# EdoardoLuciani/ARayTracingJourney

Measured on AMD Instinct MI355X. Metric: Mray/s (primary+shadow), Sponza-class 1080p, higher is better.
Workload: dtype f32; 1 GPU; sponza_like(seed=0x5A0A, 262816 triangles, 25 primitives) 1920x1080, 1 light(s), 794216 shadow rays/frame; width=1920, height=1080, lights=1, parallelism=single GPU, 8 frames in flight

## Files before the change

### araytracingjourney_amd/_abi.py

```python
import ctypes as C

ART_OK = 0
ART_E_INVALID = -1
ART_E_STATE = -2
ART_E_NO_DEVICE = -3
ART_E_HIP = -4
ART_E_NOMEM = -5
ART_FLAG_FAST_BUILD = 2
ART_FLAG_PACKED_TILES = 4
ART_FLAG_FIXED_WAVES = 16
ART_FLAG_TILE_OUTPUT = 32
ART_FLAG_DYNAMIC_SCENE = 64
ART_FLAG_KEEP_DEBUG = 1
ART_MASK_ALL = 255
ART_VIS_CAMERA = 1
ART_VIS_SHADOW = 2
ART_VIS_AO = 4
ART_VIS_QUERY = 8
ART_VERTS_FULL = 0
ART_VERTS_POSITIONS = 1
ART_CAST_CLOSEST = 0
ART_CAST_ANY = 1
ART_CAST_MAX_RAYS = 2147418112
ART_CAST_POOL = 32
# ... 93 lines not shown
                ("layout", C.c_uint32),
                ("stride_bytes", C.c_uint32),
                ("flags", C.c_uint32),
                ("reserved", C.c_uint32)]


class ArtRayCast(C.Structure):
    _fields_ = [("rays_dev", C.c_void_p),
                ("tuv_dev", C.c_void_p),
                ("ids_dev", C.c_void_p),
                ("hit_dev", C.c_void_p),
                ("hip_stream", C.c_void_p),
                ("n", C.c_uint32),
                ("kind", C.c_uint32),
                ("cull_mask", C.c_uint32),
                ("flags", C.c_uint32)]


class ArtRayCastMulti(C.Structure):
    _fields_ = [("rays_dev", C.c_void_p),
                ("tuv_dev", C.c_void_p),
                ("ids_dev", C.c_void_p),
                ("count_dev", C.c_void_p),
                ("hip_stream", C.c_void_p),
                ("n", C.c_uint32),
                ("max_hits", C.c_uint32),
                ("cull_mask", C.c_uint32),
                ("flags", C.c_uint32)]


class ArtRayCrossings(C.Structure):
    _fields_ = [("rays_dev", C.c_void_p),
                ("cross_dev", C.c_void_p),
                ("hip_stream", C.c_void_p),
                ("n", C.c_uint32),
                ("cull_mask", C.c_uint32),
                ("flags", C.c_uint32),
                ("reserved", C.c_uint32)]


class ArtHitResolve(C.Structure):
    _fields_ = [("tuv_dev", C.c_void_p),
                ("ids_dev", C.c_void_p),
                ("pos_dev", C.c_void_p),
                ("ng_dev", C.c_void_p),
                ("ns_dev", C.c_void_p),
                ("uv_dev", C.c_void_p),
                ("albedo_dev", C.c_void_p),
                ("orm_dev", C.c_void_p),
                ("hip_stream", C.c_void_p),
                ("n", C.c_uint32),
                ("flags", C.c_uint32)]


class ArtPointQuery(C.Structure):
    _fields_ = [("points_dev", C.c_void_p),
                ("duv_dev", C.c_void_p),
                ("ids_dev", C.c_void_p),
                ("point_dev", C.c_void_p),
                ("hip_stream", C.c_void_p),
                ("n", C.c_uint32),
                ("cull_mask", C.c_uint32),
                ("flags", C.c_uint32),
                ("reserved", C.c_uint32)]


class ArtSphereCast(C.Structure):
    _fields_ = [("rays_dev", C.c_void_p),
                ("tuv_dev", C.c_void_p),
                ("ids_dev", C.c_void_p),
                ("point_dev", C.c_void_p),
                ("hip_stream", C.c_void_p),
                ("n", C.c_uint32),
                ("cull_mask", C.c_uint32),
                ("flags", C.c_uint32),
                ("radius", C.c_float)]


class ArtPointQueryMulti(C.Structure):
    _fields_ = [("points_dev", C.c_void_p),
                ("duv_dev", C.c_void_p),
                ("ids_dev", C.c_void_p),
                ("point_dev", C.c_void_p),
                ("count_dev", C.c_void_p),
                ("hip_stream", C.c_void_p),
                ("n", C.c_uint32),
                ("max_hits", C.c_uint32),
                ("cull_mask", C.c_uint32),
                ("flags", C.c_uint32)]


class ArtBoxQuery(C.Structure):
    _fields_ = [("boxes_dev", C.c_void_p),
                ("hit_dev", C.c_void_p),
                ("ids_dev", C.c_void_p),
                ("count_dev", C.c_void_p),
                ("hip_stream", C.c_void_p),
                ("n", C.c_uint32),
                ("kind", C.c_uint32),
                ("max_hits", C.c_uint32),
                ("cull_mask", C.c_uint32),
                ("flags", C.c_uint32),
                ("reserved", C.c_uint32)]


class ArtTriQuery(C.Structure):
    _fields_ = [("tris_dev", C.c_void_p),
                ("hit_dev", C.c_void_p),
                ("ids_dev", C.c_void_p),
                ("count_dev", C.c_void_p),
                ("hip_stream", C.c_void_p),
                ("n", C.c_uint32),
                ("kind", C.c_uint32),
                ("max_hits", C.c_uint32),
                ("cull_mask", C.c_uint32),
                ("flags", C.c_uint32),
                ("reserved", C.c_uint32)]


class ArtTriDistance(C.Structure):
    _fields_ = [("tris_dev", C.c_void_p),
                ("duv_dev", C.c_void_p),
                ("ids_dev", C.c_void_p),
                ("point_dev", C.c_void_p),
                ("qpoint_dev", C.c_void_p),
                ("hip_stream", C.c_void_p),
                ("n", C.c_uint32),
                ("cull_mask", C.c_uint32),
                ("flags", C.c_uint32),
                ("reserved", C.c_uint32)]


class ArtLayout(C.Structure):
    _fields_ = [("width", C.c_uint32),
                ("height", C.c_uint32),
                ("frames_in_flight", C.c_uint32),
                ("frames_per_launch", C.c_uint32),
                ("shard_rank", C.c_uint32),
                ("shard_count", C.c_uint32),
                ("tiles_owned", C.c_uint32),
                ("tiles_padded", C.c_uint32),
                ("tile_bytes", C.c_uint32),
                ("reserved", C.c_uint32)]


class ArtMgpuConfig(C.Structure):
    _fields_ = [("rank", C.c_uint32),
                ("world", C.c_uint32),
                ("compositor", C.c_uint32),
                ("launches_per_gather", C.c_uint32),
                ("tile_buffers", C.c_uint32),
                ("transport", C.c_uint32),
                ("exchange", ArtMgpuExchangeFn),
                ("exchange_user", C.c_void_p),
                ("roots", C.c_uint32),
                ("reserved", C.c_uint32)]


class ArtGlbCopyInfo(C.Structure):
    _fields_ = [("mesh_buffer_offset", C.c_uint64),
                ("mesh_size", C.c_uint64),
                ("indices_buffer_offset", C.c_uint64),
                ("indices_size", C.c_uint64),
                ("image_buffer_offset", C.c_uint64),
                ("image_size", C.c_uint64),
                ("single_mesh_element_size", C.c_uint32),
                ("single_index_size", C.c_uint32),
                ("image_format", C.c_uint32),
                ("image_width", C.c_uint32),
                ("image_height", C.c_uint32),
                ("image_mip_levels", C.c_uint32),
                ("image_layers", C.c_uint32),
                ("reserved", C.c_uint32)]


SYMBOLS = {
    "art_last_error": (C.c_char_p, []),
    "art_device_count": (C.c_int32, []),
    "art_create": (C.c_int32, [C.c_void_p, C.c_void_p]),
    "art_destroy": (C.c_int32, [C.c_void_p]),
    "art_set_stream": (C.c_int32, [C.c_void_p, C.c_void_p]),
    "art_set_frames_per_launch": (C.c_int32, [C.c_void_p, C.c_uint32]),
    "art_set_camera_batch": (C.c_int32, [C.c_void_p, C.c_void_p, C.c_uint32]),
    "art_set_read_frame": (C.c_int32, [C.c_void_p, C.c_uint32]),
    "art_frames_in_flight": (C.c_int32, [C.c_void_p, C.c_void_p, C.c_void_p]),
    "art_frames_done": (C.c_int32, [C.c_void_p, C.c_uint64, C.c_uint32, C.c_void_p, C.c_void_p]),
    "art_scene_add_primitive": (C.c_int32, [C.c_void_p, C.c_void_p, C.c_uint32, C.c_void_p, C.c_uint32, C.c_uint32, C.c_void_p, C.c_uint32, C.c_uint32, C.c_void_p, C.c_void_p]),
    "art_scene_clear": (C.c_int32, [C.c_void_p]),
    "art_scene_set_primitive_enabled": (C.c_int32, [C.c_void_p, C.c_uint32, C.c_int32]),
    "art_scene_set_alpha_cutoff": (C.c_int32, [C.c_void_p, C.c_uint32, C.c_float]),
    "art_scene_set_primitive_mask": (C.c_int32, [C.c_void_p, C.c_uint32, C.c_uint32]),
    "art_set_ray_masks": (C.c_int32, [C.c_void_p, C.c_uint32, C.c_uint32, C.c_uint32]),
    "art_scene_needs_build": (C.c_int32, [C.c_void_p]),
    "art_scene_set_model_matrix": (C.c_int32, [C.c_void_p, C.c_uint32, C.c_uint32, C.c_void_p]),
    "art_scene_set_vertices": (C.c_int32, [C.c_void_p, C.c_uint32, C.c_void_p, C.c_uint32]),
    "art_scene_set_vertices_device": (C.c_int32, [C.c_void_p, C.c_void_p]),
    "art_scene_get_vertices": (C.c_int32, [C.c_void_p, C.c_uint32, C.c_void_p, C.c_uint32]),
    "art_scene_build": (C.c_int32, [C.c_void_p]),
    "art_set_camera": (C.c_int32, [C.c_void_p, C.c_void_p]),
    "art_camera_from_params": (C.c_int32, [C.c_void_p, C.c_void_p, C.c_float, C.c_float, C.c_float, C.c_float, C.c_void_p]),
    "art_set_lights": (C.c_int32, [C.c_void_p, C.c_void_p, C.c_uint32]),
    "art_light_point": (C.c_int32, [C.c_void_p, C.c_void_p, C.c_float, C.c_int32, C.c_void_p]),
    "art_light_spot": (C.c_int32, [C.c_void_p, C.c_void_p, C.c_void_p, C.c_float, C.c_float, C.c_float, C.c_int32, C.c_void_p]),
    "art_light_directional": (C.c_int32, [C.c_void_p, C.c_void_p, C.c_int32, C.c_void_p]),
    "art_light_area": (C.c_int32, [C.c_void_p, C.c_void_p, C.c_void_p, C.c_int32, C.c_void_p, C.c_float, C.c_float, C.c_float, C.c_int32, C.c_void_p]),
    "art_resize": (C.c_int32, [C.c_void_p, C.c_uint32, C.c_uint32]),
    "art_trace": (C.c_int32, [C.c_void_p]),
    "art_trace_ao": (C.c_int32, [C.c_void_p, C.c_uint32, C.c_float]),
    "art_read_ao": (C.c_int32, [C.c_void_p, C.c_void_p, C.c_size_t]),
    "art_present": (C.c_int32, [C.c_void_p]),
    "art_read_present": (C.c_int32, [C.c_void_p, C.c_void_p, C.c_size_t]),
    "art_read_packed": (C.c_int32, [C.c_void_p, C.c_void_p, C.c_void_p, C.c_void_p]),
    "art_lpm_control_block": (C.c_int32, [C.c_int32, C.c_float, C.c_float, C.c_float, C.c_float, C.c_float, C.c_void_p, C.c_void_p, C.c_void_p]),
    "art_sync": (C.c_int32, [C.c_void_p]),
    "art_cast_rays": (C.c_int32, [C.c_void_p, C.c_void_p]),
    "art_cast_rays_multi": (C.c_int32, [C.c_void_p, C.c_void_p]),
    "art_cast_crossings": (C.c_int32, [C.c_void_p, C.c_void_p]),
    "art_cast_sync": (C.c_int32, [C.c_void_p]),
    "art_cast_counts": (C.c_int32, [C.c_void_p, C.c_void_p, C.c_void_p, C.c_void_p]),
    "art_resolve_hits": (C.c_int32, [C.c_void_p, C.c_void_p]),
    "art_closest_points": (C.c_int32, [C.c_void_p, C.c_void_p]),
    "art_cast_spheres": (C.c_int32, [C.c_void_p, C.c_void_p]),
    "art_closest_points_multi": (C.c_int32, [C.c_void_p, C.c_void_p]),
    "art_overlap_boxes": (C.c_int32, [C.c_void_p, C.c_void_p]),
    "art_overlap_triangles": (C.c_int32, [C.c_void_p, C.c_void_p]),
    "art_closest_triangles": (C.c_int32, [C.c_void_p, C.c_void_p]),
    "art_read_color": (C.c_int32, [C.c_void_p, C.c_void_p, C.c_size_t]),
    "art_read_depth": (C.c_int32, [C.c_void_p, C.c_void_p, C.c_size_t]),
    "art_read_normal": (C.c_int32, [C.c_void_p, C.c_void_p, C.c_size_t]),
    "art_device_color": (C.c_int32, [C.c_void_p, C.c_void_p, C.c_void_p]),
    "art_device_depth": (C.c_int32, [C.c_void_p, C.c_void_p, C.c_void_p]),
    "art_device_normal": (C.c_int32, [C.c_void_p, C.c_void_p, C.c_void_p]),
    "art_shard_tile_count": (C.c_int32, [C.c_void_p, C.c_void_p, C.c_void_p]),
    "art_shard_layout": (C.c_int32, [C.c_uint32, C.c_uint32, C.c_uint32, C.c_uint32, C.c_uint32, C.c_void_p, C.c_uint32, C.c_void_p, C.c_void_p]),
    "art_device_color_tiles": (C.c_int32, [C.c_void_p, C.c_void_p, C.c_void_p]),
    "art_untile_gathered": (C.c_int32, [C.c_void_p, C.c_void_p, C.c_uint32, C.c_void_p, C.c_void_p]),
    "art_get_layout": (C.c_int32, [C.c_void_p, C.c_void_p]),
    "art_mgpu_shard": (C.c_int32, [C.c_uint32, C.c_uint32, C.c_uint32, C.c_void_p, C.c_void_p]),
    "art_mgpu_unique_id": (C.c_int32, [C.c_void_p]),
    "art_mgpu_create": (C.c_int32, [C.c_void_p, C.c_void_p, C.c_void_p, C.c_void_p]),
    "art_mgpu_trace": (C.c_int32, [C.c_void_p]),
    "art_mgpu_flush": (C.c_int32, [C.c_void_p]),
    "art_mgpu_device_frame": (C.c_int32, [C.c_void_p, C.c_void_p, C.c_void_p]),
    "art_mgpu_read_frame": (C.c_int32, [C.c_void_p, C.c_void_p, C.c_size_t]),
    "art_mgpu_counts": (C.c_int32, [C.c_void_p, C.c_void_p, C.c_void_p, C.c_void_p]),
    "art_mgpu_destroy": (C.c_int32, [C.c_void_p]),
    "art_get_stats": (C.c_int32, [C.c_void_p, C.c_void_p]),
    "art_glb_last_error": (C.c_char_p, []),
    "art_glb_open": (C.c_int32, [C.c_char_p, C.c_int32, C.c_int32, C.c_void_p]),
    "art_glb_close": (C.c_int32, [C.c_void_p]),
    "art_glb_primitive_count": (C.c_int32, [C.c_void_p, C.c_void_p]),
    "art_glb_primitive_alpha": (C.c_int32, [C.c_void_p, C.c_uint32, C.c_void_p, C.c_void_p, C.c_void_p]),
    "art_glb_copy_model_data": (C.c_int32, [C.c_void_p, C.c_uint32, C.c_uint32, C.c_void_p, C.c_size_t, C.c_void_p, C.c_uint32, C.c_void_p]),
    "art_glb_bounding_sphere": (C.c_int32, [C.c_void_p, C.c_void_p, C.c_void_p]),
    "art_glb_permute_pixels": (C.c_int32, [C.c_void_p, C.c_size_t, C.c_uint32, C.c_void_p, C.c_uint32, C.c_uint32, C.c_void_p, C.c_size_t]),
    "art_scene_add_glb": (C.c_int32, [C.c_void_p, C.c_void_p, C.c_void_p, C.c_void_p, C.c_void_p]),
}



class ArtTuning(C.Structure):
    _fields_ = [("frame_form", C.c_uint32),
                ("tree_builder", C.c_uint32),
                ("packet_wide", C.c_uint32),
                ("primary_walk", C.c_uint32),
                ("shadow_walk", C.c_uint32),
                ("ao_walk", C.c_uint32),
                ("block_order", C.c_uint32),
                ("fixed_waves", C.c_uint32),
                ("split_fixed_steps", C.c_uint32),
                ("split_min_steps", C.c_uint32),
                ("split_alpha", C.c_float),
                ("ao_entry_off", C.c_uint32),
                ("trace_chunk", C.c_uint32),
                ("trace_refill", C.c_uint32),
                ("trace_blocks", C.c_uint32),
                ("hw_queues", C.c_uint32),
                ("log", C.c_uint32),
                ("wide_builder", C.c_uint32),
                ("as_versions", C.c_uint32),
                ("refit_rebuild_ratio", C.c_float),
                ("trace_leaf_batch", C.c_uint32),
                ("plan_moving_interval", C.c_uint32),
                ("refit_streams", C.c_uint32),
                ("refit_fold_nodes", C.c_uint32),
                ("shadow_hints", C.c_uint32),
                ("plain_math", C.c_uint32)]


PARITY_SYMBOLS = {
    "art_set_tuning": (C.c_int32, [C.c_void_p, C.c_void_p]),
    "art_read_hits": (C.c_int32, [C.c_void_p, C.c_void_p, C.c_void_p, C.c_size_t]),
    "art_read_shadow_bits": (C.c_int32, [C.c_void_p, C.c_void_p, C.c_size_t]),
    "art_read_shadow_hints": (C.c_int32, [C.c_void_p, C.c_void_p, C.c_size_t]),
    "art_write_shadow_hints": (C.c_int32, [C.c_void_p, C.c_void_p, C.c_size_t]),
    "art_query_closest": (C.c_int32, [C.c_void_p, C.c_void_p, C.c_uint32, C.c_void_p, C.c_void_p]),
    "art_query_any": (C.c_int32, [C.c_void_p, C.c_void_p, C.c_uint32, C.c_void_p]),
    "art_query_closest_masked": (C.c_int32, [C.c_void_p, C.c_void_p, C.c_uint32, C.c_uint32, C.c_void_p, C.c_void_p]),
    "art_query_any_masked": (C.c_int32, [C.c_void_p, C.c_void_p, C.c_uint32, C.c_uint32, C.c_void_p]),
    "art_get_lbvh": (C.c_int32, [C.c_void_p, C.c_void_p, C.c_void_p, C.c_void_p, C.c_void_p, C.c_void_p, C.c_void_p, C.c_void_p]),
    "art_get_traversal_tree": (C.c_int32, [C.c_void_p, C.c_void_p, C.c_void_p, C.c_void_p]),
    "art_get_wide_nodes": (C.c_int32, [C.c_void_p, C.c_void_p, C.c_void_p, C.c_size_t, C.c_void_p]),
    "art_parity_math_sweep": (C.c_int32, [C.c_void_p, C.c_uint32, C.c_uint32, C.c_uint64, C.c_uint32, C.c_void_p, C.c_void_p, C.c_void_p, C.c_void_p]),
    "art_parity_radiance_sweep": (C.c_int32, [C.c_void_p, C.c_uint32, C.c_uint32, C.c_uint64, C.c_uint32, C.c_float, C.c_void_p, C.c_void_p, C.c_void_p, C.c_void_p]),
    "art_bind_color_tiles": (C.c_int32, [C.c_void_p, C.c_uint32, C.c_void_p, C.c_size_t]),
    "art_bind_color_tiles_pair": (C.c_int32, [C.c_void_p, C.c_uint32, C.c_void_p, C.c_void_p, C.c_size_t]),
    "art_bind_color_tiles_ring": (C.c_int32, [C.c_void_p, C.c_uint32, C.c_void_p, C.c_uint32, C.c_size_t]),
    "art_read_color_tiles": (C.c_int32, [C.c_void_p, C.c_void_p, C.c_size_t]),
    "art_untile_gathered_strided": (C.c_int32, [C.c_void_p, C.c_void_p, C.c_uint32, C.c_uint32, C.c_void_p, C.c_void_p]),
    "art_untile_gathered_frames": (C.c_int32, [C.c_void_p, C.c_void_p, C.c_uint32, C.c_uint32, C.c_uint32, C.c_void_p, C.c_void_p]),
    "art_stream_wait_frame": (C.c_int32, [C.c_void_p, C.c_void_p]),
    "art_trace_for_stream": (C.c_int32, [C.c_void_p, C.c_void_p, C.c_void_p]),
    "art_wait_external_event": (C.c_int32, [C.c_void_p, C.c_void_p]),
    "art_set_graph_mode": (C.c_int32, [C.c_void_p, C.c_int32]),
    "art_timestamp_mark": (C.c_int32, [C.c_void_p, C.c_uint32]),
    "art_timestamp_elapsed": (C.c_int32, [C.c_void_p, C.c_void_p]),
    "art_collect_timings": (C.c_int32, [C.c_void_p, C.c_void_p, C.c_void_p]),
    "art_sample_wave_steps": (C.c_int32, [C.c_void_p, C.c_void_p, C.c_void_p, C.c_uint32, C.c_void_p]),
    "art_parity_plan": (C.c_int32, [C.c_void_p, C.c_uint32, C.c_void_p, C.c_void_p, C.c_uint32, C.c_void_p, C.c_void_p, C.c_void_p, C.c_uint32, C.c_float, C.c_uint32, C.c_uint32, C.c_void_p, C.c_void_p, C.c_void_p, C.c_void_p]),
    "art_read_wave_plan": (C.c_int32, [C.c_void_p, C.c_void_p, C.c_size_t, C.c_void_p, C.c_uint32, C.c_void_p, C.c_void_p, C.c_void_p]),
    "art_parity_live_resources": (C.c_int32, [C.c_void_p]),
    "art_vertex_update_counts": (C.c_int32, [C.c_void_p, C.c_void_p, C.c_void_p, C.c_void_p]),
    "art_mgpu_pending": (C.c_int32, [C.c_void_p, C.c_void_p, C.c_void_p]),
}
```

### araytracingjourney_amd/csrc/art_api.hip

```cpp
#include "art_context.h"
#include <mutex>
#include <cmath>
#include <cstdio>
#include <cstdlib>
#include <cstring>
#include <new>

static thread_local std::string g_err;
int32_t art::fail(int32_t code, const std::string &msg) { g_err = msg; return code; }
int32_t art::hipfail(hipError_t e, const char *what) { return fail(ART_E_HIP, std::string(what) + ": " + hipGetErrorString(e)); }
void art::set_last_error(const char *msg) { g_err = msg ? msg : ""; }

static std::mutex g_stream_mutex;
static std::vector<std::pair<int, hipStream_t>> g_free_streams;
hipError_t art::acquire_stream(int device, hipStream_t *out) {
    {
        std::lock_guard<std::mutex> lock(g_stream_mutex);
        for (size_t i = 0; i < g_free_streams.size(); i++)
            if (g_free_streams[i].first == device) { *out = g_free_streams[i].second; g_free_streams.erase(g_free_streams.begin() + (long)i); live_add(kLivePooled, -1); live_add(kLiveStreams, 1); return hipSuccess; }
    }
    hipError_t e = hipStreamCreateWithFlags(out, hipStreamNonBlocking);
    if (e == hipSuccess) live_add(kLiveStreams, 1); else *out = nullptr;
    return e;
}
// ... 654 lines not shown
    if (owned) *owned = mine;
    if (padded) *padded = mx;
    return ART_OK;
}
int32_t art_shard_tile_count(ArtContext *c, uint32_t *owned, uint32_t *padded) {
    if (!c) return fail(ART_E_INVALID, "art_shard_tile_count: null context");
    int32_t r = ensure_layout(c, "art_shard_tile_count"); if (r) return r;
    if (owned) *owned = (uint32_t)c->tile_list.size();
    if (padded) *padded = c->padded_tiles;
    return ART_OK;
}
int32_t art_device_color_tiles(ArtContext *c, void **p, size_t *b) {
    int32_t r = device_ready(c, p, "art_device_color_tiles"); if (r) return r;
    *p = nullptr; if (b) *b = 0;
    if (!c->tiled()) return fail(ART_E_STATE, "art_device_color_tiles: context is not sharded");
    FrameSlot &S = c->slot[c->last];
    const size_t one = c->tiles_bytes();
    *p = (char *)S.last_tiles() + c->read_b * one; if (b) *b = one;
    return ART_OK;
}
int32_t art_bind_color_tiles(ArtContext *c, uint32_t slot, void *dev, size_t bytes) {
    if (!c) return fail(ART_E_INVALID, "art_bind_color_tiles: null context");
    if (!c->tiled()) return fail(ART_E_STATE, "art_bind_color_tiles: context is not sharded");
    if (slot >= c->F) return fail(ART_E_INVALID, "art_bind_color_tiles: slot >= frames in flight");
    int32_t r = ensure_layout(c, "art_bind_color_tiles"); if (r) return r;
    if (dev && bytes != c->tiles_bytes() * c->B) return fail(ART_E_INVALID, "art_bind_color_tiles: size mismatch (padded tiles x tile bytes x frames per launch)");
    HIPC(hipStreamSynchronize(c->stream_of(slot)));
    c->slot[slot].ext_tiles = (float4 *)dev; c->slot[slot].ext_ring_n = 0; c->slot[slot].tiles_of_last = nullptr; c->slot[slot].ext_tiles_bytes = dev ? bytes : 0;
    drop_graphs(c);
    return ART_OK;
}
int32_t art_bind_color_tiles_pair(ArtContext *c, uint32_t slot, void *dev_even, void *dev_odd, size_t bytes) {
    if (!dev_even || !dev_odd) return fail(ART_E_INVALID, "art_bind_color_tiles_pair: null buffer");
    void *two[2] = {dev_even, dev_odd};
    return art_bind_color_tiles_ring(c, slot, two, 2, bytes);
}
int32_t art_bind_color_tiles_ring(ArtContext *c, uint32_t slot, void *const *bufs, uint32_t n, size_t bytes) {
    if (!bufs || n == 0 || n > FrameSlot::kTileRing) return fail(ART_E_INVALID, "art_bind_color_tiles_ring: 1..8 buffers");
    for (uint32_t i = 0; i < n; i++) if (!bufs[i]) return fail(ART_E_INVALID, "art_bind_color_tiles_ring: null buffer");
    int32_t r = art_bind_color_tiles(c, slot, bufs[0], bytes); if (r) return r;
    for (uint32_t i = 0; i < n; i++) c->slot[slot].ext_ring[i] = (float4 *)bufs[i];
    c->slot[slot].ext_ring_n = n;
    return ART_OK;
}
int32_t art_set_graph_mode(ArtContext *c, int32_t on) {
    if (!c) return fail(ART_E_INVALID, "art_set_graph_mode: null context");
    if (on && c->ext_stream) return fail(ART_E_STATE, "art_set_graph_mode: not with an external stream");
    c->graph_mode = on != 0;
    if (!on) drop_graphs(c);
    return ART_OK;
}
int32_t art_frames_in_flight(ArtContext *c, uint32_t *frames, uint32_t *next_slot) {
    if (!c) return fail(ART_E_INVALID, "art_frames_in_flight: null context");
    if (frames) *frames = c->F;
    if (next_slot) *next_slot = (uint32_t)(c->frame_no % c->F);
    return ART_OK;
}
int32_t art_frames_done(ArtContext *c, uint64_t first, uint32_t count, int32_t *done, uint64_t *traced) {
    if (!c || !done) return fail(ART_E_INVALID, "art_frames_done: null argument");
    if (traced) *traced = c->frame_no;
    *done = 0;
    if (count == 0) { *done = 1; return ART_OK; }
    if (first + count > c->frame_no) return fail(ART_E_INVALID, "art_frames_done: frames not traced yet");
    if (c->frame_no - first > (uint64_t)ArtContext::kRing) return fail(ART_E_INVALID, "art_frames_done: older than the 128 frames whose events are kept");
    int32_t r = use_device(c); if (r) return r;
    for (uint64_t f = first + count; f-- > first;) {
        hipError_t e = hipEventQuery(c->ev[f % ArtContext::kRing][4]);
        if (e == hipErrorNotReady) return ART_OK;
        if (e != hipSuccess) return hipfail(e, "art_frames_done: hipEventQuery");
    }
    *done = 1;
    return ART_OK;
}
int32_t art_stream_wait_frame(ArtContext *c, void *hip_stream) {
    if (!c) return fail(ART_E_INVALID, "art_stream_wait_frame: null context");
    if (!c->traced) return fail(ART_E_STATE, "art_stream_wait_frame: nothing traced yet");
    int32_t r = use_device(c); if (r) return r;
    { FrameSlot &S = c->slot[c->last]; HIPC(hipStreamWaitEvent((hipStream_t)hip_stream, S.done_alias ? S.done_alias : S.done, 0)); }
    return ART_OK;
}
int32_t art_trace_for_stream(ArtContext *c, void *hip_stream, uint32_t *slot_used) {
    if (!c) return fail(ART_E_INVALID, "art_trace_for_stream: null context");
    const uint32_t k = (uint32_t)(c->frame_no % c->F);
    int32_t r = art_trace(c); if (r) return r;
    if (slot_used) *slot_used = k;
    return art_stream_wait_frame(c, hip_stream);
}
int32_t art_wait_external_event(ArtContext *c, void *hip_event) {
    if (!c) return fail(ART_E_INVALID, "art_wait_external_event: null context");
    c->slot[c->frame_no % c->F].wait_event = hip_event;
    return ART_OK;
}
int32_t art_collect_timings(ArtContext *c, float sums_ms[5], uint32_t *n_frames) {
    if (!c || !sums_ms || !n_frames) return fail(ART_E_INVALID, "art_collect_timings: null argument");
    int32_t r = use_device(c); if (r) return r;
    r = sync_all(c); if (r) return r;
    uint64_t from = c->collected_upto;
    if (c->frame_no - from > (uint64_t)ArtContext::kRing) from = c->frame_no - ArtContext::kRing;
    for (int k = 0; k < 5; k++) sums_ms[k] = 0.f;
    for (uint64_t f = from; f < c->frame_no; f++) {
        const Event *ev = c->ev[f % ArtContext::kRing];
        float ms = 0;
        if (c->ev_fused[f % ArtContext::kRing]) { HIPC(hipEventElapsedTime(&ms, ev[0], ev[4])); sums_ms[0] += ms; sums_ms[4] += ms; continue; }
        for (int k = 0; k < 4; k++) { HIPC(hipEventElapsedTime(&ms, ev[k], ev[k + 1])); sums_ms[k] += ms; }
        HIPC(hipEventElapsedTime(&ms, ev[0], ev[4])); sums_ms[4] += ms;
    }
    *n_frames = (uint32_t)(c->frame_no - from);
    c->collected_upto = c->frame_no;
    return ART_OK;
}
int32_t art_read_color_tiles(ArtContext *c, void *dst, size_t bytes) {
    if (c && !c->tiled()) return fail(ART_E_STATE, "art_read_color_tiles: context is not sharded");
    FrameSlot *S = c ? &c->slot[c->last] : nullptr;
    const size_t one = c ? c->tiles_bytes() : 0;
    return read_back(c, S ? (const char *)S->last_tiles() + c->read_b * one : nullptr, one, dst, bytes, "art_read_color_tiles");
}
int32_t art_untile_gathered_frames(ArtContext *c, const void *gathered_dev, uint32_t shard_count, uint32_t shard_stride_tiles, uint32_t n_frames, void *frames_dev, void *hip_stream) {
    if (!c || !gathered_dev) return fail(ART_E_INVALID, "art_untile_gathered: null argument");
    int32_t r = ensure_layout(c, "art_untile_gathered"); if (r) return r;
    if (shard_stride_tiles < c->padded_tiles) return fail(ART_E_INVALID, "art_untile_gathered: stride smaller than a shard's padded tile count");
    if (n_frames == 0 || (n_frames > 1 && (!frames_dev || (uint64_t)n_frames * c->padded_tiles > shard_stride_tiles))) return fail(ART_E_INVALID, "art_untile_gathered_frames: frames do not fit the shard stride (or no output given)");
    if (shard_count != (c->cfg.shard_count > 1 ? c->cfg.shard_count : 1)) return fail(ART_E_INVALID, "art_untile_gathered: shard_count differs from the context's");
    r = use_device(c); if (r) return r;
    hipStream_t us = hip_stream ? (hipStream_t)hip_stream : c->stream_of(c->last);
    if (c->tiles_packed()) {
        FrameSlot &S = c->slot[c->last];
        if (!frames_dev && S.d_pcolor.n < (size_t)c->W * c->H) { HIPC(hipStreamSynchronize(us)); HIPC(S.d_pcolor.ensure((size_t)c->W * c->H)); }
        launch_untile_packed((const uint32_t *)gathered_dev, c->d_tile_slot.p, shard_stride_tiles, n_frames, c->padded_tiles, c->W, c->H, frames_dev ? (uint32_t *)frames_dev : S.d_pcolor.p, us);
    } else
    launch_untile((const float4 *)gathered_dev, c->d_tile_slot.p, shard_stride_tiles, n_frames, c->padded_tiles, c->W, c->H, frames_dev ? (float4 *)frames_dev : c->slot[c->last].d_color.p, us);
    HIPC(hipGetLastError());
    c->traced = true;
    return ART_OK;
}
int32_t art_untile_gathered_strided(ArtContext *c, const void *gathered_dev, uint32_t shard_count, uint32_t shard_stride_tiles, void *frame_dev, void *hip_stream) {
    return art_untile_gathered_frames(c, gathered_dev, shard_count, shard_stride_tiles, 1, frame_dev, hip_stream);
}
int32_t art_untile_gathered(ArtContext *c, const void *gathered_dev, uint32_t shard_count, void *frame_dev, void *hip_stream) {
    if (!c) return fail(ART_E_INVALID, "art_untile_gathered: null argument");
    int32_t r = ensure_layout(c, "art_untile_gathered"); if (r) return r;
    return art_untile_gathered_strided(c, gathered_dev, shard_count, c->padded_tiles, frame_dev, hip_stream);
}

int32_t art_get_layout(ArtContext *c, ArtLayout *out) {
    if (!c || !out) return fail(ART_E_INVALID, "art_get_layout: null argument");
    int32_t r = ensure_layout(c, "art_get_layout"); if (r) return r;
    std::memset(out, 0, sizeof(*out));
    out->width = c->W; out->height = c->H; out->frames_in_flight = c->F; out->frames_per_launch = c->B;
    out->shard_rank = c->cfg.shard_count > 1 ? c->cfg.shard_rank : 0; out->shard_count = c->cfg.shard_count > 1 ? c->cfg.shard_count : 1;
    out->tiles_owned = (uint32_t)c->tile_list.size(); out->tiles_padded = c->padded_tiles; out->tile_bytes = c->tiled() ? (uint32_t)(kTilePixels * c->tile_px_bytes()) : 0u;
    return ART_OK;
}
int32_t art_timestamp_mark(ArtContext *c, uint32_t which) {
    if (!c || which > 1) return fail(ART_E_INVALID, "art_timestamp_mark: mark 0 or 1");
    if (!c->traced) return fail(ART_E_STATE, "art_timestamp_mark: nothing traced yet");
    int32_t r = use_device(c); if (r) return r;
    HIPC(c->mark[which].create());
    HIPC(hipEventRecord(c->mark[which], c->stream_of(c->last)));
    return ART_OK;
}
int32_t art_timestamp_elapsed(ArtContext *c, float *ms) {
    if (!c || !ms) return fail(ART_E_INVALID, "art_timestamp_elapsed: null argument");
    if (!c->mark[0] || !c->mark[1]) return fail(ART_E_STATE, "art_timestamp_elapsed: both marks must have been recorded");
    int32_t r = use_device(c); if (r) return r;
    HIPC(hipEventSynchronize(c->mark[1]));
    HIPC(hipEventElapsedTime(ms, c->mark[0], c->mark[1]));
    return ART_OK;
}

int32_t art_get_stats(ArtContext *c, ArtStats *out) {
    if (!c || !out) return fail(ART_E_INVALID, "art_get_stats: null argument");
    if (c->traced && c->frame_ready) {
        int32_t r = use_device(c); if (r) return r;
        r = sync_all(c); if (r) return r;
        std::vector<uint32_t> raw(kCounterWords);
        if (c->fused_frame()) {
            FrameSlot &S = c->slot[c->last];
            HIPC(hipMemsetAsync(S.d_counters.p, 0, kCounterWords * 4, c->stream_of(c->last)));
            if (c->n_local) {
                FrameArgs fa = make_frame_args(c, S, S.as_version);
                fa.pix_bits += (size_t)c->read_b * c->n_local; fa.depth += (size_t)c->read_b * c->W * c->H;
                launch_frame_stats(fa, S.d_counters.p, c->stream_of(c->last)); HIPC(hipGetLastError());
            }
            HIPC(hipStreamSynchronize(c->stream_of(c->last)));
        }
        HIPC(hipMemcpy(raw.data(), c->slot[c->last].d_counters.p, kCounterWords * 4, hipMemcpyDeviceToHost));
        uint64_t cnt[2] = {raw[0], raw[1]};
        for (uint32_t k = 0; k < kSlotCount; k++) { cnt[0] += raw[kShadowSlots + k * kSlotStride]; cnt[1] += raw[kHitSlots + k * kSlotStride]; }
        uint64_t owned = 0;
        for (uint32_t t : c->tile_list) {
            uint32_t tx = t % c->tiles_x, ty = t / c->tiles_x;
            uint32_t w = (tx + 1) * kTile <= c->W ? kTile : c->W - tx * kTile, h = (ty + 1) * kTile <= c->H ? kTile : c->H - ty * kTile;
            owned += (uint64_t)w * h;
        }
        c->stats.primary_rays = owned; c->stats.shadow_rays = cnt[0]; c->stats.hit_pixels = cnt[1];
        c->stats.frame_launches = c->fused_frame() ? 1u : 4u;
        c->stats.split_blocks = c->plan.split1 + c->plan.split2;
        harvest_cost(c);
        c->stats.ao_rays = (uint64_t)c->ao_spp * cnt[1];
        if (c->ao_spp && c->slot[c->last].ao_valid) { float ams = 0; if (hipEventElapsedTime(&ams, c->slot[c->last].ao_ev[0], c->slot[c->last].ao_ev[1]) == hipSuccess) c->stats.ao_ms = ams; }
        float ms = 0;
        if (c->frame_no) {
            const Event *ev = c->ev[(c->frame_no - 1) % ArtContext::kRing];
            if (hipEventElapsedTime(&ms, ev[0], ev[4]) == hipSuccess) c->stats.frame_ms = ms;
            if (c->ev_fused[(c->frame_no - 1) % ArtContext::kRing]) { c->stats.trace_primary_ms = c->stats.frame_ms; c->stats.shade_ms = c->stats.trace_shadow_ms = c->stats.accumulate_ms = 0.f; }
            else {
            if (hipEventElapsedTime(&ms, ev[0], ev[1]) == hipSuccess) c->stats.trace_primary_ms = ms;
            if (hipEventElapsedTime(&ms, ev[1], ev[2]) == hipSuccess) c->stats.shade_ms = ms;
            if (hipEventElapsedTime(&ms, ev[2], ev[3]) == hipSuccess) c->stats.trace_shadow_ms = ms;
            if (hipEventElapsedTime(&ms, ev[3], ev[4]) == hipSuccess) c->stats.accumulate_ms = ms;
            }
        }
    }
    as_fill_stats(c, &c->stats);
    *out = c->stats;
    return ART_OK;
}

static bool local_to_xy(const ArtContext *c, uint32_t p, uint32_t &x, uint32_t &y) {
    const uint32_t tile = c->tile_list[p >> 10], q = p & 1023u, sub = q >> 6, l = q & 63u;
    x = (tile % c->tiles_x) * kTile + (sub & 3u) * 8u + (l & 7u); y = (tile / c->tiles_x) * kTile + (sub >> 2) * 8u + (l >> 3);
    return x < c->W && y < c->H;
}
int32_t art_read_hits(ArtContext *c, float *tuv, int32_t *ids, size_t n_pixels) {
    if (!c || !tuv || !ids) return fail(ART_E_INVALID, "art_read_hits: null argument");
    if (!c->traced) return fail(ART_E_STATE, "art_read_hits: nothing traced yet");
    if (n_pixels != (size_t)c->W * c->H) return fail(ART_E_INVALID, "art_read_hits: size mismatch");
    if (c->fused_frame() && !(c->cfg.flags & ART_FLAG_KEEP_DEBUG)) return fail(ART_E_STATE, "art_read_hits: fused frames keep hit records only with ART_FLAG_KEEP_DEBUG");
    int32_t r = use_device(c); if (r) return r;
    r = sync_all(c); if (r) return r;
    std::vector<float4> h(c->n_local);
    std::vector<DevTri> tris(c->T);
    HIPC(hipMemcpy(h.data(), c->slot[c->last].d_hits.p + (size_t)c->read_b * c->n_local, (size_t)c->n_local * 16, hipMemcpyDeviceToHost));
    HIPC(hipMemcpy(tris.data(), c->bvh.tris, (size_t)c->T * sizeof(DevTri), hipMemcpyDeviceToHost));
    for (size_t i = 0; i < n_pixels; i++) { tuv[4 * i] = 0; tuv[4 * i + 1] = 0; tuv[4 * i + 2] = 0; tuv[4 * i + 3] = 0; ids[2 * i] = -2; ids[2 * i + 1] = -2; }
    for (uint32_t p = 0; p < c->n_local; p++) {
        uint32_t x, y;
        if (!local_to_xy(c, p, x, y)) continue;
        size_t i = (size_t)y * c->W + x;
        uint32_t pos; std::memcpy(&pos, &h[p].w, 4);
        tuv[4 * i] = h[p].x; tuv[4 * i + 1] = h[p].y; tuv[4 * i + 2] = h[p].z;
        if (pos == kNoHit) { ids[2 * i] = -1; ids[2 * i + 1] = -1; }
        else { uint32_t gid; std::memcpy(&gid, &tris[pos].f[15], 4); gid_to_ids(c, gid, ids + 2 * i); }
    }
    return ART_OK;
}

int32_t art_read_shadow_bits(ArtContext *c, uint32_t *bits, size_t n_pixels) {
    if (!c || !bits) return fail(ART_E_INVALID, "art_read_shadow_bits: null argument");
    if (!(c->cfg.flags & ART_FLAG_KEEP_DEBUG)) return fail(ART_E_STATE, "art_read_shadow_bits: context created without ART_FLAG_KEEP_DEBUG");
    if (!c->traced) return fail(ART_E_STATE, "art_read_shadow_bits: nothing traced yet");
    if (n_pixels != (size_t)c->W * c->H) return fail(ART_E_INVALID, "art_read_shadow_bits: size mismatch");
    int32_t r = use_device(c); if (r) return r;
    r = sync_all(c); if (r) return r;
    std::vector<uint32_t> sb(c->n_local);
    HIPC(hipMemcpy(sb.data(), c->slot[c->last].d_shadow_bits.p + (size_t)c->read_b * c->n_local, (size_t)c->n_local * 4, hipMemcpyDeviceToHost));
    std::memset(bits, 0, n_pixels * 4);
    for (uint32_t p = 0; p < c->n_local; p++) {
        uint32_t x, y;
        if (!local_to_xy(c, p, x, y)) continue;
        bits[(size_t)y * c->W + x] = sb[p];
    }
    return ART_OK;
}

int32_t art_read_shadow_hints(ArtContext *c, uint32_t *words, size_t n_words) {
    if (!c || !words) return fail(ART_E_INVALID, "art_read_shadow_hints: null argument");
    int32_t r = use_device(c); if (r) return r;
    r = sync_all(c); if (r) return r;
    if (!c->frame_ready) return fail(ART_E_STATE, "art_read_shadow_hints: no frame layout yet (art_trace)");
    if (n_words != c->hint_words()) return fail(ART_E_INVALID, "art_read_shadow_hints: size mismatch");
    if (n_words) HIPC(hipMemcpy(words, c->d_hints.p, n_words * 4, hipMemcpyDeviceToHost));
    return ART_OK;
}
int32_t art_write_shadow_hints(ArtContext *c, const uint32_t *words, size_t n_words) {
    if (!c || !words) return fail(ART_E_INVALID, "art_write_shadow_hints: null argument");
    int32_t r = use_device(c); if (r) return r;
    r = sync_all(c); if (r) return r;
    if (!c->frame_ready) return fail(ART_E_STATE, "art_write_shadow_hints: no frame layout yet (art_trace)");
    if (n_words != c->hint_words()) return fail(ART_E_INVALID, "art_write_shadow_hints: size mismatch");
    if (n_words) HIPC(hipMemcpy(c->d_hints.p, words, n_words * 4, hipMemcpyHostToDevice));
    HIPC(hipDeviceSynchronize());
    return ART_OK;
}

int32_t art_parity_math_sweep(ArtContext *c, uint32_t which, uint32_t first_bits, uint64_t count, uint32_t stride, uint64_t *mismatches, uint32_t *first_bad_bits,
                              uint64_t *fast_lanes, float guard[2]) {
    if (!c || !mismatches || !first_bad_bits || !fast_lanes || !guard) return fail(ART_E_INVALID, "art_parity_math_sweep: null argument");
    if (which > 4 || count > (1ull << 32)) return fail(ART_E_INVALID, "art_parity_math_sweep: which 0..4, at most 2^32 patterns");
    int32_t r = use_device(c); if (r) return r;
    r = sync_all(c); if (r) return r;
    math_sweep_guard(guard);
    unsigned long long h[3] = {0ull, ~0ull, 0ull};
    DevBuf<unsigned long long> d;
    HIPC(d.ensure(3));
    HIPC(hipMemcpy(d.p, h, sizeof h, hipMemcpyHostToDevice));
    launch_math_sweep(which, first_bits, count, stride, d.p, nullptr); HIPC(hipGetLastError());
    HIPC(hipMemcpy(h, d.p, sizeof h, hipMemcpyDeviceToHost));
    *mismatches = h[0]; *fast_lanes = h[2];
    if (h[0]) *first_bad_bits = first_bits + (uint32_t)h[1] * stride;
    return ART_OK;
}

int32_t art_parity_radiance_sweep(ArtContext *c, uint32_t which, uint32_t first_bits, uint64_t count, uint32_t stride, float numerator, uint32_t *max_ulps, uint32_t *worst_bits,
                                  uint64_t *class_mismatches, uint32_t *first_class_bits) {
    if (!c || !max_ulps || !worst_bits || !class_mismatches || !first_class_bits) return fail(ART_E_INVALID, "art_parity_radiance_sweep: null argument");
    if (which > 1 || count > (1ull << 32)) return fail(ART_E_INVALID, "art_parity_radiance_sweep: which 0..1, at most 2^32 patterns");
    int32_t r = use_device(c); if (r) return r;
    r = sync_all(c); if (r) return r;
    unsigned long long h[3] = {0ull, 0ull, ~0ull};
    DevBuf<unsigned long long> d;
    HIPC(d.ensure(3));
    HIPC(hipMemcpy(d.p, h, sizeof h, hipMemcpyHostToDevice));
    launch_radiance_sweep(which, first_bits, count, stride, numerator, d.p, nullptr); HIPC(hipGetLastError());
    HIPC(hipMemcpy(h, d.p, sizeof h, hipMemcpyDeviceToHost));
    *max_ulps = (uint32_t)(h[0] >> 32); *class_mismatches = h[1];
    if (h[0]) *worst_bits = first_bits + (uint32_t)h[0] * stride;
    if (h[1]) *first_class_bits = first_bits + (uint32_t)h[2] * stride;
    return ART_OK;
}

int32_t art_parity_live_resources(uint64_t out[5]) {
    if (!out) return fail(ART_E_INVALID, "art_parity_live_resources: null argument");
    for (int i = 0; i < 5; i++) out[i] = g_live[i].load(std::memory_order_relaxed);
    return ART_OK;
}

}
```

### araytracingjourney_amd/csrc/art_device.h

```cpp
#pragma once
#include "art_internal.h"

namespace art {

struct V3 { float x, y, z; };
__device__ __forceinline__ V3 mk(float x, float y, float z) { V3 r; r.x = x; r.y = y; r.z = z; return r; }
__device__ __forceinline__ V3 operator+(V3 a, V3 b) { return mk(a.x + b.x, a.y + b.y, a.z + b.z); }
__device__ __forceinline__ V3 operator-(V3 a, V3 b) { return mk(a.x - b.x, a.y - b.y, a.z - b.z); }
__device__ __forceinline__ V3 operator*(V3 a, V3 b) { return mk(a.x * b.x, a.y * b.y, a.z * b.z); }
__device__ __forceinline__ V3 operator*(V3 a, float s) { return mk(a.x * s, a.y * s, a.z * s); }
__device__ __forceinline__ V3 neg(V3 a) { return mk(-a.x, -a.y, -a.z); }
__device__ __forceinline__ float dot3(V3 a, V3 b) { return fmaf(a.z, b.z, fmaf(a.y, b.y, a.x * b.x)); }
__device__ __forceinline__ V3 cross3(V3 a, V3 b) {
    return mk(fmaf(a.y, b.z, -(a.z * b.y)), fmaf(a.z, b.x, -(a.x * b.z)), fmaf(a.x, b.y, -(a.y * b.x)));
}
constexpr float kExactLo = 0x1p-96f, kExactHi = 0x1p96f;
__device__ __forceinline__ float sqrt_core(float x) {
    float s = __builtin_amdgcn_sqrtf(x);
    float dn = __uint_as_float(__float_as_uint(s) - 1u), up = __uint_as_float(__float_as_uint(s) + 1u);
    float vp = fmaf(-dn, s, x), vs = fmaf(-up, s, x);
    s = vp <= 0.0f ? dn : s;
    return vs > 0.0f ? up : s;
}
__device__ __forceinline__ float rcp_core(float d) {
    float r = __builtin_amdgcn_rcpf(d);
    r = fmaf(fmaf(-d, r, 1.0f), r, r);
    float q = fmaf(fmaf(-d, r, 1.0f), r, r);
    return fmaf(fmaf(-d, q, 1.0f), r, q);
}
__device__ __forceinline__ bool exact_in_range(float x, bool plain) {
    return !plain && __builtin_amdgcn_ballot_w64(!(x >= kExactLo && x <= kExactHi)) == 0ull;
}
template <bool FAST = true> __device__ __forceinline__ float inv_sqrt_exact(float x, bool plain, bool &fast) {
    fast = FAST && exact_in_range(x, plain);
    if (fast) return rcp_core(sqrt_core(x));
    return 1.0f / sqrtf(x);
}
template <bool FAST = true> __device__ __forceinline__ float sqrt_exact(float x, bool plain, bool &fast) {
    fast = FAST && exact_in_range(x, plain);
    if (fast) return sqrt_core(x);
    return sqrtf(x);
}
__device__ __forceinline__ void exact_note(float x, uint32_t &far) { far = max(far, __float_as_uint(x) - __float_as_uint(kExactLo)); }
__device__ __forceinline__ bool exact_noted_in_range(uint32_t far) { return __builtin_amdgcn_ballot_w64(far > __float_as_uint(kExactHi) - __float_as_uint(kExactLo)) == 0ull; }
template <bool FAST = true> __device__ __forceinline__ float len3(V3 a, bool plain = false) { bool f; return sqrt_exact<FAST>(dot3(a, a), plain, f); }
template <bool FAST = true> __device__ __forceinline__ V3 nrm3(V3 a, bool plain = false) { bool f; float inv = inv_sqrt_exact<FAST>(dot3(a, a), plain, f); return a * inv; }
__device__ __forceinline__ float inv_sqrt_noting(float x, uint32_t &far) { exact_note(x, far); return rcp_core(sqrt_core(x)); }
template <bool CORE> __device__ __forceinline__ V3 nrm3_noting(V3 a, uint32_t &far) {
    float x = dot3(a, a);
    return a * (CORE ? inv_sqrt_noting(x, far) : 1.0f / sqrtf(x));
}
__device__ __forceinline__ float clampf(float x, float lo, float hi) { return fminf(fmaxf(x, lo), hi); }
__device__ __forceinline__ float mixf(float x, float y, float a) { return x * (1.0f - a) + y * a; }
__device__ __forceinline__ V3 ld3(const float *p) { return mk(p[0], p[1], p[2]); }
__device__ __forceinline__ V3 mat4_mul(const float *m, float x, float y, float z, float w) {
    return mk(((m[0] * x + m[4] * y) + m[8] * z) + m[12] * w, ((m[1] * x + m[5] * y) + m[9] * z) + m[13] * w,
              ((m[2] * x + m[6] * y) + m[10] * z) + m[14] * w);
}
__device__ __forceinline__ V3 xform_point(const float *m, V3 p) {
    return mk(((m[0] * p.x + m[1] * p.y) + m[2] * p.z) + m[3], ((m[4] * p.x + m[5] * p.y) + m[6] * p.z) + m[7],
              ((m[8] * p.x + m[9] * p.y) + m[10] * p.z) + m[11]);
}
__device__ __forceinline__ V3 xform_vec(const float *m, V3 p) {
    return mk((m[0] * p.x + m[1] * p.y) + m[2] * p.z, (m[4] * p.x + m[5] * p.y) + m[6] * p.z, (m[8] * p.x + m[9] * p.y) + m[10] * p.z);
}

__device__ __forceinline__ int wrapi(int i, int n) { int m = i % n; return m < 0 ? m + n : m; }
__device__ __forceinline__ void tex_taps(const uint32_t *__restrict__ pool, uint32_t texture_offset, uint32_t tw_, uint32_t th_, int layer, float u, float v,
                                         uint32_t &t00, uint32_t &t10, uint32_t &t01, uint32_t &t11, float &fx, float &fy) {
    int tw = (int)tw_, th = (int)th_;
    float x = u * (float)tw - 0.5f, y = v * (float)th - 0.5f;
    float x0f = floorf(x), y0f = floorf(y);
    fx = x - x0f; fy = y - y0f;
    int x0 = wrapi((int)x0f, tw), y0 = wrapi((int)y0f, th);
    int x1 = wrapi(x0 + 1, tw), y1 = wrapi(y0 + 1, th);
    const uint32_t *base = pool + texture_offset + (size_t)layer * tw * th;
    t00 = base[(size_t)y0 * tw + x0]; t10 = base[(size_t)y0 * tw + x1]; t01 = base[(size_t)y1 * tw + x0]; t11 = base[(size_t)y1 * tw + x1];
}
__device__ __forceinline__ float tex_channel(uint32_t t00, uint32_t t10, uint32_t t01, uint32_t t11, float fx, float fy, int c) {
    const float k = 1.0f / 255.0f;
    float A = (float)((t00 >> (8 * c)) & 255u) * k, B = (float)((t10 >> (8 * c)) & 255u) * k;
    float Cc = (float)((t01 >> (8 * c)) & 255u) * k, D = (float)((t11 >> (8 * c)) & 255u) * k;
    float top = A * (1.0f - fx) + B * fx, bot = Cc * (1.0f - fx) + D * fx;
    return top * (1.0f - fy) + bot * fy;
}
__device__ inline float4 sample_tex(const uint32_t *__restrict__ pool, const DevPrim &P, int layer, float u, float v) {
    int tw = (int)P.tw, th = (int)P.th;
    float x = u * (float)tw - 0.5f, y = v * (float)th - 0.5f;
    float x0f = floorf(x), y0f = floorf(y);
    float fx = x - x0f, fy = y - y0f;
    int x0 = wrapi((int)x0f, tw), y0 = wrapi((int)y0f, th);
    int x1 = wrapi(x0 + 1, tw), y1 = wrapi(y0 + 1, th);
    const uint32_t *base = pool + P.texture_offset + (size_t)layer * tw * th;
    uint32_t t00 = base[(size_t)y0 * tw + x0], t10 = base[(size_t)y0 * tw + x1], t01 = base[(size_t)y1 * tw + x0], t11 = base[(size_t)y1 * tw + x1];
    float o[4];
#pragma unroll
    for (int c = 0; c < 4; c++) o[c] = tex_channel(t00, t10, t01, t11, fx, fy, c);
    return make_float4(o[0], o[1], o[2], o[3]);
}


struct AlphaView {
    const uint32_t *bits;
    const DevShadeTri *shade;
    const DevPrim *prims;
    const uint32_t *tex;
    uint32_t cull;
};
__device__ __forceinline__ float alpha_at(const uint32_t *__restrict__ pool, uint32_t texture_offset, uint32_t tw, uint32_t th, float4 s2, float4 s3, float u, float v) {
    float bx = 1.0f - u - v, by = u, bz = v;
    float tu = (s2.y * bx + s2.w * by) + s3.y * bz, tv = (s2.z * bx + s3.x * by) + s3.z * bz;
    uint32_t t00, t10, t01, t11; float fx, fy;
    tex_taps(pool, texture_offset, tw, th, 0, tu, tv, t00, t10, t01, t11, fx, fy);
    return tex_channel(t00, t10, t01, t11, fx, fy, 3);
}
__device__ __forceinline__ bool alpha_cut(const AlphaView &av, uint32_t pos, float u, float v) {
    if (av.cull == 0u) return true;
    if (!((av.bits[pos >> 5] >> (pos & 31u)) & 1u)) return false;
    const float4 *sq = reinterpret_cast<const float4 *>(av.shade + pos);
    const float4 s8 = sq[8];
    const DevPrim &P = av.prims[__float_as_uint(s8.z)];
    if ((prim_vis(P.masked) & av.cull) == 0u) return true;
    const float4 s2 = sq[2], s3 = sq[3];
    const float c = P.cutoff;
    if (!(c > 0.0f)) return false;
    return alpha_at(av.tex, P.texture_offset, P.tw, P.th, s2, s3, u, v) < c;
}

struct Ray {
    V3 o, d;
    float tmin, tmax;
    V3 inv, ood;
};
__device__ __forceinline__ float safe_dir(float d) { return fabsf(d) < 1e-20f ? copysignf(1e-20f, d) : d; }
__device__ __forceinline__ void ray_init(Ray &r, V3 o, V3 d, float tmin, float tmax) {
    r.o = o; r.d = d; r.tmin = tmin; r.tmax = tmax;
    r.inv = mk(1.0f / safe_dir(d.x), 1.0f / safe_dir(d.y), 1.0f / safe_dir(d.z));
    r.ood = mk(o.x * r.inv.x, o.y * r.inv.y, o.z * r.inv.z);
}
__device__ __forceinline__ void ray_init_inv(Ray &r, V3 o, V3 d, V3 inv, float tmin, float tmax) {
    r.o = o; r.d = d; r.tmin = tmin; r.tmax = tmax; r.inv = inv;
    r.ood = mk(o.x * inv.x, o.y * inv.y, o.z * inv.z);
}
__device__ __forceinline__ bool ray_finite(V3 o, V3 d) {
    float z = 0.0f * o.x; z = fmaf(0.0f, o.y, z); z = fmaf(0.0f, o.z, z); z = fmaf(0.0f, d.x, z); z = fmaf(0.0f, d.y, z); z = fmaf(0.0f, d.z, z);
    return z == 0.0f;
}
__device__ __forceinline__ bool slab(const Ray &r, float lx, float ly, float lz, float hx, float hy, float hz, float tlimit, float &tn) {
    float t0x = fmaf(lx, r.inv.x, -r.ood.x), t1x = fmaf(hx, r.inv.x, -r.ood.x);
    float t0y = fmaf(ly, r.inv.y, -r.ood.y), t1y = fmaf(hy, r.inv.y, -r.ood.y);
    float t0z = fmaf(lz, r.inv.z, -r.ood.z), t1z = fmaf(hz, r.inv.z, -r.ood.z);
    tn = fmaxf(fmaxf(fminf(t0x, t1x), fminf(t0y, t1y)), fminf(t0z, t1z));
    float tf = fminf(fminf(fmaxf(t0x, t1x), fmaxf(t0y, t1y)), fmaxf(t0z, t1z));
    return fmaxf(tn, r.tmin) <= fminf(tf, tlimit);
}
#define ART_BARY_EPS 1.0e-6f
__device__ __forceinline__ bool moller_trumbore(const Ray &r, V3 v0, V3 e1, V3 e2, float &t, float &u, float &v) {
    V3 p = cross3(r.d, e2);
    float det = dot3(e1, p);
    if (det == 0.0f) return false;
    float inv = 1.0f / det;
    V3 tv = r.o - v0;
    float uu = dot3(tv, p) * inv;
    if (!(uu >= -ART_BARY_EPS && uu <= 1.0f + ART_BARY_EPS)) return false;
    V3 q = cross3(tv, e1);
    float vv = dot3(r.d, q) * inv;
    if (!(vv >= -ART_BARY_EPS && uu + vv <= 1.0f + ART_BARY_EPS)) return false;
    float tt = dot3(e2, q) * inv;
    if (!(tt > r.tmin && tt < r.tmax)) return false;
    t = tt; u = uu; v = vv;
    return true;
}
__device__ __forceinline__ bool moller_trumbore_det(const Ray &r, V3 v0, V3 e1, V3 e2, float &t, float &u, float &v, float &det_out) {
    V3 p = cross3(r.d, e2);
    float det = dot3(e1, p);
    if (det == 0.0f) return false;
    float inv = 1.0f / det;
    V3 tv = r.o - v0;
    float uu = dot3(tv, p) * inv;
    if (!(uu >= -ART_BARY_EPS && uu <= 1.0f + ART_BARY_EPS)) return false;
    V3 q = cross3(tv, e1);
    float vv = dot3(r.d, q) * inv;
    if (!(vv >= -ART_BARY_EPS && uu + vv <= 1.0f + ART_BARY_EPS)) return false;
    float tt = dot3(e2, q) * inv;
    if (!(tt > r.tmin && tt < r.tmax)) return false;
    t = tt; u = uu; v = vv; det_out = det;
    return true;
}

__device__ __forceinline__ bool moller_trumbore_flat(const Ray &r, V3 v0, V3 e1, V3 e2, float &t, float &u, float &v) {
    V3 p = cross3(r.d, e2);
    float det = dot3(e1, p);
    float inv = 1.0f / det;
    V3 tv = r.o - v0;
    u = dot3(tv, p) * inv;
    V3 q = cross3(tv, e1);
    v = dot3(r.d, q) * inv;
    t = dot3(e2, q) * inv;
    return (det != 0.0f) & (u >= -ART_BARY_EPS) & (u <= 1.0f + ART_BARY_EPS) & (v >= -ART_BARY_EPS) & (u + v <= 1.0f + ART_BARY_EPS) & (t > r.tmin) & (t < r.tmax);
}

__device__ __forceinline__ uint64_t moller_trumbore_mask(const Ray &r, V3 v0, V3 e1, V3 e2, float &t, float &u, float &v) {
    V3 p = cross3(r.d, e2);
    float det = dot3(e1, p);
    float inv = 1.0f / det;
    V3 tv = r.o - v0;
    u = dot3(tv, p) * inv;
    V3 q = cross3(tv, e1);
    v = dot3(r.d, q) * inv;
    t = dot3(e2, q) * inv;
    return __builtin_amdgcn_ballot_w64(det != 0.0f) & __builtin_amdgcn_ballot_w64(u >= -ART_BARY_EPS) & __builtin_amdgcn_ballot_w64(u <= 1.0f + ART_BARY_EPS) &
           __builtin_amdgcn_ballot_w64(v >= -ART_BARY_EPS) & __builtin_amdgcn_ballot_w64(u + v <= 1.0f + ART_BARY_EPS) & __builtin_amdgcn_ballot_w64(t > r.tmin) &
           __builtin_amdgcn_ballot_w64(t < r.tmax);
}

constexpr int kLdsStack = 16;
constexpr int kOvfStack = 80;
constexpr int kBlock = 256;
constexpr int kFrameBlock = 64;
constexpr int kTraceBlock = 64;
struct Tune { uint32_t chunk, refill, blocks, leaf_batch; };
static const Tune kPreset[4] = {{64, 12, 1536, 1}, {128, 24, 1024, 1}, {256, 16, 2048, 8}, {1024, 24, 2048, 8}};
static inline Tune tune_over(Tune t, const TraceTune &o) {
    if (o.chunk >= 64 && o.chunk <= 65536) t.chunk = o.chunk;
    if (o.refill >= 1 && o.refill <= 64) t.refill = o.refill;
    if (o.blocks >= 1 && o.blocks <= 16384) t.blocks = o.blocks;
    if (o.leaf_batch >= 1 && o.leaf_batch <= 64) t.leaf_batch = o.leaf_batch;
    return t;
}
static inline Tune tune(bool pipelined, bool ao, const TraceTune &o) { return tune_over(kPreset[(ao ? 2 : 0) + (pipelined ? 1 : 0)], o); }
constexpr int kCursorStride = 32;

__device__ __forceinline__ bool local_to_xy(uint32_t p, const uint32_t *__restrict__ tile_list, uint32_t tiles_x, uint32_t W, uint32_t H, uint32_t &x, uint32_t &y) {
    uint32_t tile = tile_list[p >> 10];
    uint32_t q = p & 1023u, sub = q >> 6, l = q & 63u;
    x = (tile % tiles_x) * kTile + (sub & 3u) * 8u + (l & 7u);
    y = (tile / tiles_x) * kTile + (sub >> 2) * 8u + (l >> 3);
    return x < W && y < H;
}

__device__ __forceinline__ uint32_t launder(uint32_t v) { asm volatile("" : "+s"(v)); return v; }
__device__ __forceinline__ uint32_t launder_v(uint32_t v) { asm volatile("" : "+v"(v)); return v; }
__device__ __forceinline__ uint64_t ballot64(bool p) { return __builtin_amdgcn_ballot_w64(p); }

typedef float f4v __attribute__((ext_vector_type(4)));
__device__ __forceinline__ void st_nt(float4 *p, float4 v) { __builtin_nontemporal_store(f4v{v.x, v.y, v.z, v.w}, reinterpret_cast<f4v *>(p)); }
__device__ __forceinline__ void st_nt(float *p, float v) { __builtin_nontemporal_store(v, p); }
typedef float f3v __attribute__((ext_vector_type(3)));
__device__ __forceinline__ void st_nt_rgb(float4 *tiles, size_t texel, float4 v) { __builtin_nontemporal_store(f3v{v.x, v.y, v.z}, reinterpret_cast<f3v *>(reinterpret_cast<float *>(tiles) + 3 * texel)); }
__device__ __forceinline__ float4 ld_nt(const float4 *p) { f4v v = __builtin_nontemporal_load(reinterpret_cast<const f4v *>(p)); return make_float4(v.x, v.y, v.z, v.w); }

static inline uint32_t blocks_for(uint32_t n) { return (n + kBlock - 1) / kBlock; }
static inline uint32_t persistent_blocks(uint32_t total, const Tune &t) {
    uint32_t need = (total + kTraceBlock - 1) / kTraceBlock, cap = t.blocks * (kBlock / kTraceBlock);
    return need < cap ? (need ? need : 1u) : cap;
}

}
```

### araytracingjourney_amd/csrc/art_frame.hip

```cpp
#include "art_shade.h"
#include <type_traits>

namespace art {

constexpr int kPacketStack = 288;

__device__ __forceinline__ void sel(float &x, float y, uint64_t m) { asm("v_cndmask_b32_e64 %0, %0, %1, %2" : "+v"(x) : "v"(y), "s"(m)); }
__device__ __forceinline__ void sel(uint32_t &x, uint32_t y, uint64_t m) { asm("v_cndmask_b32_e64 %0, %0, %1, %2" : "+v"(x) : "v"(y), "s"(m)); }
__device__ __forceinline__ void sel_off(float &x, uint64_t m) { asm("v_cndmask_b32_e64 %0, %0, -1.0, %1" : "+v"(x) : "s"(m)); }

template <int OCT> __device__ __forceinline__ bool slab_oct(const Ray &r, float lx, float ly, float lz, float hx, float hy, float hz, float tlimit, float &tn) {
    if (OCT >= 8) return slab(r, lx, ly, lz, hx, hy, hz, tlimit, tn);
    float nx = fmaf((OCT & 1) ? hx : lx, r.inv.x, -r.ood.x), fx = fmaf((OCT & 1) ? lx : hx, r.inv.x, -r.ood.x);
    float ny = fmaf((OCT & 2) ? hy : ly, r.inv.y, -r.ood.y), fy = fmaf((OCT & 2) ? ly : hy, r.inv.y, -r.ood.y);
    float nz = fmaf((OCT & 4) ? hz : lz, r.inv.z, -r.ood.z), fz = fmaf((OCT & 4) ? lz : hz, r.inv.z, -r.ood.z);
    tn = fmaxf(fmaxf(nx, ny), nz);
    float tf = fminf(fminf(fx, fy), fz);
    return fmaxf(tn, r.tmin) <= fminf(tf, tlimit);
}

struct ConstQuads {
    typedef float Quad __attribute__((ext_vector_type(4)));
    __attribute__((address_space(4))) const Quad *p;
    __device__ __forceinline__ float4 operator[](int i) const { Quad v = p[i]; return make_float4(v.x, v.y, v.z, v.w); }
};
template <class T> __device__ __forceinline__ ConstQuads const_quads(const T *p) { ConstQuads q; q.p = (__attribute__((address_space(4))) const ConstQuads::Quad *)(uintptr_t)p; return q; }

#ifdef ART_PACKET_PROF
__device__ unsigned long long g_packet_prof[24];
#define PPROF(i, n) do { if ((threadIdx.x & 63u) == 0) atomicAdd(&g_packet_prof[(ANY ? 12 : 0) + (i)], (unsigned long long)(n)); } while (0)
#else
#define PPROF(i, n)
#endif
struct PacketHints { int cur, sp; uint32_t n; };
__device__ __forceinline__ PacketHints hints_seed(int *stk, uint32_t w0, uint32_t w1, uint32_t w2, uint32_t w3, uint32_t n_leaves) {
    PacketHints h{0, 0, 0u};
    if ((w0 & w1 & w2 & w3) == kHintEmpty) return h;
    const bool lane0 = (threadIdx.x & 63u) == 0;
    if (w3 < n_leaves) { if (lane0) stk[h.sp] = h.cur; h.sp++; h.cur = (int)~w3; }
    if (w2 < n_leaves) { if (lane0) stk[h.sp] = h.cur; h.sp++; h.cur = (int)~w2; }
    if (w1 < n_leaves) { if (lane0) stk[h.sp] = h.cur; h.sp++; h.cur = (int)~w1; }
    if (w0 < n_leaves) { if (lane0) stk[h.sp] = h.cur; h.sp++; h.cur = (int)~w0; }
    return h;
}
struct StepUpdate { uint64_t m = 0ull; float t, u, v; uint32_t pos, gid; };
struct NoUpdate {};
template <bool ANY, bool WIDE, int OCT, bool COUNT = false, bool ALPHA = false, bool HINTS = false, class ON>
__device__ __forceinline__ void packet_walk(const FrameArgs &a, const Ray &r, ON &on, int *stk, float &tbest, float &bu, float &bv, uint32_t &bpos, uint32_t &bgid, uint32_t &steps, PacketHints &h) {
    constexpr bool MASKS = std::is_same<ON, uint64_t>::value;
    int cur = HINTS ? h.cur : 0, sp = HINTS ? h.sp : 0;
    constexpr int kPop = kAbsentChild;
    const auto cull = [&]() -> uint32_t { return ANY ? (a.ray_masks >> 8) & 0xFFu : a.ray_masks & 0xFFu; };
    if (ALPHA && cull() == 0u) return;
#ifdef ART_PACKET_PROF
    unsigned long long pp_[12] = {1, 0, 0, 0, 0, 0, 0, OCT == 8, 0, 0, 0, 0}; bool from_stack_ = false; int hints_left_ = 0;
#endif
#ifdef ART_PACKET_PROF
    if (HINTS) hints_left_ = sp;
#endif
    typename std::conditional<MASKS, StepUpdate, NoUpdate>::type up;
    for (;;) {
#ifdef ART_PACKET_PROF
        const unsigned long long tk0_ = __builtin_amdgcn_s_memtime(); const bool was_node_ = cur >= 0;
#endif
        if constexpr (MASKS) up.m = 0ull;
        if (COUNT) steps++;
        if (cur >= 0 && WIDE) {
            ConstQuads nq = const_quads(a.widef + cur);
            float4 w0 = nq[0], w1 = nq[1], w2 = nq[2], w3 = nq[3], w4 = nq[4], w5 = nq[5], w6 = nq[6], w7 = nq[7];
            const int c0 = __float_as_int(w6.x), c1 = __float_as_int(w6.y), c2 = __float_as_int(w6.z), c3 = __float_as_int(w6.w);
            float te;
            const uint64_t m0 = ballot64(slab_oct<OCT>(r, w0.x, w0.y, w0.z, w0.w, w1.x, w1.y, tbest, te));
            const uint64_t m1 = ballot64(slab_oct<OCT>(r, w1.z, w1.w, w2.x, w2.y, w2.z, w2.w, tbest, te));
            const uint64_t m2 = ballot64(slab_oct<OCT>(r, w3.x, w3.y, w3.z, w3.w, w4.x, w4.y, tbest, te));
            const uint64_t m3 = ballot64(slab_oct<OCT>(r, w4.z, w4.w, w5.x, w5.y, w5.z, w5.w, tbest, te));
#ifdef ART_PACKET_PROF
            pp_[1]++; pp_[6] += (m0 != 0ull) + (m1 != 0ull) + (m2 != 0ull) + (m3 != 0ull); from_stack_ = false;
#endif
            const uint32_t ax = __float_as_uint(w7.y);
            bool rev = ((OCT >> ax) & 1) != 0;
            if constexpr (OCT >= 8 && MASKS) rev = 2 * (int)__popcll(on & ballot64((ax == 0 ? r.inv.x : (ax == 1 ? r.inv.y : r.inv.z)) < 0.0f)) > (int)__popcll(on);
            else if constexpr (OCT >= 8) rev = 2 * (int)__popcll(ballot64(on && (ax == 0 ? r.inv.x : (ax == 1 ? r.inv.y : r.inv.z)) < 0.0f)) > (int)__popcll(ballot64(on));
            const bool lane0 = (threadIdx.x & 63u) == 0;
            int next = kPop;
            if (!rev) {
                if (m3 != 0ull) next = c3;
                if (m2 != 0ull) { if (next != kPop) { if (lane0) stk[min(sp, kPacketStack - 1)] = next; sp = min(sp + 1, kPacketStack); } next = c2; }
                if (m1 != 0ull) { if (next != kPop) { if (lane0) stk[min(sp, kPacketStack - 1)] = next; sp = min(sp + 1, kPacketStack); } next = c1; }
                if (m0 != 0ull) { if (next != kPop) { if (lane0) stk[min(sp, kPacketStack - 1)] = next; sp = min(sp + 1, kPacketStack); } next = c0; }
            } else {
                if (m0 != 0ull) next = c0;
                if (m1 != 0ull) { if (next != kPop) { if (lane0) stk[min(sp, kPacketStack - 1)] = next; sp = min(sp + 1, kPacketStack); } next = c1; }
                if (m2 != 0ull) { if (next != kPop) { if (lane0) stk[min(sp, kPacketStack - 1)] = next; sp = min(sp + 1, kPacketStack); } next = c2; }
                if (m3 != 0ull) { if (next != kPop) { if (lane0) stk[min(sp, kPacketStack - 1)] = next; sp = min(sp + 1, kPacketStack); } next = c3; }
            }
            cur = next;
        } else if (cur >= 0) {
            ConstQuads nq = const_quads(a.nodes + cur);
            float4 q0 = nq[0], q1 = nq[1], q2 = nq[2], q3 = nq[3];
            int c0 = __float_as_int(q3.x), c1 = __float_as_int(q3.y);
            float te0, te1;
            uint64_t m0 = ballot64(slab_oct<OCT>(r, q0.x, q0.y, q0.z, q0.w, q1.x, q1.y, tbest, te0));
            uint64_t m1 = ballot64(slab_oct<OCT>(r, q1.z, q1.w, q2.x, q2.y, q2.z, q2.w, tbest, te1));
            if (m0 != 0ull && m1 != 0ull) {
                uint64_t fl = ballot64(te0 <= te1), both = m0 & m1;
                uint64_t f0 = (m0 & ~m1) | (both & fl), f1 = (m1 & ~m0) | (both & ~fl);
                bool first0 = (int)__popcll(f0) >= (int)__popcll(f1);
                if ((threadIdx.x & 63u) == 0) stk[min(sp, kPacketStack - 1)] = first0 ? c1 : c0;
                sp = min(sp + 1, kPacketStack);
                cur = first0 ? c0 : c1;
            } else if (m0 != 0ull) cur = c0;
            else if (m1 != 0ull) cur = c1;
            else cur = kPop;
        } else {
            uint32_t pos = (uint32_t)~cur;
            typedef __attribute__((address_space(4))) const uint32_t *Words;
            bool unseen = false;
            const auto flagged = [&]() -> bool { return ((((Words)(uintptr_t)a.alpha_bits)[pos >> 5] >> (pos & 31u)) & 1u) != 0u; };
            if (ALPHA && flagged()) {
                const float4 s8 = const_quads(a.shade_tris + pos)[8];
                const Words P = (Words)(uintptr_t)(a.prims + __float_as_uint(s8.z));
                unseen = (prim_vis(P[offsetof(DevPrim, masked) / 4]) & cull()) == 0u;
            }
            if (!unseen) {
                ConstQuads tq = const_quads(a.tris + pos);
                float4 ta = tq[0], tb = tq[1], tc = tq[2], td = tq[3];
                float te = 0.f, t = 0.f, u = 0.f, v = 0.f;
                if constexpr (MASKS) {
                    uint64_t acc = moller_trumbore_mask(r, mk(ta.x, ta.y, ta.z), mk(ta.w, tb.x, tb.y), mk(tb.z, tb.w, tc.x), t, u, v) & on;
                    if (acc != 0ull) acc &= ballot64(slab_oct<OCT>(r, tc.y, tc.z, tc.w, td.x, td.y, td.z, tbest, te));
                    const auto alpha_keep = [&](uint64_t cand) -> uint64_t {
                        if (!ALPHA || cand == 0ull || !flagged()) return cand;
                        ConstQuads sq = const_quads(a.shade_tris + pos);
                        const float4 s2 = sq[2], s3 = sq[3], s8 = sq[8];
                        const Words P = (Words)(uintptr_t)(a.prims + __float_as_uint(s8.z));
                        const float c = __uint_as_float(P[offsetof(DevPrim, cutoff) / 4]);
                        if (!(c > 0.0f)) return cand;
                        const uint32_t toff = P[offsetof(DevPrim, texture_offset) / 4], tw = P[offsetof(DevPrim, tw) / 4], th = P[offsetof(DevPrim, th) / 4];
                        bool keep = __builtin_amdgcn_inverse_ballot_w64(cand);
                        if (keep) keep = !(alpha_at(a.tex_pool, toff, tw, th, s2, s3, u, v) < c);
                        return cand & ballot64(keep);
                    };
                    if (ANY) {
                        if (ALPHA) acc = alpha_keep(acc);
                        up.m = acc; up.pos = pos; on &= ~acc;
                        if (HINTS && acc != 0ull) { const uint32_t n = launder(h.n); if ((threadIdx.x & 63u) == 0) stk[kPacketStack + (n & 3u)] = (int)pos; h.n = n + 1u; }
                    }
                    else {
                        float teff;
                        asm("v_max_f32 %0, %1, %2" : "=v"(teff) : "v"(t), "v"(te));
                        uint32_t gid = __float_as_uint(td.w);
                        uint64_t better = acc & (ballot64(teff < tbest) | (ballot64(teff == tbest) & ballot64(gid < bgid)));
                        if (ALPHA) better = alpha_keep(better);
                        up.m = better; up.t = teff; up.u = u; up.v = v; up.pos = pos; up.gid = gid;
                    }
#ifdef ART_PACKET_PROF
                    { uint64_t am_ = acc; pp_[2]++; pp_[3] += from_stack_; pp_[4] += am_ != 0ull; pp_[5] += __popcll(am_); }
                    if (ANY && hints_left_ > 0) { pp_[10]++; pp_[11] += on == 0ull; hints_left_--; }
#endif
                } else {
                    bool acc = moller_trumbore_flat(r, mk(ta.x, ta.y, ta.z), mk(ta.w, tb.x, tb.y), mk(tb.z, tb.w, tc.x), t, u, v) && on;
                    if (acc) acc = slab_oct<OCT>(r, tc.y, tc.z, tc.w, td.x, td.y, td.z, tbest, te);
                    const auto alpha_keep = [&](bool cand) -> bool {
                        if (!ALPHA || ballot64(cand) == 0ull || !flagged()) return cand;
                        ConstQuads sq = const_quads(a.shade_tris + pos);
                        const float4 s2 = sq[2], s3 = sq[3], s8 = sq[8];
                        const Words P = (Words)(uintptr_t)(a.prims + __float_as_uint(s8.z));
                        const float c = __uint_as_float(P[offsetof(DevPrim, cutoff) / 4]);
                        if (!(c > 0.0f)) return cand;
                        const uint32_t toff = P[offsetof(DevPrim, texture_offset) / 4], tw = P[offsetof(DevPrim, tw) / 4], th = P[offsetof(DevPrim, th) / 4];
                        if (cand) cand = !(alpha_at(a.tex_pool, toff, tw, th, s2, s3, u, v) < c);
                        return cand;
                    };
                    if (ANY) {
                        if (ALPHA) acc = alpha_keep(acc);
                        bpos = acc ? pos : bpos; on = on && !acc; tbest = acc ? -1.0f : tbest;
                        if (HINTS && ballot64(acc) != 0ull) { if ((threadIdx.x & 63u) == 0) stk[kPacketStack + (h.n & 3u)] = (int)pos; h.n++; }
                    }
                    else {
                        float teff;
                        asm("v_max_f32 %0, %1, %2" : "=v"(teff) : "v"(t), "v"(te));
                        uint32_t gid = __float_as_uint(td.w);
                        bool better = acc & ((teff < tbest) | ((teff == tbest) & (gid < bgid)));
                        if (ALPHA) better = alpha_keep(better);
                        tbest = better ? teff : tbest; bu = better ? u : bu; bv = better ? v : bv; bpos = better ? pos : bpos; bgid = better ? gid : bgid;
                    }
#ifdef ART_PACKET_PROF
                    { uint64_t am_ = ballot64(acc); pp_[2]++; pp_[3] += from_stack_; pp_[4] += am_ != 0ull; pp_[5] += __popcll(am_); }
                    if (ANY && hints_left_ > 0) { pp_[10]++; pp_[11] += ballot64(on) == 0ull; hints_left_--; }
#endif
                }
                if constexpr (!MASKS) { if (ANY && ballot64(on) == 0ull) break; }
            }
            cur = kPop;
        }
        if constexpr (MASKS) if (up.m != 0ull) {
            if (ANY) { sel(bpos, up.pos, up.m); sel_off(tbest, up.m); if (on == 0ull) break; }
            else { sel(tbest, up.t, up.m); sel(bu, up.u, up.m); sel(bv, up.v, up.m); sel(bpos, up.pos, up.m); sel(bgid, up.gid, up.m); }
        }
        if (cur == kPop) {
            if (sp == 0) break;
            sp--;
            cur = __builtin_amdgcn_readfirstlane(stk[sp]);
#ifdef ART_PACKET_PROF
            from_stack_ = true;
#endif
        }
#ifdef ART_PACKET_PROF
        pp_[was_node_ ? 8 : 9] += __builtin_amdgcn_s_memtime() - tk0_;
#endif
    }
#ifdef ART_PACKET_PROF
    for (int i = 0; i < 12; i++) PPROF(i, pp_[i]);
#endif
}

template <bool ANY, bool WIDE, bool COUNT = false, bool ALPHA = false, bool HINTS = false, bool MASKS = true>
__device__ __forceinline__ void walk_dispatch(const FrameArgs &a, const Ray &r, bool alive, int *stk, float &tbest, float &bu, float &bv, uint32_t &bpos, uint32_t &bgid, uint32_t &steps, PacketHints &h) {
    typename std::conditional<MASKS, uint64_t, bool>::type on;
    int oct;
    if constexpr (MASKS) {
        on = ballot64(alive);
        const uint64_t act = on;
        if (act == 0ull) return;
        uint64_t nx = act & ballot64(r.inv.x < 0.0f), ny = act & ballot64(r.inv.y < 0.0f), nz = act & ballot64(r.inv.z < 0.0f);
        bool uniform = (nx == 0ull || nx == act) && (ny == 0ull || ny == act) && (nz == 0ull || nz == act);
        oct = !uniform ? 8 : (int)(launder(nx ? 2u : 0u) >> 1) | (ny ? 2 : 0) | (nz ? 4 : 0);
    } else {
        on = alive;
        uint64_t act = ballot64(on);
        if (act == 0ull) return;
        uint64_t nx = ballot64(on && r.inv.x < 0.0f), ny = ballot64(on && r.inv.y < 0.0f), nz = ballot64(on && r.inv.z < 0.0f);
        bool uniform = (nx == 0ull || nx == act) && (ny == 0ull || ny == act) && (nz == 0ull || nz == act);
        oct = !uniform ? 8 : (nx ? 1 : 0) | (ny ? 2 : 0) | (nz ? 4 : 0);
    }
    switch (oct) {
    case 0: packet_walk<ANY, WIDE, 0, COUNT, ALPHA, HINTS>(a, r, on, stk, tbest, bu, bv, bpos, bgid, steps, h); break;
    case 1: packet_walk<ANY, WIDE, 1, COUNT, ALPHA, HINTS>(a, r, on, stk, tbest, bu, bv, bpos, bgid, steps, h); break;
    case 2: packet_walk<ANY, WIDE, 2, COUNT, ALPHA, HINTS>(a, r, on, stk, tbest, bu, bv, bpos, bgid, steps, h); break;
    case 3: packet_walk<ANY, WIDE, 3, COUNT, ALPHA, HINTS>(a, r, on, stk, tbest, bu, bv, bpos, bgid, steps, h); break;
    case 4: packet_walk<ANY, WIDE, 4, COUNT, ALPHA, HINTS>(a, r, on, stk, tbest, bu, bv, bpos, bgid, steps, h); break;
    case 5: packet_walk<ANY, WIDE, 5, COUNT, ALPHA, HINTS>(a, r, on, stk, tbest, bu, bv, bpos, bgid, steps, h); break;
    case 6: packet_walk<ANY, WIDE, 6, COUNT, ALPHA, HINTS>(a, r, on, stk, tbest, bu, bv, bpos, bgid, steps, h); break;
    case 7: packet_walk<ANY, WIDE, 7, COUNT, ALPHA, HINTS>(a, r, on, stk, tbest, bu, bv, bpos, bgid, steps, h); break;
    default: packet_walk<ANY, WIDE, 8, COUNT, ALPHA, HINTS>(a, r, on, stk, tbest, bu, bv, bpos, bgid, steps, h); break;
    }
}

__device__ __forceinline__ bool frame_pixel(const FrameArgs &a, uint32_t wid, uint32_t &p, uint32_t &x, uint32_t &y, bool &mine) {
    typedef uint32_t U2 __attribute__((ext_vector_type(2)));
    const U2 item_ = ((__attribute__((address_space(4))) const U2 *)(uintptr_t)a.wave_items)[wid];
    const uint2 item = make_uint2(item_.x, item_.y);
    const uint32_t txy = ((__attribute__((address_space(4))) const uint32_t *)(uintptr_t)a.tile_xy)[item.x >> 4];
    const uint32_t lane = __lane_id(), sub = item.x & 15u;
    p = item.x * 64u + lane;
    mine = (item.y >> (((lane >> 4) << 2) | ((lane >> 1) & 3u))) & 1u;
    x = (txy & 0xFFFFu) * kTile + (sub & 3u) * 8u + (lane & 7u);
    y = (txy >> 16) * kTile + (sub >> 2) * 8u + (lane >> 3);
    return x < a.W && y < a.H && mine;
}
#ifdef ART_PHASE_PROF
constexpr uint32_t kPhaseWaves = 1u << 18;
__device__ uint32_t g_phase[8][kPhaseWaves];
__device__ __forceinline__ uint64_t tick(float &dep) { uint64_t t; asm volatile("s_memtime %0\n\ts_waitcnt lgkmcnt(0)" : "=s"(t), "+v"(dep)); return t; }
#define PHASE(i, dep) { uint64_t t1_ = tick(dep); if (__lane_id() == 0 && blockIdx.x < kPhaseWaves) g_phase[i][blockIdx.x] = (uint32_t)(t1_ - t0_); t0_ = t1_; }
#else
#define PHASE(i, dep)
#endif
template <bool WIDE, bool ONE_LIGHT, bool COUNT, bool BATCH, bool ALPHA> constexpr bool kFrameHints = !(!WIDE && BATCH) && !(ALPHA && !ONE_LIGHT && !COUNT && !BATCH) &&
                                                                                                      !(ALPHA && !WIDE && !ONE_LIGHT && COUNT && !BATCH);
template <bool WIDE, bool ONE_LIGHT, bool COUNT, bool BATCH, bool ALPHA> constexpr bool kFrameFastMath = ONE_LIGHT && !BATCH && !ALPHA;
constexpr uint8_t kFrameMovesTable[32] = {55, 63, 63, 63, 55, 63, 0, 0, 49, 55, 63, 0, 49, 63, 63, 56, 31, 63, 63, 0, 63, 63, 63, 63, 19, 63, 0, 0, 19, 63, 0, 0};
#ifdef ART_MOVES_FORCE
template <bool WIDE, bool ONE_LIGHT, bool COUNT, bool BATCH, bool ALPHA> constexpr uint32_t kFrameMoves = ART_MOVES_FORCE;
#else
template <bool WIDE, bool ONE_LIGHT, bool COUNT, bool BATCH, bool ALPHA> constexpr uint32_t kFrameMoves = kFrameMovesTable[WIDE << 4 | ONE_LIGHT << 3 | COUNT << 2 | BATCH << 1 | ALPHA];
#endif
__device__ __forceinline__ const FrameArgs &frame_args_again(const FrameArgs &a) {
#ifdef __HIP_DEVICE_COMPILE__
    __attribute__((address_space(4))) const char *p = (__attribute__((address_space(4))) const char *)__builtin_amdgcn_kernarg_segment_ptr();
    asm volatile("" : "+s"(p));
    return *(const FrameArgs *)p;
#else
    return a;
#endif
}
template <bool WIDE, bool ONE_LIGHT, bool COUNT = false, bool BATCH = false, bool ALPHA = false>
__global__ __launch_bounds__(kFrameBlock) __attribute__((amdgpu_waves_per_eu(8, 8))) void k_frame(FrameArgs a_) {
    __shared__ int wstack[kPacketStack + 4];
    constexpr bool HINTS = kFrameHints<WIDE, ONE_LIGHT, COUNT, BATCH, ALPHA>;
    constexpr bool FASTM = kFrameFastMath<WIDE, ONE_LIGHT, COUNT, BATCH, ALPHA>;
    constexpr uint32_t MV = kFrameMoves<WIDE, ONE_LIGHT, COUNT, BATCH, ALPHA>;
    int *stk = wstack;
    const uint32_t wid = blockIdx.x;
    if (wid >= a_.n_wave_items) return;
    uint32_t steps = 0;
    const uint32_t fb = BATCH ? blockIdx.y : 0u;
    const CameraArg &cam0 = (BATCH && fb) ? a_.cam_more[fb - 1] : a_.cam;
    const size_t frame_px = (size_t)fb * a_.W * a_.H, frame_local = (size_t)fb * a_.n_local;
    bool in;
    Ray r;
#ifdef ART_PHASE_PROF
    float dep0_ = 0.f; uint64_t t0_ = tick(dep0_);
#endif
    {
        uint32_t p, x, y; bool mine;
        in = frame_pixel(a_, wid, p, x, y, mine);
        float fx = (float)x + 0.5f, fy = (float)y + 0.5f;
        float dx = (fx / (float)a_.W) * 2.0f - 1.0f, dy = (fy / (float)a_.H) * 2.0f - 1.0f;
        V3 org = mat4_mul(cam0.view_inv, 0.f, 0.f, 0.f, 1.f);
        V3 tgt = nrm3<FASTM>(mat4_mul(cam0.proj_inv, dx, dy, 1.f, 1.f), a_.plain_math);
        V3 dir = mat4_mul(cam0.view_inv, tgt.x, tgt.y, tgt.z, 0.f);
        ray_init(r, org, dir, 0.001f, 10000.0f);
    }
    bool on = in && ray_finite(r.o, r.d);
    PHASE(0, r.inv.x)
    float tbest = on ? r.tmax : -1.0f, bu = 0.f, bv = 0.f;
    uint32_t bpos = kNoHit, bgid = kNoHit;
    { PacketHints none{0, 0, 0u}; walk_dispatch<false, WIDE, COUNT, ALPHA, false, (MV & 1u) != 0u>(a_, r, on, stk, tbest, bu, bv, bpos, bgid, steps, none); }
    PHASE(1, tbest)
    const FrameArgs &a = (MV & 2u) ? frame_args_again(a_) : a_;
    const FrameArgs &as = (MV & 4u) ? a : a_;
    const CameraArg &cam = (BATCH && fb) ? as.cam_more[fb - 1] : as.cam;
    uint32_t p, x, y; bool mine;
    frame_pixel(a, wid, p, x, y, mine);
    if (a.keep_hits && mine) a.hits[frame_local + p] = bpos != kNoHit ? make_float4(tbest, bu, bv, __uint_as_float(bpos)) : make_float4(10000.0f, 0.f, 0.f, __uint_as_float(kNoHit));
    const bool hit = in && bpos != kNoHit;
    float out_depth = 10000.0f;
    V3 out_normal = mk(0.5f, 0.5f, 0.5f);
    Surface S;
    S.world_pos = mk(0.f, 0.f, 0.f); S.N = mk(0.f, 0.f, 1.f); S.Vv = mk(0.f, 0.f, 1.f); S.albedo = mk(0.f, 0.f, 0.f);
    S.metallic = 0.f; S.alpha = 0.f; S.nc_NdotV = 0.f; S.NdotV = 0.f;
    if (hit) shade_surface<FASTM, ONE_LIGHT && !BATCH && ALPHA>(as, cam, bpos, bu, bv, S, out_depth, out_normal);
    if (in) {
        const size_t pix = frame_px + (size_t)y * a.W + x;
        st_nt(&a.depth[pix], out_depth);
        st_nt(&a.normal[pix], make_float4(out_normal.x, out_normal.y, out_normal.z, 1.0f));
    }
    PHASE(2, S.NdotV)
    float rx = 0.f, ry = 0.f, rz = 0.f;
    uint32_t sbits = 0, more = 0;
    for (uint32_t i = 0; i < (ONE_LIGHT ? 1u : a_.n_lights); i++) {
        const FrameArgs &b = (MV & 8u) ? frame_args_again(a_) : a_;
        PacketHints hn{0, 0, 0u};
        typedef uint32_t U4 __attribute__((ext_vector_type(4)));
        if (HINTS && b.hints) {
            const uint32_t blk = ((__attribute__((address_space(4))) const uint32_t *)(uintptr_t)b.wave_items)[2u * wid];
            const U4 e = ((__attribute__((address_space(4))) const U4 *)(uintptr_t)b.hints)[blk * kHintLights + (i & (kHintLights - 1u))];
            hn = hints_seed(stk, e.x, e.y, e.z, e.w, b.hint_leaves);
        }
        float4 c4 = make_float4(0.f, 0.f, 0.f, 0.f), ro = make_float4(0.f, 0.f, 0.f, 1.0f), rd = make_float4(0.f, 0.f, 1.f, 0.f);
        bool want = false;
        const ArtLight L = ONE_LIGHT ? b.lights[0] : frame_light(b, i);
        if (hit) want = shade_light<FASTM>(L, S, b.plain_math, c4, ro, rd);
        if (want) { if (i < 16u) sbits |= 1u << (16u + i); else more++; }
        Ray sr;
        if (L.type == 2u) ray_init_inv(sr, mk(ro.x, ro.y, ro.z), ld3(L.area_pos2), ld3(L.area_pos3), 0.01f, L.penumbra_angle);
        else ray_init(sr, mk(ro.x, ro.y, ro.z), mk(rd.x, rd.y, rd.z), 0.01f, ro.w);
        bool son = want && ray_finite(sr.o, sr.d);
        PHASE(3, sr.inv.x)
        float st = son ? sr.tmax : -1.0f, su = 0.f, sv = 0.f;
        uint32_t spos = kNoHit, sgid = kNoHit;
        const uint64_t traced = HINTS ? ballot64(son) : 0ull;
        walk_dispatch<true, WIDE, COUNT, ALPHA, HINTS, (MV & 1u) != 0u>(b, sr, son, stk, st, su, sv, spos, sgid, steps, hn);
        const FrameArgs &c = (MV & 16u) ? frame_args_again(a_) : a_;
        if (HINTS && c.hints && traced != 0ull) {
            uint32_t o[4];
#pragma unroll
            for (uint32_t k = 0; k < 4u; k++) o[k] = k < hn.n ? (uint32_t)stk[kPacketStack + ((hn.n - 1u - k) & 3u)] : kHintEmpty;
            const uint32_t blk = ((__attribute__((address_space(4))) const uint32_t *)(uintptr_t)c.wave_items)[2u * launder(wid)];
            const size_t at = blk * kHintLights + (i & (kHintLights - 1u));
            const U4 e = ((__attribute__((address_space(4))) const U4 *)(uintptr_t)c.hints)[at];
            if (((e.x ^ o[0]) | (e.y ^ o[1]) | (e.z ^ o[2]) | (e.w ^ o[3])) != 0u && __lane_id() == 0) reinterpret_cast<uint4 *>(c.hints)[at] = make_uint4(o[0], o[1], o[2], o[3]);
        }
        PHASE(4, st)
        if (want && spos != kNoHit) {
            c4 = make_float4(c4.x * 0.05f, c4.y * 0.05f, c4.z * 0.05f, c4.w);
            if (i < 16u) sbits |= 1u << i;
        }
        rx += c4.x * c4.w; ry += c4.y * c4.w; rz += c4.z * c4.w;
    }
    if (!in) { rx = 0.f; ry = 0.f; rz = 0.f; }
    float4 o = make_float4(rx, ry, rz, 1.0f);
    const FrameArgs &e = (MV & 32u) ? frame_args_again(a_) : a_;
    frame_pixel(e, wid, p, x, y, mine);
    if (in) st_nt(&e.color[frame_px + (size_t)y * e.W + x], o);
    if (e.color_tiles && mine) {
        uint32_t q = p & 1023u, sub = q >> 6, l = q & 63u;
        uint32_t lx = (sub & 3u) * 8u + (l & 7u), ly = (sub >> 2) * 8u + (l >> 3);
        size_t ti = (size_t)fb * e.tiles_stride + (size_t)(p >> 10) * kTilePixels + ly * kTile + lx;
        if (e.tiles_packed) __builtin_nontemporal_store(pack_b10g11r11(o.x, o.y, o.z), reinterpret_cast<uint32_t *>(e.color_tiles) + ti);
        else st_nt_rgb(e.color_tiles, ti, o);
    }
    if (mine) e.pix_bits[frame_local + p] = sbits;
    if (!ONE_LIGHT && e.pix_more && mine) e.pix_more[frame_local + p] = more;
    PHASE(5, rx)
#ifdef ART_PHASE_PROF
    if (__lane_id() == 0 && blockIdx.x < kPhaseWaves) { g_phase[6][blockIdx.x] = 1u; g_phase[7][blockIdx.x] = steps; }
#endif
    if (COUNT && __lane_id() == 0) e.wave_cost[wid] = steps;
}

__device__ __forceinline__ uint32_t plan_block_sum(uint32_t v, uint32_t *sh) {
    for (int off = 32; off >= 1; off >>= 1) v += (uint32_t)__shfl_xor((int)v, off);
    __syncthreads();
    if ((threadIdx.x & 63u) == 0) sh[threadIdx.x >> 6] = v;
    __syncthreads();
    uint32_t t = 0;
    for (int i = 0; i < 16; i++) t += sh[i];
    return t;
}
__device__ __forceinline__ uint32_t plan_deal(uint32_t j, uint32_t total) { const uint32_t g = j >> 5; return (g + 1u) * 32u <= total ? g * 32u + 8u * (j & 3u) + ((j & 31u) >> 2) : j; }
__global__ __launch_bounds__(1024) void k_plan(PlanArgs p) {
    __shared__ uint32_t sh[16], sc2[1024], sc1[1024];
    __shared__ unsigned long long sh64[16];
    const uint32_t tid = threadIdx.x;
    unsigned long long sum = 0;
    for (uint32_t i = tid; i < p.n_items_in; i += 1024u) { const uint2 it = p.items_in[i]; if (it.y) { const uint32_t c = p.cost[i]; atomicMax(&p.worst[it.x], c); sum += c; } }
    for (int off = 32; off >= 1; off >>= 1) sum += (unsigned long long)__shfl_xor((long long)sum, off);
    if ((tid & 63u) == 0) sh64[tid >> 6] = sum;
    __threadfence_block();
    __syncthreads();
    sum = 0;
    for (int i = 0; i < 16; i++) sum += sh64[i];
    uint32_t T = p.fixed_steps ? p.fixed_steps : max(p.min_steps, (uint32_t)(p.share * (float)sum));
    const uint32_t per = (p.n64 + 1023u) / 1024u, b0 = min(tid * per, p.n64), b1 = min(b0 + per, p.n64);
    uint32_t n1 = 0, n2 = 0, N1 = 0, N2 = 0, ups = 0, downs = 0, split = 0, wmax = 0;
    for (int attempt = 0; attempt < 8; attempt++, T += T / 2) {
        n1 = n2 = 0; uint32_t u = 0, d = 0, sp = 0;
        for (uint32_t b = b0; b < b1; b++) {
            const uint32_t w = __hip_atomic_load(&p.worst[b], __ATOMIC_RELAXED, __HIP_MEMORY_SCOPE_AGENT);
            const uint32_t old = p.level[b];
            uint32_t lv = old;
            if (old == 0) lv = w > 4u * T ? 2u : (w > T ? 1u : 0u);
            else if (old == 1) lv = w > T ? 2u : (w * 4u < T / 2u ? 0u : 1u);
            else lv = w * 4u < T / 2u ? 1u : 2u;
            p.level_tmp[b] = (uint8_t)lv;
            n1 += lv == 1u; n2 += lv == 2u; u += lv > old; d += lv < old; sp += old != 0u; wmax = max(wmax, w);
        }
        N1 = plan_block_sum(n1, sh); N2 = plan_block_sum(n2, sh); ups = plan_block_sum(u, sh); downs = plan_block_sum(d, sh); split = plan_block_sum(sp, sh);
        if (p.n64 + (p.n64 & 3u) + 4u * N1 + 16u * N2 + 32u <= p.cap) break;
        if (attempt == 7) { N1 = N2 = ups = downs = 0; for (uint32_t b = b0; b < b1; b++) p.level_tmp[b] = p.level[b]; n1 = n2 = 0; }
    }
    for (int off = 32; off >= 1; off >>= 1) wmax = max(wmax, (uint32_t)__shfl_xor((int)wmax, off));
    __syncthreads();
    if ((tid & 63u) == 0) sh[tid >> 6] = wmax;
    __syncthreads();
    for (int i = 0; i < 16; i++) wmax = max(wmax, sh[i]);
    for (uint32_t b = b0; b < b1; b++) p.worst[b] = 0u;
    const bool changed = p.fixed_steps ? (ups + downs) != 0u : (ups != 0u || downs > max(16u, split / 4u));
    if (!changed) { if (tid == 0) { p.result[1] = 0u; p.result[4] = T; p.result[5] = wmax; } return; }
    sc2[tid] = n2; sc1[tid] = n1;
    __syncthreads();
    uint32_t base2 = 0, base1 = 0;
    for (uint32_t i = 0; i < tid; i++) { base2 += sc2[i]; base1 += sc1[i]; }
    const uint32_t heavy = 16u * N2 + 4u * N1, heavy_pad = (heavy + 31u) & ~31u, total = heavy_pad + p.n256 * 4u;
    for (uint32_t b = b0; b < b1; b++) {
        const uint32_t lv = p.level_tmp[b];
        p.level[b] = (uint8_t)lv;
        if (lv == 2u) { for (uint32_t cell = 0; cell < 16u; cell++) p.items_out[plan_deal(16u * base2 + cell, total)] = make_uint2(b, 1u << cell); base2++; }
        else if (lv == 1u) { const uint32_t quad[4] = {0x0033u, 0x00CCu, 0x3300u, 0xCC00u}; for (uint32_t q = 0; q < 4u; q++) p.items_out[plan_deal(16u * N2 + 4u * base1 + q, total)] = make_uint2(b, quad[q]); base1++; }
    }
    for (uint32_t j = heavy + tid; j < heavy_pad; j += 1024u) p.items_out[plan_deal(j, total)] = make_uint2(0u, 0u);
    __threadfence_block();
    __syncthreads();
    for (uint32_t r = tid; r < p.n256 * 4u; r += 1024u) {
        const uint32_t b = p.order[r >> 2] * 4u + (r & 3u);
        p.items_out[plan_deal(heavy_pad + r, total)] = make_uint2(b, p.level[b] ? 0u : 0xFFFFu);
    }
    if (tid == 0) { p.result[0] = total; p.result[1] = 1u; p.result[2] = N1; p.result[3] = N2; p.result[4] = T; p.result[5] = wmax; }
}
void launch_plan(const PlanArgs &p, hipStream_t s) { k_plan<<<1, 1024, 0, s>>>(p); }

template <bool WIDE, bool ONE_LIGHT, bool ALPHA = false> static void launch_frame_form(const FrameArgs &a, uint32_t g, bool count, hipStream_t s) {
    if (a.batch > 1) {
        const dim3 gb(g, a.batch);
        if (count) k_frame<WIDE, ONE_LIGHT, true, true, ALPHA><<<gb, kFrameBlock, 0, s>>>(a); else k_frame<WIDE, ONE_LIGHT, false, true, ALPHA><<<gb, kFrameBlock, 0, s>>>(a);
    } else if (count) k_frame<WIDE, ONE_LIGHT, true, false, ALPHA><<<g, kFrameBlock, 0, s>>>(a);
    else k_frame<WIDE, ONE_LIGHT, false, false, ALPHA><<<g, kFrameBlock, 0, s>>>(a);
}
bool launch_frame(const FrameArgs &a, hipStream_t s) {
    const uint32_t g = a.n_wave_items;
    if (g == 0) return false;
    const bool one = a.n_lights == 1;
    const bool count = a.wave_cost != nullptr && a.n_lights > 0;
    if (a.alpha) {
        if (a.packet_wide) { if (one) launch_frame_form<true, true, true>(a, g, count, s); else launch_frame_form<true, false, true>(a, g, count, s); }
        else { if (one) launch_frame_form<false, true, true>(a, g, count, s); else launch_frame_form<false, false, true>(a, g, count, s); }
    } else if (a.packet_wide) { if (one) launch_frame_form<true, true>(a, g, count, s); else launch_frame_form<true, false>(a, g, count, s); }
    else { if (one) launch_frame_form<false, true>(a, g, count, s); else launch_frame_form<false, false>(a, g, count, s); }
    return count;
}
#ifdef ART_PACKET_PROF
extern "C" int32_t art_debug_packet_prof(unsigned long long *out, int32_t reset) {
    if (hipMemcpyFromSymbol(out, HIP_SYMBOL(g_packet_prof), sizeof(g_packet_prof)) != hipSuccess) return -1;
    void *dp = nullptr;
    if (reset && (hipGetSymbolAddress(&dp, HIP_SYMBOL(g_packet_prof)) != hipSuccess || hipMemset(dp, 0, sizeof(g_packet_prof)) != hipSuccess)) return -1;
    return 0;
}
#endif
#ifdef ART_PHASE_PROF
extern "C" int32_t art_debug_phase(uint32_t *out, int32_t reset) {
    if (hipMemcpyFromSymbol(out, HIP_SYMBOL(g_phase), sizeof(g_phase)) != hipSuccess) return -1;
    void *dp = nullptr;
    if (reset && (hipGetSymbolAddress(&dp, HIP_SYMBOL(g_phase)) != hipSuccess || hipMemset(dp, 0, sizeof(g_phase)) != hipSuccess)) return -1;
    return 0;
}
#endif

}
```

### araytracingjourney_amd/csrc/art_internal.h

```cpp
#pragma once
#include <hip/hip_runtime.h>
#include <stdint.h>
#include <cstring>
#include <string>
#include <vector>
#include <algorithm>
#include <utility>
#include "../../include/art.h"
#include "../../include/art_parity.h"
#include "art_own.h"

namespace art {

struct DevPrim {
    const float *vertices;
    const void *indices;
    uint32_t texture_offset;
    uint32_t single_index_size;
    uint32_t tw, th;
    uint32_t first_tri, n_tri;
    float o2w[12];
    float w2o[12];
    uint32_t masked;
    float cutoff;
};
static_assert(sizeof(DevPrim) == 144, "DevPrim layout");
constexpr uint32_t kPrimOut = 1u;
constexpr uint32_t kPrimVisShift = 8u;
__host__ __device__ inline uint32_t prim_vis(uint32_t masked) { return ~(masked >> kPrimVisShift) & 0xFFu; }
constexpr float kNowhere = 3.0e38f;
__host__ __device__ inline bool box_nowhere(float lo_x) { return lo_x >= kNowhere; }

struct alignas(16) DevNode { float4 q[4]; };
struct alignas(16) DevNode4 { float ox, oy, oz; uint32_t exps; uint32_t q[6]; uint32_t spare[2]; int32_t child[4]; };
static_assert(sizeof(DevNode4) == 64, "DevNode4 layout");
struct alignas(16) DevNodeW { float box[4][6]; int32_t child[4]; uint32_t valid; uint32_t pad[3]; };
static_assert(sizeof(DevNodeW) == 128, "DevNodeW layout");
constexpr int32_t kAbsentChild = (int32_t)0x80000000;
struct alignas(16) DevTri { float f[16]; };
static_assert(sizeof(DevTri) == 64, "DevTri layout");
struct alignas(16) DevShadeTri { float f[36]; };

struct CameraArg { float view[16], view_inv[16], proj[16], proj_inv[16], camera_pos[3]; };

constexpr int kTile = 32;
constexpr int kTilePixels = kTile * kTile;
constexpr uint32_t kNoHit = 0xFFFFFFFFu;
constexpr int kMaxLights = 16;
constexpr uint32_t kMaxLightsTotal = 1024;
constexpr uint32_t kMaxFrameSlots = 24;
constexpr uint32_t kTileRingMax = 8;
int32_t ring_rewind(ArtContext *ctx);
void set_last_error(const char *msg);

#define HIPQ(x) do { hipError_t e_ = (x); if (e_ != hipSuccess) return e_; } while (0)
struct BuildInputs {
    const DevPrim *prims; uint32_t n_prims; const uint32_t *prim_first_tri;
    uint32_t T; uint32_t morton_bits;
};
struct Arena {
    DevBuf<char> mem; size_t off = 0;
    uint64_t generation = 0;
    static size_t pad(size_t bytes) { return (bytes + 255) & ~(size_t)255; }
    hipError_t reserve(size_t bytes) {
        off = 0; generation++;
        if (bytes <= mem.n && mem.p) return hipSuccess;
        return mem.ensure(bytes + bytes / 8);
    }
    template <class T> T *take(size_t n) { T *p = reinterpret_cast<T *>(mem.p + off); off += pad(n * sizeof(T)); return p; }
    void release() { mem.release(); off = 0; }
};
struct WalkTree { int32_t *child; float *lo, *hi; };
struct Lbvh {
    Arena *arena = nullptr;
    uint32_t *leaf_gid;
    uint64_t *keys;
    int32_t *child;
    float *node_lo, *node_hi;
    float *leaf_lo, *leaf_hi;
    DevTri *tris;
    DevNode *nodes;
    uint32_t *tri_prim;
    uint32_t *gid_leaf;
    DevBuf<DevNode4> wide;
    DevBuf<DevNodeW> widef;
    uint32_t n_wide;
    bool canon_boxes = false;
    uint32_t log = 0;
    std::vector<uint32_t> wide_levels;
    DevShadeTri *shade_tris;
    DevBuf<uint32_t> leaf_parent;
    DevBuf<uint32_t> node_parent;
    DevBuf<uint32_t> sub_nodes, sub_leaves, sub_off;
    uint32_t sub_batches = 0, sub_levels = 0;
    std::vector<uint32_t> batch_prim_off, batch_prim_ids;
    int32_t *trav_child;
    float *trav_lo, *trav_hi;
    WalkTree walk_tree() const { return trav_child ? WalkTree{trav_child, trav_lo, trav_hi} : WalkTree{child, node_lo, node_hi}; }
    DevBuf<int32_t> own_trav_child; DevBuf<float> own_trav_lo, own_trav_hi;
    DevBuf<char> block;
    int32_t *res_trav_child = nullptr; float *res_trav_lo = nullptr, *res_trav_hi = nullptr;
    uint32_t *cbounds;
};
bool decode_jpeg(const uint8_t *data, size_t n, std::vector<uint8_t> &pixels, uint32_t &width, uint32_t &height, int &channels, std::string &err);
hipError_t lbvh_build(const BuildInputs &in, Lbvh &out, hipStream_t s, bool node_boxes = true);
hipError_t wide_build(Lbvh &l, uint32_t T, hipStream_t s, bool on_host = false);
hipError_t sah_build(Lbvh &l, uint32_t T, hipStream_t s);
hipError_t sah_build_device(Lbvh &l, uint32_t T, hipStream_t s);
void launch_emit_nodes(Lbvh &l, uint32_t T, hipStream_t s);
void build_prewarm(hipStream_t s);
void wide_prewarm(hipStream_t s); void refit_prewarm(hipStream_t s);
void sah_prewarm(hipStream_t s);
struct RefitArgs {
    uint32_t T, n_wide, n_prims;
    const uint32_t *sub_nodes, *sub_leaves, *sub_off; uint32_t sub_batches, sub_levels;
    DevShadeTri *shade; const DevPrim *prims_host; DevPrim *prims_dev; const uint8_t *touched;
    const uint32_t *leaf_parent, *node_parent; uint32_t *mark;
    DevTri *tris; DevNode4 *wide; DevNodeW *widef; double *acc, *result;
    const uint32_t *dirty; uint32_t n_dirty;
    double *batch_cost;
    bool fold;
};
constexpr uint8_t kTouchRegather = 2u;
constexpr uint32_t kFoldRequantNodes = 400000;
void launch_refit(const RefitArgs &r, hipStream_t s);
void launch_ingest_verts(const void *src, uint32_t stride_bytes, float *slot, uint32_t n_verts, hipStream_t s);
void launch_wide_parents(uint32_t n_wide, const DevNodeW *widef, uint32_t *leaf_parent, uint32_t *node_parent, hipStream_t s);
hipError_t refit_lists_build(Lbvh &l, uint32_t T, hipStream_t s);
void launch_wide_cost(uint32_t n_wide, const DevNodeW *widef, DevNode4 *wide , double *acc, double *result, hipStream_t s);
hipError_t binary_refit(Lbvh &l, uint32_t T, const DevTri *tris, hipStream_t s);
struct TraceTune { uint32_t chunk, refill, blocks, leaf_batch; };
hipError_t lbvh_claim_trav(Lbvh &l, uint32_t NI);

template <int MB> __host__ __device__ inline uint32_t pack_ufloat(float f) {
    uint32_t u;
#ifdef __HIP_DEVICE_COMPILE__
    u = __float_as_uint(f);
#else
    std::memcpy(&u, &f, 4);
#endif
    uint32_t e8 = (u >> 23) & 255u, m = u & 0x7FFFFFu;
    if (e8 == 255u && m) return (31u << MB) | 1u;
    if (u >> 31) return 0;
    if (e8 == 255u) return 31u << MB;
    int e = (int)e8 - 127 + 15;
    if (e >= 31) return 31u << MB;
    int shift = 23 - MB;
    uint32_t full = m | (e8 ? 0x800000u : 0u);
    if (e <= 0) { shift += 1 - e; e = 0; if (shift > 31) return 0; } else full &= 0x7FFFFFu;
    uint32_t q = full >> shift, rem = full & ((1u << shift) - 1u), half = 1u << (shift - 1);
    if (rem > half || (rem == half && (q & 1u))) q++;
    uint32_t out = ((uint32_t)e << MB) + q;
    return out > (31u << MB) ? (31u << MB) : out;
}
template <int MB> __device__ inline float unpack_ufloat(uint32_t v) {
    uint32_t e = v >> MB, m = v & ((1u << MB) - 1u);
    if (e == 31u) return m ? __uint_as_float(0x7FC00000u) : __uint_as_float(0x7F800000u);
    if (e == 0) return ldexpf((float)m, -14 - MB);
    return ldexpf((float)(m | (1u << MB)), (int)e - 15 - MB);
}
__device__ inline uint32_t pack_b10g11r11(float r, float g, float b) { return pack_ufloat<6>(r) | (pack_ufloat<6>(g) << 11) | (pack_ufloat<5>(b) << 22); }

struct FrameArgs {
    CameraArg cam;
    uint32_t W, H;
    const uint32_t *tile_list; uint32_t n_tiles_owned; uint32_t tiles_x;
    uint32_t n_local;
    const uint32_t *block_order;
    const DevNode *nodes; const DevNode4 *wide; const DevNodeW *widef; const DevTri *tris; const DevShadeTri *shade_tris; const DevPrim *prims; const uint32_t *tex_pool;
    bool packet_wide;
    bool pipelined;
    int trace_kind[3];
    TraceTune tune;
    ArtLight lights[kMaxLights]; uint32_t n_lights;
    const ArtLight *lights_more;
    uint32_t *pix_more;
    float4 *hits;
    float4 *contrib;
    float4 *shadow_rays;
    uint32_t *counters;
    float4 *color; float *depth; float4 *normal;
    float4 *color_tiles;
    bool tiles_packed;
    uint32_t *shadow_bits;
    uint32_t *pix_bits;
    bool keep_hits;
    const uint2 *wave_items; uint32_t n_wave_items;
    const uint32_t *tile_xy;
    uint32_t *wave_cost;
    uint32_t batch; uint32_t tiles_stride; CameraArg cam_more[3];
    bool alpha; const uint32_t *alpha_bits;
    uint32_t *hints; uint32_t hint_leaves;
    uint32_t ray_masks;
    bool plain_math;
};
constexpr uint32_t kRayMasksAll = 0xFFFFFFu;
constexpr uint32_t kHintLights = 4;
constexpr uint32_t kHintEmpty = 0xFFFFFFFFu;
constexpr uint32_t kMaxBatch = 4;
void launch_primary(const FrameArgs &a, hipStream_t s);
void launch_shade(const FrameArgs &a, hipStream_t s);
void launch_shadow(const FrameArgs &a, hipStream_t s);
void launch_accumulate(const FrameArgs &a, hipStream_t s);
bool launch_frame(const FrameArgs &a, hipStream_t s);
void launch_frame_stats(const FrameArgs &a, uint32_t *out, hipStream_t s);
void launch_math_sweep(uint32_t which, uint32_t first_bits, uint64_t count, uint32_t stride, unsigned long long *out, hipStream_t s);
void math_sweep_guard(float guard[2]);
void launch_radiance_sweep(uint32_t which, uint32_t first_bits, uint64_t count, uint32_t stride, float numer, unsigned long long *out, hipStream_t s);
struct PlanArgs {
    const uint2 *items_in; uint32_t n_items_in; const uint32_t *cost;
    uint8_t *level, *level_tmp; uint32_t n64;
    uint32_t *worst;
    const uint32_t *order; uint32_t n256;
    uint2 *items_out; uint32_t cap;
    float share; uint32_t min_steps, fixed_steps;
    uint32_t *result;
};
void launch_plan(const PlanArgs &p, hipStream_t s);
constexpr uint32_t kAoTableEntriesPerSample = 64 * 64;
void launch_ao_table(uint32_t spp, float4 *tab, hipStream_t s);
void launch_ao(const FrameArgs &f, uint32_t spp, float radius, uint8_t *occl, float4 *pix, const float4 *tab, bool entry_search, uint32_t *ao, const uint32_t *lut, hipStream_t s);
struct QueryArgs {
    const DevNode4 *wide; const DevTri *tris;
    const uint32_t *tri_prim, *first_tri;
    uint32_t n; float4 *tuv; int2 *ids;
    uint32_t *cursors;
    TraceTune tune;
    bool filter;
    const uint32_t *alpha_bits; const DevShadeTri *shade; const DevPrim *prims; const uint32_t *tex_pool;
    uint32_t cull;
};
constexpr uint32_t kCastCursorWords = 8 * 32;
enum class CastKind { Closest, Any, Multi, Sweep, Crossings };
struct CastArgs : QueryArgs { const float4 *rays; CastKind kind; uint8_t *hit; uint32_t max_hits; uint8_t *count; float radius; float4 *point; uint2 *cross; };
void launch_cast(const CastArgs &c, hipStream_t s);
struct ClosestArgs : QueryArgs { const float4 *points; float4 *point; };
void launch_closest(const ClosestArgs &c, hipStream_t s);
struct ClosestMultiArgs : ClosestArgs { uint32_t max_hits; uint8_t *count; const uint32_t *gid_leaf; };
void launch_closest_multi(const ClosestMultiArgs &c, hipStream_t s);
struct OverlapArgs : QueryArgs { const float4 *boxes; bool any; uint8_t *hit; uint32_t *count; uint32_t max_hits; };
void launch_overlap(const OverlapArgs &c, hipStream_t s);
struct TriOverlapArgs : OverlapArgs { const float4 *qtris; };
void launch_tri_overlap(const TriOverlapArgs &c, hipStream_t s);
struct TriDistanceArgs : ClosestArgs { const float4 *qtris; float4 *qpoint; };
void launch_tri_distance(const TriDistanceArgs &c, hipStream_t s);
struct ResolveArgs {
    const float4 *tuv; const int2 *ids; uint32_t n;
    uint32_t n_prims, T;
    const DevPrim *prims; const DevShadeTri *shade; const uint32_t *gid_leaf; const uint32_t *tex_pool;
    float4 *pos, *ng, *ns; float2 *uv; float4 *albedo, *orm;
};
void launch_resolve(const ResolveArgs &r, hipStream_t s);
void launch_alpha_bits(uint32_t T, const uint32_t *leaf_gid, const uint32_t *tri_prim, const DevPrim *prims, uint32_t *bits, hipStream_t s);
constexpr uint32_t kCounterWords = 8192;
constexpr uint32_t kHitSlots = 1024, kShadowSlots = 1024 + 64 * 32, kSlotStride = 32, kSlotCount = 64;
void lpm_control_block(bool shoulder, float soft_gap, float hdr_max, float exposure, float contrast, float shoulder_contrast, const float saturation[3],
                       const float crosstalk[3], uint32_t ctl[96]);
void launch_present(uint32_t n, const float4 *color, const float4 *normal, const float *depth, const uint32_t *ao, const uint32_t ctl[96], uint32_t *pcolor,
                    uint32_t *pnormal, uint16_t *pdepth, uint32_t *bgra, hipStream_t s);
void launch_untile_packed(const uint32_t *gathered, const uint32_t *tile_slot, uint32_t shard_stride, uint32_t n_frames, uint32_t frame_stride, uint32_t W, uint32_t H, uint32_t *frame, hipStream_t s);
void launch_untile(const float4 *gathered, const uint32_t *tile_slot, uint32_t shard_stride, uint32_t n_frames, uint32_t frame_stride, uint32_t W, uint32_t H, float4 *frame, hipStream_t s);

inline std::vector<uint8_t> shard_owner_table(uint32_t tiles_x, uint32_t tiles_y, uint32_t count, uint32_t relief) {
    std::vector<uint8_t> owner((size_t)tiles_x * tiles_y, 0);
    if (count <= 1) return owner;
    uint32_t relieved = 0;
    auto spread = [](uint32_t v) { v &= 0xFFFFu; v = (v | (v << 8)) & 0x00FF00FFu; v = (v | (v << 4)) & 0x0F0F0F0Fu; v = (v | (v << 2)) & 0x33333333u; v = (v | (v << 1)) & 0x55555555u; return v; };
    std::vector<std::pair<uint32_t, uint32_t>> order;
    order.reserve(owner.size());
    for (uint32_t ty = 0; ty < tiles_y; ty++) for (uint32_t tx = 0; tx < tiles_x; tx++) order.push_back({spread(tx) | (spread(ty) << 1), ty * tiles_x + tx});
    std::sort(order.begin(), order.end());
    std::vector<uint32_t> perm(count);
    for (size_t g = 0; g * count < order.size(); g++) {
        uint32_t state = (uint32_t)g * 2654435761u + 0x9E3779B9u;
        for (uint32_t i = 0; i < count; i++) perm[i] = i;
        for (uint32_t i = count - 1; i > 0; i--) { state = state * 1664525u + 1013904223u; uint32_t j = (state >> 8) % (i + 1); std::swap(perm[i], perm[j]); }
        const bool relieve = relief && ((((uint32_t)g * 2246822519u) >> 24) < relief);
        for (uint32_t i = 0; i < count && g * count + i < order.size(); i++) {
            uint32_t o = perm[i];
            if (relieve && o == 0) o = 1 + (relieved++ % (count - 1));
            owner[order[g * count + i].second] = (uint8_t)o;
        }
    }
    return owner;
}

}
```

### araytracingjourney_amd/csrc/art_shade.h

```cpp
#pragma once
#include "art_device.h"

namespace art {

__device__ inline V3 compute_barycentric(V3 a, V3 b, V3 c, V3 p) {
    V3 v0 = b - a, v1 = c - a, v2 = p - a;
    float d00 = dot3(v0, v0), d01 = dot3(v0, v1), d11 = dot3(v1, v1), d20 = dot3(v2, v0), d21 = dot3(v2, v1);
    float denom = d00 * d11 - d01 * d01;
    V3 r;
    r.x = (d11 * d20 - d01 * d21) / denom;
    r.y = (d00 * d21 - d01 * d20) / denom;
    r.z = 1.0f - r.x - r.y;
    return r;
}
__device__ inline V3 closest_point_to_segment(V3 p0, V3 p1, V3 p) {
    V3 v01 = p1 - p0;
    float t = dot3(p - p0, v01) / dot3(v01, v01);
    t = clampf(t, 0.0f, 1.0f);
    return p0 + v01 * t;
}
__device__ inline V3 closest_point_to_triangle(V3 p0, V3 p1, V3 p2, V3 pt) {
    V3 b = compute_barycentric(p0, p1, p2, pt);
    if (b.x < 0.0f) return closest_point_to_segment(p2, p0, pt);
    else if (b.z < 0.0f) return closest_point_to_segment(p1, p2, pt);
    return pt;
}
__device__ inline V3 get_unnormalized_L_vec(const ArtLight &l, V3 pos) {
    if (l.type == 0u || l.type == 1u) return ld3(l.pos) - pos;
    if (l.type == 2u) return neg(ld3(l.dir)) * 10.0f;
    if (l.type == 3u) {
        V3 ldir = ld3(l.dir), lp = ld3(l.pos), p2 = ld3(l.area_pos2), p3 = ld3(l.area_pos3);
        float distance = dot3(ldir, p2) - dot3(ldir, pos);
        V3 cp = pos + ldir * distance;
        V3 b = compute_barycentric(lp, p2, p3, cp);
        V3 c;
        if (b.x < 0.0f) { V3 p4 = (lp - p2) + p3; c = closest_point_to_triangle(lp, p3, p4, cp); }
        else if (b.y < 0.0f) c = closest_point_to_segment(lp, p2, cp);
        else if (b.z < 0.0f) c = closest_point_to_segment(p2, p3, cp);
        else c = cp;
        return c - pos;
    }
    return mk(1.0f, 1.0f, 1.0f);
}
template <bool FAST> __device__ inline V3 get_light_radiance(const ArtLight &l, V3 pos, V3 L, bool plain) {
    V3 rad = ld3(l.color);
    if (l.type == 1u || l.type == 3u) {
        float theta_s = acosf(clampf(dot3(ld3(l.dir), neg(L)), -1.0f, 1.0f));
        float t = clampf((theta_s - l.umbra_angle) / (l.penumbra_angle - l.umbra_angle), 0.0f, 1.0f);
        rad = rad * (t * t);
    }
    if (l.falloff_distance > 0.0f) {
        float q = __fdividef(len3<FAST>(ld3(l.pos) - pos, plain), l.falloff_distance);
        float w = fmaxf(1.0f - q * q, 0.0f);
        rad = rad * (w * w);
    }
    return rad;
}

#define ART_INV_PI (1.0f / 3.14159265359f)
__device__ __forceinline__ float D_GGX(float a_, float NdotH) {
    float om = 1.0f - NdotH * NdotH;
    float a = NdotH * a_;
    float k = __fdividef(a_, om + a * a);
    return k * k * ART_INV_PI;
}
__device__ __forceinline__ float V_SmithGGXCorrelated_fast(float a_, float NdotV, float NdotL) {
    return __fdividef(0.5f, mixf(2.0f * NdotL * NdotV, NdotL + NdotV, a_));
}
__device__ __forceinline__ float pow5(float x) { float x2 = x * x; return x2 * x2 * x; }
__device__ __forceinline__ float F_Schlick1(float F0, float F90, float x) { return F0 + (F90 - F0) * pow5(1.0f - x); }
__device__ inline float Burley_diffuse_local_sss(float a_, float NdotV, float nc_NdotV, float nc_NdotL, float LdotH, float ratio) {
    float F_SS90 = a_ * LdotH * LdotH;
    float F_SS = F_Schlick1(1.0f, F_SS90, nc_NdotL) * F_Schlick1(1.0f, F_SS90, nc_NdotV);
    float f_ss = (__fdividef(1.0f, nc_NdotV * nc_NdotL) - 0.5f) * F_SS + 0.5f;
    float local_sss = 1.25f * ratio * f_ss;
    float f90 = 0.5f + 2.0f * F_SS90;
    float diffuse = (1.0f - ratio) * F_Schlick1(1.0f, f90, nc_NdotL) * F_Schlick1(1.0f, f90, nc_NdotV);
    return NdotV * (diffuse + local_sss) * ART_INV_PI;
}
constexpr uint32_t kPow22UnderflowBits = 0x1d9aa2a3u;
__device__ __forceinline__ float pow22_texel(float x) {
    x = x < __uint_as_float(kPow22UnderflowBits) ? 0.0f : x;
    const float fe = (float)__builtin_amdgcn_frexp_expf(x), m = __builtin_amdgcn_frexp_mantf(x);
    const float n = rintf(2.2f * fe), f = fmaf(2.2f, fe, -n);
    const float g = fmaf(2.2f, __builtin_amdgcn_logf(m), f);
    return __builtin_amdgcn_ldexpf(__builtin_amdgcn_exp2f(g), (int)n);
}

struct Surface { V3 world_pos, N, Vv, albedo; float metallic, alpha, nc_NdotV, NdotV; };

template <bool CORE, bool HOLD = false> __device__ __forceinline__ void shade_surface_body(const FrameArgs &a, const CameraArg &cam, uint32_t pos, float hu, float hv, Surface &S, float &out_depth, V3 &out_normal, uint32_t &far) {
    const float4 *sq = reinterpret_cast<const float4 *>(a.shade_tris + pos);
    float4 s0 = sq[0], s1 = sq[1], s2 = sq[2], s3 = sq[3], s4 = sq[4], s5 = sq[5], s6 = sq[6], s7 = sq[7], s8 = sq[8];
    const DevPrim &P = a.prims[__float_as_uint(s8.z)];
    float bx = 1.0f - hu - hv, by = hu, bz = hv;
    V3 posv = (mk(s0.x, s0.y, s0.z) * bx + mk(s0.w, s1.x, s1.y) * by) + mk(s1.z, s1.w, s2.x) * bz;
    V3 world_pos = xform_point(P.o2w, posv);
    float tu = (s2.y * bx + s2.w * by) + s3.y * bz, tv = (s2.z * bx + s3.x * by) + s3.z * bz;
    V3 nrm = nrm3_noting<CORE>((mk(s3.w, s4.x, s4.y) * bx + mk(s4.z, s4.w, s5.x) * by) + mk(s5.y, s5.z, s5.w) * bz, far);
    const float *Wm = P.w2o;
    V3 world_normal = nrm3_noting<CORE>(mk(dot3(nrm, mk(Wm[0], Wm[4], Wm[8])), dot3(nrm, mk(Wm[1], Wm[5], Wm[9])), dot3(nrm, mk(Wm[2], Wm[6], Wm[10]))), far);
    V3 tan = nrm3_noting<CORE>((mk(s6.x, s6.y, s6.z) * bx + mk(s6.w, s7.x, s7.y) * by) + mk(s7.z, s7.w, s8.x) * bz, far);
    V3 world_tangent = nrm3_noting<CORE>(xform_vec(P.o2w, tan), far);
    world_tangent = nrm3_noting<CORE>(world_tangent - world_normal * dot3(world_tangent, world_normal), far);
    V3 world_binormal = cross3(world_normal, world_tangent) * s8.y;
    float4 tx = sample_tex(a.tex_pool, P, 2, tu, tv);
    V3 N = nrm3_noting<CORE>(mk(tx.x * 2.0f - 1.0f, tx.y * 2.0f - 1.0f, tx.z * 2.0f - 1.0f), far);
    N = nrm3_noting<CORE>((world_tangent * N.x + world_binormal * N.y) + world_normal * N.z, far);
    tx = sample_tex(a.tex_pool, P, 0, tu, tv);
    V3 albedo = mk(pow22_texel(tx.x), pow22_texel(tx.y), pow22_texel(tx.z));
    tx = sample_tex(a.tex_pool, P, 1, tu, tv);
    float roughness = tx.y, metallic = tx.z;
    S.world_pos = world_pos; S.N = N; S.albedo = albedo; S.metallic = metallic;
    S.Vv = nrm3_noting<CORE>(ld3(cam.camera_pos) - world_pos, far);
    S.alpha = roughness * roughness;
    S.nc_NdotV = dot3(N, S.Vv);
    S.NdotV = clampf(S.nc_NdotV, 1e-5f, 1.0f);
    V3 vp = mat4_mul(cam.view, world_pos.x, world_pos.y, world_pos.z, 1.0f);
    out_depth = -vp.z;
    const float *VI = cam.view_inv;
    V3 on = mk((VI[0] * N.x + VI[1] * N.y) + VI[2] * N.z, (VI[4] * N.x + VI[5] * N.y) + VI[6] * N.z, (VI[8] * N.x + VI[9] * N.y) + VI[10] * N.z);
    on.y = -on.y; on.z = -on.z;
    on = nrm3_noting<CORE>(on, far);
    out_normal = mk(on.x * 0.5f + 0.5f, on.y * 0.5f + 0.5f, on.z * 0.5f + 0.5f);
    if (HOLD) { asm volatile("" : "+{v60}"(out_normal.x)); }
}

template <bool FAST, bool HOLD = false> __device__ __forceinline__ void shade_surface(const FrameArgs &a, const CameraArg &cam, uint32_t pos, float hu, float hv, Surface &S, float &out_depth, V3 &out_normal) {
    uint32_t far = 0u;
    if (FAST) { if (!a.plain_math) { shade_surface_body<true>(a, cam, pos, hu, hv, S, out_depth, out_normal, far); if (exact_noted_in_range(far)) return; } }
    shade_surface_body<false, HOLD>(a, cam, pos, hu, hv, S, out_depth, out_normal, far);
}
template <bool FAST> __device__ __forceinline__ bool shade_light(const ArtLight &l, const Surface &S, bool plain, float4 &c4, float4 &ro, float4 &rd) {
    const bool directional = l.type == 2u;
    V3 nn_L = directional ? mk(0.f, 0.f, 0.f) : get_unnormalized_L_vec(l, S.world_pos);
    V3 L = directional ? ld3(l.area_pos2) : nrm3<FAST>(nn_L, plain);
    V3 Hh = nrm3<FAST>(S.Vv + L, plain);
    float nc_NdotL = dot3(S.N, L);
    float NdotL = clampf(nc_NdotL, 0.0f, 1.0f);
    float NdotH = clampf(dot3(S.N, Hh), 0.0f, 1.0f);
    float LdotH = clampf(dot3(L, Hh), 0.0f, 1.0f);
    float sch = pow5(1.0f - LdotH);
    V3 F0 = mk(mixf(0.04f, S.albedo.x, S.metallic), mixf(0.04f, S.albedo.y, S.metallic), mixf(0.04f, S.albedo.z, S.metallic));
    V3 Ks = mk(F0.x + (1.0f - F0.x) * sch, F0.y + (1.0f - F0.y) * sch, F0.z + (1.0f - F0.z) * sch);
    V3 Kd = S.albedo * (1.0f - S.metallic);
    float DG = D_GGX(S.alpha, NdotH) * V_SmithGGXCorrelated_fast(S.alpha, S.NdotV, NdotL);
    V3 rho_s = Ks * DG;
    V3 rho_d = Kd * Burley_diffuse_local_sss(S.alpha, S.NdotV, S.nc_NdotV, nc_NdotL, LdotH, 0.4f);
    V3 rad = get_light_radiance<FAST>(l, S.world_pos, L, plain);
    V3 c = (rho_s + rho_d) * rad;
    c4 = make_float4(c.x, c.y, c.z, NdotL);
    if (l.casts_shadows && nc_NdotL > 0.0f) {
        ro = make_float4(S.world_pos.x, S.world_pos.y, S.world_pos.z, directional ? l.penumbra_angle : len3<FAST>(nn_L, plain));
        rd = make_float4(L.x, L.y, L.z, 0.f);
        return true;
    }
    return false;
}

__device__ __forceinline__ ArtLight frame_light(const FrameArgs &a, uint32_t i) {
    ArtLight L;
#ifdef __HIP_DEVICE_COMPILE__
    typedef __attribute__((address_space(4))) const uint32_t *Words;
    const Words args = (Words)((__attribute__((address_space(4))) const char *)__builtin_amdgcn_kernarg_segment_ptr() + offsetof(FrameArgs, lights));
    const Words p = i < (uint32_t)kMaxLights ? args + i * (uint32_t)(sizeof(ArtLight) / 4) : (Words)(uintptr_t)(a.lights_more + (i - (uint32_t)kMaxLights));
    uint32_t w[sizeof(ArtLight) / 4];
#pragma unroll
    for (uint32_t k = 0; k < sizeof(ArtLight) / 4; k++) w[k] = p[k];
    __builtin_memcpy(&L, w, sizeof(ArtLight));
#else
    L = a.lights[i < (uint32_t)kMaxLights ? i : 0];
#endif
    return L;
}

}
```

### araytracingjourney_amd/csrc/art_sweeps.hip

```cpp
#include "art_shade.h"

namespace art {

__device__ __attribute__((noinline)) float plain_inv_sqrt(float x) { return 1.0f / sqrtf(x); }
__device__ __attribute__((noinline)) float plain_sqrt(float x) { return sqrtf(x); }
__device__ __forceinline__ float inv_sqrt_short(float x) {
    float y = __builtin_amdgcn_rsqf(x);
    float s = x * y, h = 0.5f * y;
    s = fmaf(s, fmaf(-h, s, 0.5f), s);
    s = fmaf(fmaf(-s, s, x), h, s);
    float q = __builtin_amdgcn_rcpf(s);
    return fmaf(fmaf(-s, q, 1.0f), q, q);
}
constexpr uint32_t kSweepBlocks = 4096;
template <int WHICH> __global__ __launch_bounds__(kBlock) void k_math_sweep(uint32_t first_bits, uint64_t count, uint32_t stride, unsigned long long *__restrict__ out) {
    unsigned long long bad = 0, fast_n = 0, bad_at = ~0ull;
    const uint64_t step = (uint64_t)gridDim.x * kBlock;
    for (uint64_t base = (uint64_t)blockIdx.x * kBlock + (threadIdx.x & ~63u); base < count; base += step) {
        const uint64_t i = base + (threadIdx.x & 63u);
        if (i < count) {
            const float x = __uint_as_float(first_bits + (uint32_t)i * stride);
            bool fast = false;
            float got, ref;
            if (WHICH == 0) { got = inv_sqrt_exact(x, false, fast); ref = plain_inv_sqrt(x); }
            else if (WHICH == 1) { got = sqrt_exact(x, false, fast); ref = plain_sqrt(x); }
            else if (WHICH == 2) {
                uint32_t far = 0u;
                got = inv_sqrt_noting(x, far);
                fast = exact_noted_in_range(far);
                if (!fast) got = 1.0f / sqrtf(x);
                ref = plain_inv_sqrt(x);
            } else if (WHICH == 3) { fast = exact_in_range(x, false); got = fast ? inv_sqrt_short(x) : 1.0f / sqrtf(x); ref = plain_inv_sqrt(x); }
            else { fast = exact_in_range(x, false); got = fast ? __builtin_amdgcn_rsqf(x) : 1.0f / sqrtf(x); ref = plain_inv_sqrt(x); }
            if (__float_as_uint(got) != __float_as_uint(ref)) { bad++; if (i < bad_at) bad_at = i; }
            fast_n += fast ? 1u : 0u;
        }
    }
    for (int off = 32; off >= 1; off >>= 1) {
        bad += __shfl_xor(bad, off); fast_n += __shfl_xor(fast_n, off);
        const unsigned long long o = __shfl_xor(bad_at, off); bad_at = o < bad_at ? o : bad_at;
    }
    if ((threadIdx.x & 63u) == 0) {
        if (bad) { atomicAdd(&out[0], bad); atomicMin(&out[1], bad_at); }
        if (fast_n) atomicAdd(&out[2], fast_n);
    }
}
void launch_math_sweep(uint32_t which, uint32_t first_bits, uint64_t count, uint32_t stride, unsigned long long *out, hipStream_t s) {
    const uint32_t blocks = (uint32_t)std::min<uint64_t>(kSweepBlocks, (count + kBlock - 1) / kBlock);
    if (!blocks) return;
    if (which == 0) k_math_sweep<0><<<blocks, kBlock, 0, s>>>(first_bits, count, stride, out);
    else if (which == 1) k_math_sweep<1><<<blocks, kBlock, 0, s>>>(first_bits, count, stride, out);
    else if (which == 2) k_math_sweep<2><<<blocks, kBlock, 0, s>>>(first_bits, count, stride, out);
    else if (which == 3) k_math_sweep<3><<<blocks, kBlock, 0, s>>>(first_bits, count, stride, out);
    else k_math_sweep<4><<<blocks, kBlock, 0, s>>>(first_bits, count, stride, out);
}
void math_sweep_guard(float guard[2]) { guard[0] = kExactLo; guard[1] = kExactHi; }

__device__ __attribute__((noinline)) float plain_pow22(float x) { return __ocml_pow_f32(x, 2.2f); }
__device__ __attribute__((noinline)) float plain_quotient(float a, float b) { return a / b; }
__device__ __forceinline__ float quotient_rcp(float a, float b) { return a * __builtin_amdgcn_rcpf(b); }
__device__ __forceinline__ uint32_t float_class(float v) { return v != v ? 3u : (fabsf(v) == INFINITY ? 2u : (v == 0.0f ? 0u : 1u)); }
__device__ __forceinline__ long long float_order(float v) { const uint32_t b = __float_as_uint(v); return (b & 0x80000000u) ? -(long long)(b & 0x7fffffffu) : (long long)b; }
constexpr float kRadianceSweepFloor = 0x1p-100f;
template <int WHICH> __global__ __launch_bounds__(kBlock) void k_radiance_sweep(uint32_t first_bits, uint64_t count, uint32_t stride, float numer, unsigned long long *__restrict__ out) {
    unsigned long long worst = 0, class_bad = 0, class_at = ~0ull;
    const uint64_t step = (uint64_t)gridDim.x * kBlock;
    for (uint64_t i = (uint64_t)blockIdx.x * kBlock + threadIdx.x; i < count; i += step) {
        const float x = __uint_as_float(first_bits + (uint32_t)i * stride);
        const float got = WHICH == 0 ? pow22_texel(x) : quotient_rcp(numer, x), ref = WHICH == 0 ? plain_pow22(x) : plain_quotient(numer, x);
        const uint32_t cg = float_class(got), cr = float_class(ref);
        if (cg != cr) { class_bad++; if (i < class_at) class_at = i; }
        else if (cr <= 1u && fabsf(ref) >= kRadianceSweepFloor) {
            long long d = float_order(got) - float_order(ref); d = d < 0 ? -d : d; d = d > 0xffffffffll ? 0xffffffffll : d;
            const unsigned long long w = ((unsigned long long)d << 32) | (uint32_t)i;
            worst = w > worst ? w : worst;
        }
    }
    for (int off = 32; off >= 1; off >>= 1) {
        class_bad += __shfl_xor(class_bad, off);
        const unsigned long long w = __shfl_xor(worst, off); worst = w > worst ? w : worst;
        const unsigned long long o = __shfl_xor(class_at, off); class_at = o < class_at ? o : class_at;
    }
    if ((threadIdx.x & 63u) == 0) {
        if (worst) atomicMax(&out[0], worst);
        if (class_bad) { atomicAdd(&out[1], class_bad); atomicMin(&out[2], class_at); }
    }
}
void launch_radiance_sweep(uint32_t which, uint32_t first_bits, uint64_t count, uint32_t stride, float numer, unsigned long long *out, hipStream_t s) {
    const uint32_t blocks = (uint32_t)std::min<uint64_t>(kSweepBlocks, (count + kBlock - 1) / kBlock);
    if (!blocks) return;
    if (which == 0) k_radiance_sweep<0><<<blocks, kBlock, 0, s>>>(first_bits, count, stride, numer, out);
    else k_radiance_sweep<1><<<blocks, kBlock, 0, s>>>(first_bits, count, stride, numer, out);
}

}
```

### araytracingjourney_amd/renderer.py

```python
from __future__ import annotations

import ctypes as C
import math
import os

import numpy as np

from . import _lib
from ._lib import ArtCamera, ArtConfig, ArtLight, ArtStats, check


def _f3(v):
    return (C.c_float * 3)(*[float(x) for x in v])


def _ptr(a):
    return a.ctypes.data_as(C.c_void_p) if a is not None else None


class PointLight:
    def __init__(self, pos, color, falloff_distance, casts_shadows):
        self.pos, self.color, self.falloff_distance, self.casts_shadows = tuple(pos), tuple(color), float(falloff_distance), bool(casts_shadows)

    def get_light_shader_data(self) -> ArtLight:
# ... 302 lines not shown
        self.extent = (w, h)
        self._device = device
        self.shard = shard
        self.packed_tiles = packed_tiles
        self._camera = Camera((0.0, 0.0, 0.0), (0.0, 0.0, 1.0), w / h, math.pi / 2, 0.1, 1000.0)
        self._lights = Lights()
        self._models = []

    def close(self):
        if getattr(self, "_ctx", None):
            self._L.art_destroy(self._ctx)
            self._ctx = None

    def __del__(self):
        try:
            self.close()
        except Exception:
            pass

    def add_model(self, primitives, model_matrix=None):
        ids = []
        for p in primitives:
            verts = np.ascontiguousarray(p.verts, dtype=np.float32)
            idx = np.ascontiguousarray(p.indices)
            if idx.dtype not in (np.uint16, np.uint32):
                raise TypeError("indices must be uint16 or uint32")
            tex = np.ascontiguousarray(p.tex, dtype=np.uint8)
            m = np.ascontiguousarray(model_matrix if model_matrix is not None else p.model, dtype=np.float32)
            pid = C.c_uint32()
            check(self._L.art_scene_add_primitive(self._ctx, _ptr(verts), verts.shape[0], _ptr(idx), idx.size, idx.dtype.itemsize, _ptr(tex),
                                                  tex.shape[2], tex.shape[1], _ptr(m), C.byref(pid)))
            ids.append(pid.value)
        positions = [np.asarray(p.verts)[:, :3] for p in primitives]
        sp = _positions_sphere(positions)
        mm = model_matrix if model_matrix is not None else primitives[0].model
        self._models.append(Model(ids, sp.transform(mm), renderer=self, model_matrix=mm, object_sphere=sp, positions=positions))
        return ids

    def add_model_glb(self, reader, model_matrix, alpha_mask=False):
        first, n = C.c_uint32(), C.c_uint32()
        m = np.ascontiguousarray(model_matrix, dtype=np.float32)
        r = self._L.art_scene_add_glb(self._ctx, reader._h, _ptr(m), C.byref(first), C.byref(n))
        if r != 0:
            raise _lib.ArtError(r, self._L.art_glb_last_error().decode("utf-8", "replace"))
        ids = list(range(first.value, first.value + n.value))
        c, rad = reader.get_primitives_bounding_sphere()
        from .model_reader import VERTICES
        data, infos = reader.copy_model_data_to_ptr(VERTICES, 0)
        positions = [data[i.mesh_buffer_offset:i.mesh_buffer_offset + i.mesh_size].view(np.float32).reshape(-1, 3) for i in infos]
        model = Model(ids, Sphere(c, rad).transform(model_matrix), renderer=self, model_matrix=model_matrix, object_sphere=Sphere(c, rad), positions=positions)
        self._models.append(model)
        if alpha_mask:
            for i in range(len(ids)):
                mode, cutoff, has_alpha = reader.primitive_alpha(i)
                if mode == 1 and has_alpha:
                    model.set_alpha_cutoff(i, min(max(cutoff, 0.0), 1.0))
        return ids

    def models_mut(self):
        return self._models

    def camera_mut(self) -> Camera:
        return self._camera

    def lights_mut(self) -> Lights:
        return self._lights

    def prepare_first_frame(self):
        self.update_models_status(build=False)
        check(self._L.art_scene_build(self._ctx))

    def update_models_status(self, build=True):
        changed = False
        for m in self._models:
            m.update_model_status(self._camera.pos())
            m.reset_command_buffer_submission_status()
            if (m.state == DEVICE) != m._instanced:
                m._instanced = m.state == DEVICE
                for pid in m.primitive_ids:
                    check(self._L.art_scene_set_primitive_enabled(self._ctx, pid, 1 if m._instanced else 0))
                changed = True
        rebuilt = False
        if changed and build and self.needs_build():
            check(self._L.art_scene_build(self._ctx))
            rebuilt = True
        return rebuilt

    def needs_build(self) -> bool:
        nb = self._L.art_scene_needs_build(self._ctx)
        if nb < 0:
            check(nb)
        return bool(nb)

    def set_stream(self, hip_stream_ptr):
        check(self._L.art_set_stream(self._ctx, C.c_void_p(hip_stream_ptr)))

    def resize(self, extent):
        check(self._L.art_resize(self._ctx, extent[0], extent[1]))
        self.extent = tuple(extent)
        self._camera.set_aspect(extent[0] / extent[1])

    def upload_state(self):
        check(self._L.art_set_camera(self._ctx, C.byref(self._camera.update_host_buffer())))
        arr, n = self._lights.copy_lights_shader_data()
        check(self._L.art_set_lights(self._ctx, arr, n))

    def trace(self):
        check(self._L.art_trace(self._ctx))

    def trace_ao(self, spp=16, radius=0.2 * 1.457):
        check(self._L.art_trace_ao(self._ctx, spp, radius))

    def read_ao(self):
        w, h = self.extent
        a = np.empty((h, w), np.uint32)
        check(self._L.art_read_ao(self._ctx, _ptr(a), a.nbytes))
        return a

    def present(self):
        check(self._L.art_present(self._ctx))

    def read_present(self):
        w, h = self.extent
        a = np.empty((h, w, 4), np.uint8)
        check(self._L.art_read_present(self._ctx, _ptr(a), a.nbytes))
        return a

    def read_packed(self):
        w, h = self.extent
        c, n, d = np.empty((h, w), np.uint32), np.empty((h, w), np.uint32), np.empty((h, w), np.uint16)
        check(self._L.art_read_packed(self._ctx, _ptr(c), _ptr(n), _ptr(d)))
        return c, n, d

    def render_frame(self, sync=True):
        self.update_models_status()
        self.upload_state()
        self.trace()
        if sync:
            self.sync()

    def sync(self):
        check(self._L.art_sync(self._ctx))

    def read_color(self):
        w, h = self.extent
        a = np.empty((h, w, 4), np.float32)
        check(self._L.art_read_color(self._ctx, _ptr(a), a.nbytes))
        return a

    def read_depth(self):
        w, h = self.extent
        a = np.empty((h, w), np.float32)
        check(self._L.art_read_depth(self._ctx, _ptr(a), a.nbytes))
        return a

    def read_normal(self):
        w, h = self.extent
        a = np.empty((h, w, 4), np.float32)
        check(self._L.art_read_normal(self._ctx, _ptr(a), a.nbytes))
        return a

    def device_color(self):
        p, n = C.c_void_p(), C.c_size_t()
        check(self._L.art_device_color(self._ctx, C.byref(p), C.byref(n)))
        return p.value, n.value

    def _dev(self, which):
        p, n = C.c_void_p(), C.c_size_t()
        check(getattr(self._L, "art_device_" + which)(self._ctx, C.byref(p), C.byref(n)))
        return p.value, n.value

    def device_color_tiles(self):
        p, n = C.c_void_p(), C.c_size_t()
        check(self._L.art_device_color_tiles(self._ctx, C.byref(p), C.byref(n)))
        return p.value, n.value

    def bind_color_tiles(self, slot, dev_ptr, nbytes):
        check(self._L.art_bind_color_tiles(self._ctx, slot, C.c_void_p(dev_ptr) if dev_ptr else None, nbytes))

    def bind_color_tiles_pair(self, slot, dev_even, dev_odd, nbytes):
        check(self._L.art_bind_color_tiles_pair(self._ctx, slot, C.c_void_p(dev_even), C.c_void_p(dev_odd), nbytes))

    def bind_color_tiles_ring(self, slot, dev_ptrs, nbytes):
        arr = (C.c_void_p * len(dev_ptrs))(*dev_ptrs)
        check(self._L.art_bind_color_tiles_ring(self._ctx, slot, arr, len(dev_ptrs), nbytes))

    def set_graph_mode(self, on):
        check(self._L.art_set_graph_mode(self._ctx, int(bool(on))))

    def set_frames_per_launch(self, n):
        check(self._L.art_set_frames_per_launch(self._ctx, n))
        self.frames_per_launch = n

    def set_camera_batch(self, cameras):
        arr = (ArtCamera * len(cameras))()
        for i, cam in enumerate(cameras):
            C.memmove(C.byref(arr[i]), C.byref(cam.update_host_buffer()), C.sizeof(ArtCamera))
        check(self._L.art_set_camera_batch(self._ctx, arr, len(cameras)))

    def set_read_frame(self, b):
        check(self._L.art_set_read_frame(self._ctx, b))

    def frames_done(self, first, count):
        d = C.c_int32()
        check(self._L.art_frames_done(self._ctx, first, count, C.byref(d), None))
        return bool(d.value)

    def frames_traced(self):
        d, n = C.c_int32(), C.c_uint64()
        check(self._L.art_frames_done(self._ctx, 0, 0, C.byref(d), C.byref(n)))
        return n.value

    def frames_in_flight(self):
        f, nxt = C.c_uint32(), C.c_uint32()
        check(self._L.art_frames_in_flight(self._ctx, C.byref(f), C.byref(nxt)))
        return f.value, nxt.value

    def stream_wait_frame(self, hip_stream_ptr):
        check(self._L.art_stream_wait_frame(self._ctx, C.c_void_p(hip_stream_ptr)))

    def trace_for_stream(self, hip_stream_ptr):
        k = C.c_uint32()
        check(self._L.art_trace_for_stream(self._ctx, C.c_void_p(hip_stream_ptr), C.byref(k)))
        return k.value

    def wait_external_event(self, hip_event_ptr):
        check(self._L.art_wait_external_event(self._ctx, C.c_void_p(hip_event_ptr)))

    def layout(self) -> dict:
        lay = _lib.ArtLayout()
        check(self._L.art_get_layout(self._ctx, C.byref(lay)))
        return {n: getattr(lay, n) for n, _ in lay._fields_ if n != "reserved"}

    def timestamp_mark(self, which):
        check(self._L.art_timestamp_mark(self._ctx, which))

    def timestamp_elapsed_ms(self):
        ms = C.c_float()
        check(self._L.art_timestamp_elapsed(self._ctx, C.byref(ms)))
        return ms.value

    def collect_timings(self):
        sums = (C.c_float * 5)()
        n = C.c_uint32()
        check(self._L.art_collect_timings(self._ctx, sums, C.byref(n)))
        names = ("primary_ms", "shade_ms", "shadow_ms", "accumulate_ms", "frame_ms")
        k = max(1, n.value)
        return {nm: sums[i] / k for i, nm in enumerate(names)}, n.value

    def read_color_tiles(self):
        _, padded = self.shard_tile_count()
        a = np.empty((padded, 32, 32), np.uint32) if self.packed_tiles else np.empty((padded, 32, 32, 3), np.float32)
        check(self._L.art_read_color_tiles(self._ctx, _ptr(a), a.nbytes))
        return a

    def shard_tile_count(self):
        o, pd = C.c_uint32(), C.c_uint32()
        check(self._L.art_shard_tile_count(self._ctx, C.byref(o), C.byref(pd)))
        return o.value, pd.value

    def untile_gathered(self, gathered_dev_ptr, shard_count, frame_dev_ptr=None, hip_stream_ptr=None, shard_stride_tiles=None, n_frames=None):
        if n_frames is not None:
            check(self._L.art_untile_gathered_frames(self._ctx, C.c_void_p(gathered_dev_ptr), shard_count, shard_stride_tiles, n_frames,
                                                     C.c_void_p(frame_dev_ptr) if frame_dev_ptr else None, C.c_void_p(hip_stream_ptr) if hip_stream_ptr else None))
            return
        if shard_stride_tiles is not None:
            check(self._L.art_untile_gathered_strided(self._ctx, C.c_void_p(gathered_dev_ptr), shard_count, shard_stride_tiles,
                                                      C.c_void_p(frame_dev_ptr) if frame_dev_ptr else None, C.c_void_p(hip_stream_ptr) if hip_stream_ptr else None))
            return
        check(self._L.art_untile_gathered(self._ctx, C.c_void_p(gathered_dev_ptr), shard_count, C.c_void_p(frame_dev_ptr) if frame_dev_ptr else None,
                                          C.c_void_p(hip_stream_ptr) if hip_stream_ptr else None))

    def stats(self) -> dict:
        st = ArtStats()
        check(self._L.art_get_stats(self._ctx, C.byref(st)))
        return st.as_dict()

    def read_hits(self):
        w, h = self.extent
        tuv = np.empty((h, w, 4), np.float32)
        ids = np.empty((h, w, 2), np.int32)
        check(self._L.art_read_hits(self._ctx, _ptr(tuv), _ptr(ids), w * h))
        return tuv, ids

    def read_shadow_bits(self):
        w, h = self.extent
        b = np.empty((h, w), np.uint32)
        check(self._L.art_read_shadow_bits(self._ctx, _ptr(b), w * h))
        return b

    def read_shadow_hints(self):
        a = np.empty((self.layout()["tiles_owned"] * 16, 4, 4), np.uint32)
        check(self._L.art_read_shadow_hints(self._ctx, _ptr(a), a.size))
        return a

    def write_shadow_hints(self, table):
        a = np.ascontiguousarray(table, dtype=np.uint32)
        check(self._L.art_write_shadow_hints(self._ctx, _ptr(a), a.size))

    def math_sweep(self, which, first_bits=0, count=1 << 32, stride=1):
        bad, fast, first, guard = C.c_uint64(0), C.c_uint64(0), C.c_uint32(0), (C.c_float * 2)()
        check(self._L.art_parity_math_sweep(self._ctx, which, first_bits, count, stride, C.byref(bad), C.byref(first), C.byref(fast), guard))
        return dict(mismatches=bad.value, first_bad_bits=first.value if bad.value else None, fast_lanes=fast.value, guard=(guard[0], guard[1]))

    def radiance_sweep(self, which, first_bits=0, count=1 << 32, stride=1, numerator=1.0):
        ulps, worst, bad, first = C.c_uint32(0), C.c_uint32(0), C.c_uint64(0), C.c_uint32(0)
        check(self._L.art_parity_radiance_sweep(self._ctx, which, first_bits, count, stride, numerator, C.byref(ulps), C.byref(worst), C.byref(bad), C.byref(first)))
        return dict(max_ulps=ulps.value, worst_bits=worst.value if ulps.value else None, class_mismatches=bad.value, first_class_bits=first.value if bad.value else None)

    @staticmethod
    def live_resources():
        out = (C.c_uint64 * 5)()
        check(_lib.load().art_parity_live_resources(out))
        return dict(zip(("device", "pinned", "events", "streams", "pooled"), (int(v) for v in out)))

    PLAN_UNWRITTEN = 0xFFFFFFFF

    def parity_plan(self, order, items_in, cost, level_in, worst_in, cap, share, min_steps, fixed_steps, result_in=None):
        order, cost, worst_in = (np.ascontiguousarray(a, np.uint32) for a in (order, cost, worst_in))
        items_in, level_in = np.ascontiguousarray(items_in, np.uint32).reshape(-1, 2), np.ascontiguousarray(level_in, np.uint8)
        n256 = order.size
        if level_in.size != 4 * n256 or worst_in.size != 4 * n256 or cost.size != items_in.shape[0]:
            raise ValueError("parity_plan: level_in and worst_in hold 4 * len(order) entries, cost one per item")
        items_out, level_out, worst_out = np.zeros((max(int(cap), 1), 2), np.uint32), np.zeros(4 * n256, np.uint8), np.zeros(4 * n256, np.uint32)
        result = np.zeros(8, np.uint32) if result_in is None else np.array(result_in, np.uint32)
        assert result.size == 8
        check(self._L.art_parity_plan(self._ctx, n256, _ptr(order), _ptr(items_in), items_in.shape[0], _ptr(cost), _ptr(level_in), _ptr(worst_in), int(cap), float(share),
                                      int(min_steps), int(fixed_steps), _ptr(items_out), _ptr(level_out), _ptr(worst_out), _ptr(result)))
        return items_out, level_out, worst_out, result

    def read_wave_plan(self):
        n, state, result = C.c_uint32(), (C.c_uint32 * 4)(), np.zeros(8, np.uint32)
        check(self._L.art_read_wave_plan(self._ctx, None, 0, None, 0, C.byref(n), None, state))
        level, items = np.zeros(self.layout()["tiles_owned"] * 16, np.uint8), np.zeros((n.value, 2), np.uint32)
        check(self._L.art_read_wave_plan(self._ctx, _ptr(level), level.size, _ptr(items), n.value, C.byref(n), _ptr(result), state))
        assert n.value == items.shape[0]
        return dict(level=level, items=items, result=result, cur=state[0], pending=bool(state[1]), replans=state[2], cap=state[3])

    def sample_wave_steps(self):
        cap = self.layout()["tiles_owned"] * 16 * 2 + 64
        items, steps, n = np.zeros((cap, 2), np.uint32), np.zeros(cap, np.uint32), C.c_uint32()
        check(self._L.art_sample_wave_steps(self._ctx, _ptr(items), _ptr(steps), cap, C.byref(n)))
        assert n.value <= cap
        return items[:n.value].copy(), steps[:n.value].copy()

    def set_ray_masks(self, primary=0xFF, shadow=0xFF, ao=0xFF):
        p, s, a = _mask_value("primary", primary), _mask_value("shadow", shadow), _mask_value("ao", ao)
        check(self._L.art_set_ray_masks(self._ctx, p, s, a))

    _RECORDS = (("tuv", "float32", (4,), 16), ("ids", "int32", (2,), 8))
    _POINT = ("point", "float32", (4,), 16)
    _RESOLVE_OUTPUTS = dict(pos=4, ng=4, ns=4, uv=2, albedo=4, orm=4)

    def _query_device(self):
        if self._device < 0:
            import torch
            self._device = torch.cuda.current_device()
        return self._device

    def _on_device(self, t, dtype, align):
        import torch
        return isinstance(t, torch.Tensor) and t.is_cuda and t.device.index == self._query_device() and t.dtype == getattr(torch, dtype) and t.is_contiguous() and \
            t.data_ptr() % align == 0

    def _dev_tensor(self, t, name, dtype, tail_shape, align, n=None, exact=False):
        import torch
        dev = self._query_device()
        if self._on_device(t, dtype, align) and (tuple(t.shape) == tail_shape if exact else
                                                 t.dim() == 1 + len(tail_shape) and tuple(t.shape[1:]) == tail_shape and (n is None or t.shape[0] >= n)):
            return t
        if exact:
            raise ValueError(f"out: {name} must be a contiguous {dtype} tensor on cuda:{dev} of shape {tail_shape}, {align}-byte aligned")
        if n is not None:
            shape = "".join(f", {w}" for w in tail_shape) + ("," if len(tail_shape) != 1 else "")
            raise ValueError(f"out: {name} must be a contiguous torch.{dtype} tensor on cuda:{dev} of shape (>= n{shape}), {align}-byte aligned")
        if not (isinstance(t, torch.Tensor) and t.is_cuda and t.device.index == dev):
            raise ValueError(f"{name} must be a torch tensor on cuda:{dev}")
        raise ValueError(f"{name} must be {dtype} of shape (n, {tail_shape[0]}), contiguous and {align}-byte aligned")

    def _outputs(self, out, n, device, specs):
        import torch
        if out is None:
            return tuple(torch.empty((n,) + tail, dtype=getattr(torch, dtype), device=device) for _, dtype, tail, _ in specs)
        return tuple(self._dev_tensor(t, name, dtype, tail, align, n) for t, (name, dtype, tail, align) in zip(out, specs, strict=True))

    @staticmethod
    def _stream_handle(stream, device):
        if stream is None:
            import torch
            stream = torch.cuda.current_stream(device)
        return int(getattr(stream, "cuda_stream", stream)) or 1

    def cast_rays(self, rays, kind="closest", cull_mask=0xFF, out=None, stream=None):
        m = _mask_value("cull_mask", cull_mask)
        if kind not in ("closest", "any"):
            raise ValueError("kind must be 'closest' or 'any'")
        n = self._dev_tensor(rays, "rays", "float32", (8,), 16).shape[0]
        d = _lib.ArtRayCast(rays_dev=rays.data_ptr() or None, n=n, cull_mask=m, flags=0)
        if kind == "closest":
            res = tuv, ids = self._outputs(out, n, rays.device, self._RECORDS)
            d.kind, d.tuv_dev, d.ids_dev = _lib.ART_CAST_CLOSEST, tuv.data_ptr() or None, ids.data_ptr() or None
        else:
            res, = self._outputs(None if out is None else (out,), n, rays.device, (("hit", "uint8", (), 1),))
            d.kind, d.hit_dev = _lib.ART_CAST_ANY, res.data_ptr() or None
        d.hip_stream = self._stream_handle(stream, rays.device)
        check(self._L.art_cast_rays(self._ctx, C.byref(d)))
        return res

    def cast_rays_multi(self, rays, max_hits, cull_mask=0xFF, out=None, stream=None):
        m = _mask_value("cull_mask", cull_mask)
        k = int(max_hits)
        if k != max_hits or not 1 <= k <= _lib.ART_CAST_MAX_HITS:
            raise ValueError(f"max_hits must be an integer in 1..{_lib.ART_CAST_MAX_HITS}")
        n = self._dev_tensor(rays, "rays", "float32", (8,), 16).shape[0]
        tuv, ids, count = self._outputs(out, n, rays.device, (("tuv", "float32", (k, 4), 16), ("ids", "int32", (k, 2), 8), ("count", "uint8", (), 1)))
        d = _lib.ArtRayCastMulti(rays_dev=rays.data_ptr() or None, tuv_dev=tuv.data_ptr() or None, ids_dev=ids.data_ptr() or None, count_dev=count.data_ptr() or None,
                                 n=n, max_hits=k, cull_mask=m, flags=0, hip_stream=self._stream_handle(stream, rays.device))
        check(self._L.art_cast_rays_multi(self._ctx, C.byref(d)))
        return tuv, ids, count

    def resolve_hits(self, tuv, ids, want=("pos", "ng", "ns", "uv", "albedo", "orm"), out=None, stream=None):
        import torch
        dev = self._query_device()
        want = tuple(want)
        if not want or len(set(want)) != len(want) or any(w not in self._RESOLVE_OUTPUTS for w in want):
            raise ValueError(f"want must name one or more of {tuple(self._RESOLVE_OUTPUTS)}, each once")
        for t, (name, dtype, (width,), align) in zip((tuv, ids), self._RECORDS):
            if not (self._on_device(t, dtype, align) and t.dim() in (2, 3) and t.shape[-1] == width):
                raise ValueError(f"{name} must be a contiguous torch.{dtype} tensor on cuda:{dev} of shape (n, {width}) or (n, K, {width}), {align}-byte aligned")
        lead = tuple(tuv.shape[:-1])
        if tuple(ids.shape[:-1]) != lead:
            raise ValueError("tuv and ids must hold the same records")
        res = {}
        for name in want:
            width = self._RESOLVE_OUTPUTS[name]
            t = out[name] if out is not None and name in out else torch.empty(lead + (width,), dtype=torch.float32, device=tuv.device)
            res[name] = self._dev_tensor(t, name, "float32", lead + (width,), 4 * width, exact=True)
        d = _lib.ArtHitResolve(tuv_dev=tuv.data_ptr() or None, ids_dev=ids.data_ptr() or None, n=tuv.numel() // 4, flags=0, hip_stream=self._stream_handle(stream, tuv.device))
        for name, t in res.items():
            setattr(d, name + "_dev", t.data_ptr() or None)
        check(self._L.art_resolve_hits(self._ctx, C.byref(d)))
        return res

    def cast_surface(self, rays, cull_mask=0xFF, want=("pos", "ng", "ns", "uv", "albedo", "orm"), stream=None):
        tuv, ids = self.cast_rays(rays, "closest", cull_mask, stream=stream)
        return (tuv, ids), self.resolve_hits(tuv, ids, want, stream=stream)

    def closest_points(self, points, cull_mask=0xFF, out=None, stream=None):
        m = _mask_value("cull_mask", cull_mask)
        n = self._dev_tensor(points, "points", "float32", (4,), 16).shape[0]
        duv, ids, point = self._outputs(out, n, points.device, (("duv", "float32", (4,), 16), self._RECORDS[1], self._POINT))
        d = _lib.ArtPointQuery(points_dev=points.data_ptr() or None, duv_dev=duv.data_ptr() or None, ids_dev=ids.data_ptr() or None, point_dev=point.data_ptr() or None,
                               n=n, cull_mask=m, flags=0, reserved=0, hip_stream=self._stream_handle(stream, points.device))
        check(self._L.art_closest_points(self._ctx, C.byref(d)))
        return duv, ids, point

    def closest_surface(self, points, cull_mask=0xFF, want=("pos", "ng", "ns", "uv", "albedo", "orm"), stream=None):
        duv, ids, point = self.closest_points(points, cull_mask, stream=stream)
        return (duv, ids, point), self.resolve_hits(duv, ids, want, stream=stream)

    def closest_points_multi(self, points, max_hits, cull_mask=0xFF, out=None, stream=None):
        m = _mask_value("cull_mask", cull_mask)
        k = int(max_hits)
        if k != max_hits or not 1 <= k <= _lib.ART_CAST_MAX_HITS:
            raise ValueError(f"max_hits must be an integer in 1..{_lib.ART_CAST_MAX_HITS}")
        n = self._dev_tensor(points, "points", "float32", (4,), 16).shape[0]
        duv, ids, point, count = self._outputs(out, n, points.device, (("duv", "float32", (k, 4), 16), ("ids", "int32", (k, 2), 8), ("point", "float32", (k, 4), 16),
                                                                       ("count", "uint8", (), 1)))
        d = _lib.ArtPointQueryMulti(points_dev=points.data_ptr() or None, duv_dev=duv.data_ptr() or None, ids_dev=ids.data_ptr() or None, point_dev=point.data_ptr() or None,
                                    count_dev=count.data_ptr() or None, n=n, max_hits=k, cull_mask=m, flags=0, hip_stream=self._stream_handle(stream, points.device))
        check(self._L.art_closest_points_multi(self._ctx, C.byref(d)))
        return duv, ids, point, count

    def closest_surface_multi(self, points, max_hits, cull_mask=0xFF, want=("pos", "ng", "ns", "uv", "albedo", "orm"), stream=None):
        duv, ids, point, count = self.closest_points_multi(points, max_hits, cull_mask, stream=stream)
        return (duv, ids, point, count), self.resolve_hits(duv, ids, want, stream=stream)

    def overlap_boxes(self, boxes, kind="list", max_hits=8, cull_mask=0xFF, out=None, stream=None):
        return self._overlap(self._L.art_overlap_boxes, _lib.ArtBoxQuery, "boxes_dev", boxes, "boxes", 8, kind, max_hits, cull_mask, out, stream)

    def _overlap(self, entry, desc, field, queries, name, width, kind, max_hits, cull_mask, out, stream):
        m = _mask_value("cull_mask", cull_mask)
        if kind not in ("list", "any"):
            raise ValueError("kind must be 'list' or 'any'")
        k = 0
        if kind == "list":
            k = int(max_hits)
            if k != max_hits or not 1 <= k <= _lib.ART_CAST_MAX_HITS:
                raise ValueError(f"max_hits must be an integer in 1..{_lib.ART_CAST_MAX_HITS}")
        n = self._dev_tensor(queries, name, "float32", (width,), 16).shape[0]
        d = desc(n=n, max_hits=k, cull_mask=m, flags=0, reserved=0)
        setattr(d, field, queries.data_ptr() or None)
        if kind == "list":
            res = ids, count = self._outputs(out, n, queries.device, (("ids", "int32", (k, 2), 8), ("count", "int32", (), 4)))
            d.kind, d.ids_dev, d.count_dev = _lib.ART_OVERLAP_LIST, ids.data_ptr() or None, count.data_ptr() or None
        else:
            res, = self._outputs(None if out is None else (out,), n, queries.device, (("hit", "uint8", (), 1),))
            d.kind, d.hit_dev = _lib.ART_OVERLAP_ANY, res.data_ptr() or None
        d.hip_stream = self._stream_handle(stream, queries.device)
        check(entry(self._ctx, C.byref(d)))
        return res

    def overlap_triangles(self, tris, kind="list", max_hits=8, cull_mask=0xFF, out=None, stream=None):
        return self._overlap(self._L.art_overlap_triangles, _lib.ArtTriQuery, "tris_dev", tris, "tris", 12, kind, max_hits, cull_mask, out, stream)

    def collide_mesh(self, positions, indices, model_matrix=None, kind="any", max_hits=8, cull_mask=0xFF, stream=None):
        _mask_value("cull_mask", cull_mask)
        if kind not in ("list", "any"):
            raise ValueError("kind must be 'list' or 'any'")
        import torch
        tris, stream = self._mesh_tris(positions, indices, model_matrix, stream)
        with torch.cuda.stream(stream):
            return self.overlap_triangles(tris, kind, max_hits, cull_mask, stream=stream)

    def closest_triangles(self, tris, cull_mask=0xFF, out=None, stream=None):
        m = _mask_value("cull_mask", cull_mask)
        n = self._dev_tensor(tris, "tris", "float32", (12,), 16).shape[0]
        duv, ids, point, qpoint = self._outputs(out, n, tris.device, (("duv", "float32", (4,), 16), self._RECORDS[1], self._POINT, ("qpoint", "float32", (4,), 16)))
        d = _lib.ArtTriDistance(tris_dev=tris.data_ptr() or None, duv_dev=duv.data_ptr() or None, ids_dev=ids.data_ptr() or None, point_dev=point.data_ptr() or None,
                                qpoint_dev=qpoint.data_ptr() or None, n=n, cull_mask=m, flags=0, reserved=0, hip_stream=self._stream_handle(stream, tris.device))
        check(self._L.art_closest_triangles(self._ctx, C.byref(d)))
        return duv, ids, point, qpoint

    def mesh_clearance(self, positions, indices, model_matrix=None, radius=float("inf"), cull_mask=0xFF, stream=None):
        import torch
        _mask_value("cull_mask", cull_mask)
        radius = float(radius)
        if not radius >= 0.0:
            raise ValueError("radius must be a float >= 0 (inf: unbounded)")
        tris, stream = self._mesh_tris(positions, indices, model_matrix, stream)
        with torch.cuda.stream(stream):
            tris[:, 3] = radius
            duv, ids, point, qpoint = records = self.closest_triangles(tris, cull_mask, stream=stream)
            nt, dev = tris.shape[0], tris.device
            if nt == 0:
                return records, dict(distance=torch.full((), radius, dtype=torch.float32, device=dev), index=torch.full((), -1, dtype=torch.int64, device=dev),
                                     ids=torch.full((2,), -1, dtype=torch.int32, device=dev), point=torch.zeros(4, device=dev), qpoint=torch.zeros(4, device=dev))
            has = ids[:, 0] >= 0
            key = torch.where(has, duv[:, 0], torch.full_like(duv[:, 0], float("inf")))
            at = torch.where(key == key.min(), torch.arange(nt, device=dev), nt).min()
            any_ = has.any()
            at = torch.where(any_, at, torch.zeros_like(at))
            row = at.reshape(1)
            pick = lambda t: t.index_select(0, row)[0]
            return records, dict(distance=pick(duv)[0], index=torch.where(any_, at, torch.full_like(at, -1)), ids=pick(ids), point=pick(point), qpoint=pick(qpoint))

    def _mesh_tris(self, positions, indices, model_matrix, stream):
        import torch
        nv = self._dev_tensor(positions, "positions", "float32", (3,), 4).shape[0]
        dev = positions.device
        if not (isinstance(indices, torch.Tensor) and indices.device == dev and indices.dtype in (torch.int32, torch.int64) and indices.dim() == 2 and indices.shape[1] == 3
                and indices.is_contiguous()):
            raise ValueError(f"indices must be a contiguous int32 or int64 torch tensor on {dev} of shape (T, 3)")
        nt = indices.shape[0]
        if nt > _lib.ART_CAST_MAX_RAYS:
            raise ValueError("indices: more than ART_CAST_MAX_RAYS triangles")
        if nt and not nv:
            raise ValueError("positions: empty, with triangles to gather")
        mm = None
        if model_matrix is not None:
            mm = np.asarray(model_matrix.cpu() if isinstance(model_matrix, torch.Tensor) else model_matrix, np.float32).reshape(-1)
            if mm.size != 12 or not np.isfinite(mm).all():
                raise ValueError("model_matrix must be 12 finite floats, a row-major 3x4")
            mm = [float(x) for x in mm]
        stream = self._torch_stream(stream, dev)
        with torch.cuda.stream(stream):
            tris = torch.zeros((nt, 3, 4), dtype=torch.float32, device=dev)
            if nt:
                idx = indices.to(torch.int64)
                p = positions[idx.clamp(0, nv - 1)]
                if mm is not None:
                    x, y, z = p[..., 0], p[..., 1], p[..., 2]
                    p = torch.stack([((x * mm[4 * r] + y * mm[4 * r + 1]) + z * mm[4 * r + 2]) + mm[4 * r + 3] for r in range(3)], dim=-1)
                outside = ((idx < 0) | (idx >= nv)).any(dim=1)
                tris[..., 0:3] = torch.where(outside[:, None, None], torch.full_like(p, float("nan")), p)
        return tris.reshape(nt, 12), stream

    def voxelize(self, origin, cell, dims, cull_mask=0xFF, stream=None):
        import torch
        m = _mask_value("cull_mask", cull_mask)
        dims = tuple(int(x) for x in dims)
        if len(dims) != 3 or any(x < 0 for x in dims):
            raise ValueError("dims must be three integers >= 0")
        dev = torch.device("cuda", self._query_device())
        org = np.asarray(origin, np.float32).reshape(-1)
        cel = np.asarray(cell, np.float32).reshape(-1)
        if org.size != 3 or cel.size not in (1, 3) or not (np.isfinite(org).all() and np.isfinite(cel).all() and (cel > 0).all()):
            raise ValueError("origin must be three finite floats and cell one or three finite floats > 0")
        cel = np.broadcast_to(cel, (3,))
        n = dims[0] * dims[1] * dims[2]
        if n > _lib.ART_CAST_MAX_RAYS:
            raise ValueError("dims: more than ART_CAST_MAX_RAYS cells")
        if stream is None:
            stream = torch.cuda.current_stream(dev)
        elif not hasattr(stream, "cuda_stream"):
            stream = torch.cuda.ExternalStream(int(stream), device=dev)
        with torch.cuda.stream(stream):
            boxes = torch.zeros(dims + (8,), dtype=torch.float32, device=dev)
            for axis in range(3):
                shape = [1, 1, 1]
                shape[axis] = dims[axis]
                idx = torch.arange(dims[axis] + 1, dtype=torch.float32, device=dev)
                plane = idx * float(cel[axis]) + float(org[axis])
                boxes[..., axis] = plane[:-1].reshape(shape)
                boxes[..., 4 + axis] = plane[1:].reshape(shape)
            hit = self.overlap_boxes(boxes.reshape(n, 8), "any", cull_mask=m, stream=stream)
# ... 240 lines not shown
```

### include/art_parity.h

```cpp
#ifndef ART_PARITY_H
#define ART_PARITY_H
#include "art.h"

#ifdef __cplusplus
extern "C" {
#endif

typedef struct ArtTuning {
    uint32_t frame_form;
    uint32_t tree_builder;
    uint32_t packet_wide;
    uint32_t primary_walk, shadow_walk, ao_walk;
    uint32_t block_order;
    uint32_t fixed_waves;
    uint32_t split_fixed_steps;
    uint32_t split_min_steps;
    float split_alpha;
    uint32_t ao_entry_off;
    uint32_t trace_chunk, trace_refill, trace_blocks;
    uint32_t hw_queues;
    uint32_t log;
    uint32_t wide_builder;
    uint32_t as_versions;
    float refit_rebuild_ratio;
    uint32_t trace_leaf_batch;
    uint32_t plan_moving_interval;
    uint32_t refit_streams;
    uint32_t refit_fold_nodes;
    uint32_t shadow_hints;
    uint32_t plain_math;
} ArtTuning;
int32_t art_set_tuning(ArtContext *ctx, const ArtTuning *tuning);
int32_t art_read_hits(ArtContext *ctx, float *tuv, int32_t *ids, size_t n_pixels);
int32_t art_read_shadow_bits(ArtContext *ctx, uint32_t *bits, size_t n_pixels);
int32_t art_read_shadow_hints(ArtContext *ctx, uint32_t *words, size_t n_words);
int32_t art_write_shadow_hints(ArtContext *ctx, const uint32_t *words, size_t n_words);
int32_t art_query_closest(ArtContext *ctx, const float *rays, uint32_t n, float *tuv, int32_t *ids);
int32_t art_query_any(ArtContext *ctx, const float *rays, uint32_t n, uint8_t *hit);
int32_t art_query_closest_masked(ArtContext *ctx, const float *rays, uint32_t n, uint32_t cull_mask, float *tuv, int32_t *ids);
int32_t art_query_any_masked(ArtContext *ctx, const float *rays, uint32_t n, uint32_t cull_mask, uint8_t *hit);
int32_t art_get_lbvh(ArtContext *ctx, uint32_t *leaf_gid, uint64_t *keys, int32_t *child, float *node_lo,
                     float *node_hi, float *leaf_lo, float *leaf_hi);
int32_t art_get_traversal_tree(ArtContext *ctx, int32_t *child, float *node_lo, float *node_hi);
int32_t art_get_wide_nodes(ArtContext *ctx, void *quantised, void *floats, size_t capacity_nodes, uint32_t *n_nodes);
int32_t art_parity_math_sweep(ArtContext *ctx, uint32_t which, uint32_t first_bits, uint64_t count, uint32_t stride, uint64_t *mismatches, uint32_t *first_bad_bits,
                              uint64_t *fast_lanes, float guard[2]);
int32_t art_parity_radiance_sweep(ArtContext *ctx, uint32_t which, uint32_t first_bits, uint64_t count, uint32_t stride, float numerator, uint32_t *max_ulps, uint32_t *worst_bits,
                                  uint64_t *class_mismatches, uint32_t *first_class_bits);


int32_t art_bind_color_tiles(ArtContext *ctx, uint32_t slot, void *dev_ptr, size_t bytes);
int32_t art_bind_color_tiles_pair(ArtContext *ctx, uint32_t slot, void *dev_even, void *dev_odd, size_t bytes);
int32_t art_bind_color_tiles_ring(ArtContext *ctx, uint32_t slot, void *const *bufs, uint32_t n, size_t bytes);
int32_t art_read_color_tiles(ArtContext *ctx, void *dst, size_t bytes);
int32_t art_untile_gathered_strided(ArtContext *ctx, const void *gathered_dev, uint32_t shard_count, uint32_t shard_stride_tiles, void *frame_dev, void *hip_stream);
int32_t art_untile_gathered_frames(ArtContext *ctx, const void *gathered_dev, uint32_t shard_count, uint32_t shard_stride_tiles, uint32_t n_frames, void *frames_dev, void *hip_stream);

int32_t art_stream_wait_frame(ArtContext *ctx, void *hip_stream);
int32_t art_trace_for_stream(ArtContext *ctx, void *hip_stream, uint32_t *slot_used);
int32_t art_wait_external_event(ArtContext *ctx, void *hip_event);


int32_t art_set_graph_mode(ArtContext *ctx, int32_t on);
int32_t art_timestamp_mark(ArtContext *ctx, uint32_t which);
int32_t art_timestamp_elapsed(ArtContext *ctx, float *ms);

int32_t art_collect_timings(ArtContext *ctx, float sums_ms[5], uint32_t *n_frames);
int32_t art_sample_wave_steps(ArtContext *ctx, uint32_t *items, uint32_t *steps, uint32_t cap, uint32_t *n);
int32_t art_parity_plan(ArtContext *ctx, uint32_t n256, const uint32_t *order, const uint32_t *items_in, uint32_t n_items_in, const uint32_t *cost, const uint8_t *level_in,
                        const uint32_t *worst_in, uint32_t cap, float share, uint32_t min_steps, uint32_t fixed_steps, uint32_t *items_out, uint8_t *level_out,
                        uint32_t *worst_out, uint32_t result[8]);
int32_t art_read_wave_plan(ArtContext *ctx, uint8_t *level, size_t n64, uint32_t *items, uint32_t cap, uint32_t *n_items, uint32_t result[8], uint32_t state[4]);
int32_t art_parity_live_resources(uint64_t out[5]);
int32_t art_vertex_update_counts(ArtContext *ctx, uint64_t *ingests, uint64_t *host_syncs, uint64_t *readbacks);


int32_t art_mgpu_pending(ArtMgpu *mg, uint32_t *groups_queued, uint32_t *launches_open);

#ifdef __cplusplus
}
#endif
#endif
```

Measured before the change: 23540 Mray/s.

## Use shorter exact-rounding divide, inverse-sqrt and wrap paths in frame kernel

```diff
diff --git a/araytracingjourney_amd/_abi.py b/araytracingjourney_amd/_abi.py
--- a/araytracingjourney_amd/_abi.py
+++ b/araytracingjourney_amd/_abi.py
@@ -419,6 +419,7 @@
     "art_get_traversal_tree": (C.c_int32, [C.c_void_p, C.c_void_p, C.c_void_p, C.c_void_p]),
     "art_get_wide_nodes": (C.c_int32, [C.c_void_p, C.c_void_p, C.c_void_p, C.c_size_t, C.c_void_p]),
     "art_parity_math_sweep": (C.c_int32, [C.c_void_p, C.c_uint32, C.c_uint32, C.c_uint64, C.c_uint32, C.c_void_p, C.c_void_p, C.c_void_p, C.c_void_p]),
+    "art_parity_div_sweep": (C.c_int32, [C.c_void_p, C.c_uint32, C.c_uint32, C.c_uint64, C.c_uint32, C.c_uint32, C.c_void_p, C.c_void_p, C.c_void_p, C.c_void_p, C.c_void_p]),
     "art_parity_radiance_sweep": (C.c_int32, [C.c_void_p, C.c_uint32, C.c_uint32, C.c_uint64, C.c_uint32, C.c_float, C.c_void_p, C.c_void_p, C.c_void_p, C.c_void_p]),
     "art_bind_color_tiles": (C.c_int32, [C.c_void_p, C.c_uint32, C.c_void_p, C.c_size_t]),
     "art_bind_color_tiles_pair": (C.c_int32, [C.c_void_p, C.c_uint32, C.c_void_p, C.c_void_p, C.c_size_t]),
diff --git a/araytracingjourney_amd/csrc/art_api.hip b/araytracingjourney_amd/csrc/art_api.hip
--- a/araytracingjourney_amd/csrc/art_api.hip
+++ b/araytracingjourney_amd/csrc/art_api.hip
@@ -980,6 +980,28 @@
     return ART_OK;
 }
 
+int32_t art_parity_div_sweep(ArtContext *c, uint32_t which, uint32_t first_bits, uint64_t count, uint32_t stride, uint32_t numerator_bits, uint64_t *mismatches, uint32_t first_bad[2],
+                             uint64_t *short_lanes, uint64_t *lanes, float guard[4]) {
+    if (!c || !mismatches || !first_bad || !short_lanes || !lanes || !guard) return fail(ART_E_INVALID, "art_parity_div_sweep: null argument");
+    if (which > 4 || count > (1ull << 32)) return fail(ART_E_INVALID, "art_parity_div_sweep: which 0..4, at most 2^32 patterns");
+    int32_t r = use_device(c); if (r) return r;
+    r = sync_all(c); if (r) return r;
+    div_sweep_guard(guard);
+    unsigned long long h[4] = {0ull, ~0ull, 0ull, 0ull};
+    DevBuf<unsigned long long> d;
+    HIPC(d.ensure(4));
+    HIPC(hipMemcpy(d.p, h, sizeof h, hipMemcpyHostToDevice));
+    launch_div_sweep(which, first_bits, count, stride, numerator_bits, d.p, nullptr); HIPC(hipGetLastError());
+    HIPC(hipMemcpy(h, d.p, sizeof h, hipMemcpyDeviceToHost));
+    *mismatches = h[0]; *short_lanes = h[2]; *lanes = h[3];
+    if (h[0]) {
+        const uint32_t j = first_bits + (uint32_t)h[1] * stride;
+        first_bad[0] = numerator_bits; first_bad[1] = j;
+        if (which >= 3) div_sweep_pair(which, j, numerator_bits, first_bad[0], first_bad[1]);
+    }
+    return ART_OK;
+}
+
 int32_t art_parity_radiance_sweep(ArtContext *c, uint32_t which, uint32_t first_bits, uint64_t count, uint32_t stride, float numerator, uint32_t *max_ulps, uint32_t *worst_bits,
                                   uint64_t *class_mismatches, uint32_t *first_class_bits) {
     if (!c || !max_ulps || !worst_bits || !class_mismatches || !first_class_bits) return fail(ART_E_INVALID, "art_parity_radiance_sweep: null argument");
diff --git a/araytracingjourney_amd/csrc/art_device.h b/araytracingjourney_amd/csrc/art_device.h
--- a/araytracingjourney_amd/csrc/art_device.h
+++ b/araytracingjourney_amd/csrc/art_device.h
@@ -28,12 +28,29 @@
     float q = fmaf(fmaf(-d, r, 1.0f), r, r);
     return fmaf(fmaf(-d, q, 1.0f), r, q);
 }
+__device__ __forceinline__ float inv_sqrt_short(float x) {
+    float y = __builtin_amdgcn_rsqf(x);
+    float s = x * y, h = 0.5f * y;
+    s = fmaf(s, fmaf(-h, s, 0.5f), s);
+    s = fmaf(fmaf(-s, s, x), h, s);
+    float q = __builtin_amdgcn_rcpf(s);
+    return fmaf(fmaf(-s, q, 1.0f), q, q);
+}
+constexpr float kDivLo = 0x1p-47f, kDivHi = 0x1p47f;
+__device__ __forceinline__ float div_core(float a, float b) {
+    float r = __builtin_amdgcn_rcpf(b);
+    r = fmaf(fmaf(-b, r, 1.0f), r, r);
+    float q = a * r;
+    q = fmaf(fmaf(-b, q, a), r, q);
+    return fmaf(fmaf(-b, q, a), r, q);
+}
+__device__ __forceinline__ bool div_core_domain(float a, float b) { return fabsf(a) >= kDivLo && fabsf(a) <= kDivHi && fabsf(b) >= kDivLo && fabsf(b) <= kDivHi; }
 __device__ __forceinline__ bool exact_in_range(float x, bool plain) {
     return !plain && __builtin_amdgcn_ballot_w64(!(x >= kExactLo && x <= kExactHi)) == 0ull;
 }
-template <bool FAST = true> __device__ __forceinline__ float inv_sqrt_exact(float x, bool plain, bool &fast) {
+template <bool FAST = true, bool SHORT = false> __device__ __forceinline__ float inv_sqrt_exact(float x, bool plain, bool &fast) {
     fast = FAST && exact_in_range(x, plain);
-    if (fast) return rcp_core(sqrt_core(x));
+    if (fast) return SHORT ? inv_sqrt_short(x) : rcp_core(sqrt_core(x));
     return 1.0f / sqrtf(x);
 }
 template <bool FAST = true> __device__ __forceinline__ float sqrt_exact(float x, bool plain, bool &fast) {
@@ -44,11 +61,11 @@
 __device__ __forceinline__ void exact_note(float x, uint32_t &far) { far = max(far, __float_as_uint(x) - __float_as_uint(kExactLo)); }
 __device__ __forceinline__ bool exact_noted_in_range(uint32_t far) { return __builtin_amdgcn_ballot_w64(far > __float_as_uint(kExactHi) - __float_as_uint(kExactLo)) == 0ull; }
 template <bool FAST = true> __device__ __forceinline__ float len3(V3 a, bool plain = false) { bool f; return sqrt_exact<FAST>(dot3(a, a), plain, f); }
-template <bool FAST = true> __device__ __forceinline__ V3 nrm3(V3 a, bool plain = false) { bool f; float inv = inv_sqrt_exact<FAST>(dot3(a, a), plain, f); return a * inv; }
-__device__ __forceinline__ float inv_sqrt_noting(float x, uint32_t &far) { exact_note(x, far); return rcp_core(sqrt_core(x)); }
-template <bool CORE> __device__ __forceinline__ V3 nrm3_noting(V3 a, uint32_t &far) {
+template <bool FAST = true, bool SHORT = false> __device__ __forceinline__ V3 nrm3(V3 a, bool plain = false) { bool f; float inv = inv_sqrt_exact<FAST, SHORT>(dot3(a, a), plain, f); return a * inv; }
+template <bool SHORT = false> __device__ __forceinline__ float inv_sqrt_noting(float x, uint32_t &far) { exact_note(x, far); return SHORT ? inv_sqrt_short(x) : rcp_core(sqrt_core(x)); }
+template <bool CORE, bool SHORT = false> __device__ __forceinline__ V3 nrm3_noting(V3 a, uint32_t &far) {
     float x = dot3(a, a);
-    return a * (CORE ? inv_sqrt_noting(x, far) : 1.0f / sqrtf(x));
+    return a * (CORE ? inv_sqrt_noting<SHORT>(x, far) : 1.0f / sqrtf(x));
 }
 __device__ __forceinline__ float clampf(float x, float lo, float hi) { return fminf(fmaxf(x, lo), hi); }
 __device__ __forceinline__ float mixf(float x, float y, float a) { return x * (1.0f - a) + y * a; }
@@ -66,14 +83,15 @@
 }
 
 __device__ __forceinline__ int wrapi(int i, int n) { int m = i % n; return m < 0 ? m + n : m; }
-__device__ __forceinline__ void tex_taps(const uint32_t *__restrict__ pool, uint32_t texture_offset, uint32_t tw_, uint32_t th_, int layer, float u, float v,
+template <bool SEL> __device__ __forceinline__ int wrap_next(int i, int n) { return SEL ? (i + 1 == n ? 0 : i + 1) : wrapi(i + 1, n); }
+template <bool SEL = false> __device__ __forceinline__ void tex_taps(const uint32_t *__restrict__ pool, uint32_t texture_offset, uint32_t tw_, uint32_t th_, int layer, float u, float v,
                                          uint32_t &t00, uint32_t &t10, uint32_t &t01, uint32_t &t11, float &fx, float &fy) {
     int tw = (int)tw_, th = (int)th_;
     float x = u * (float)tw - 0.5f, y = v * (float)th - 0.5f;
     float x0f = floorf(x), y0f = floorf(y);
     fx = x - x0f; fy = y - y0f;
     int x0 = wrapi((int)x0f, tw), y0 = wrapi((int)y0f, th);
-    int x1 = wrapi(x0 + 1, tw), y1 = wrapi(y0 + 1, th);
+    int x1 = wrap_next<SEL>(x0, tw), y1 = wrap_next<SEL>(y0, th);
     const uint32_t *base = pool + texture_offset + (size_t)layer * tw * th;
     t00 = base[(size_t)y0 * tw + x0]; t10 = base[(size_t)y0 * tw + x1]; t01 = base[(size_t)y1 * tw + x0]; t11 = base[(size_t)y1 * tw + x1];
 }
@@ -84,13 +102,13 @@
     float top = A * (1.0f - fx) + B * fx, bot = Cc * (1.0f - fx) + D * fx;
     return top * (1.0f - fy) + bot * fy;
 }
-__device__ inline float4 sample_tex(const uint32_t *__restrict__ pool, const DevPrim &P, int layer, float u, float v) {
+template <bool SEL = false> __device__ inline float4 sample_tex(const uint32_t *__restrict__ pool, const DevPrim &P, int layer, float u, float v) {
     int tw = (int)P.tw, th = (int)P.th;
     float x = u * (float)tw - 0.5f, y = v * (float)th - 0.5f;
     float x0f = floorf(x), y0f = floorf(y);
     float fx = x - x0f, fy = y - y0f;
     int x0 = wrapi((int)x0f, tw), y0 = wrapi((int)y0f, th);
-    int x1 = wrapi(x0 + 1, tw), y1 = wrapi(y0 + 1, th);
+    int x1 = wrap_next<SEL>(x0, tw), y1 = wrap_next<SEL>(y0, th);
     const uint32_t *base = pool + P.texture_offset + (size_t)layer * tw * th;
     uint32_t t00 = base[(size_t)y0 * tw + x0], t10 = base[(size_t)y0 * tw + x1], t01 = base[(size_t)y1 * tw + x0], t11 = base[(size_t)y1 * tw + x1];
     float o[4];
@@ -107,11 +125,11 @@
     const uint32_t *tex;
     uint32_t cull;
 };
-__device__ __forceinline__ float alpha_at(const uint32_t *__restrict__ pool, uint32_t texture_offset, uint32_t tw, uint32_t th, float4 s2, float4 s3, float u, float v) {
+template <bool SEL = false> __device__ __forceinline__ float alpha_at(const uint32_t *__restrict__ pool, uint32_t texture_offset, uint32_t tw, uint32_t th, float4 s2, float4 s3, float u, float v) {
     float bx = 1.0f - u - v, by = u, bz = v;
     float tu = (s2.y * bx + s2.w * by) + s3.y * bz, tv = (s2.z * bx + s3.x * by) + s3.z * bz;
     uint32_t t00, t10, t01, t11; float fx, fy;
-    tex_taps(pool, texture_offset, tw, th, 0, tu, tv, t00, t10, t01, t11, fx, fy);
+    tex_taps<SEL>(pool, texture_offset, tw, th, 0, tu, tv, t00, t10, t01, t11, fx, fy);
     return tex_channel(t00, t10, t01, t11, fx, fy, 3);
 }
 __device__ __forceinline__ bool alpha_cut(const AlphaView &av, uint32_t pos, float u, float v) {
diff --git a/araytracingjourney_amd/csrc/art_frame.hip b/araytracingjourney_amd/csrc/art_frame.hip
--- a/araytracingjourney_amd/csrc/art_frame.hip
+++ b/araytracingjourney_amd/csrc/art_frame.hip
@@ -45,7 +45,7 @@
 }
 struct StepUpdate { uint64_t m = 0ull; float t, u, v; uint32_t pos, gid; };
 struct NoUpdate {};
-template <bool ANY, bool WIDE, int OCT, bool COUNT = false, bool ALPHA = false, bool HINTS = false, class ON>
+template <bool ANY, bool WIDE, int OCT, bool COUNT = false, bool ALPHA = false, bool HINTS = false, bool TSEL = false, class ON>
 __device__ __forceinline__ void packet_walk(const FrameArgs &a, const Ray &r, ON &on, int *stk, float &tbest, float &bu, float &bv, uint32_t &bpos, uint32_t &bgid, uint32_t &steps, PacketHints &h) {
     constexpr bool MASKS = std::is_same<ON, uint64_t>::value;
     int cur = HINTS ? h.cur : 0, sp = HINTS ? h.sp : 0;
@@ -138,7 +138,7 @@
                         if (!(c > 0.0f)) return cand;
                         const uint32_t toff = P[offsetof(DevPrim, texture_offset) / 4], tw = P[offsetof(DevPrim, tw) / 4], th = P[offsetof(DevPrim, th) / 4];
                         bool keep = __builtin_amdgcn_inverse_ballot_w64(cand);
-                        if (keep) keep = !(alpha_at(a.tex_pool, toff, tw, th, s2, s3, u, v) < c);
+                        if (keep) keep = !(alpha_at<TSEL>(a.tex_pool, toff, tw, th, s2, s3, u, v) < c);
                         return cand & ballot64(keep);
                     };
                     if (ANY) {
@@ -169,7 +169,7 @@
                         const float c = __uint_as_float(P[offsetof(DevPrim, cutoff) / 4]);
                         if (!(c > 0.0f)) return cand;
                         const uint32_t toff = P[offsetof(DevPrim, texture_offset) / 4], tw = P[offsetof(DevPrim, tw) / 4], th = P[offsetof(DevPrim, th) / 4];
-                        if (cand) cand = !(alpha_at(a.tex_pool, toff, tw, th, s2, s3, u, v) < c);
+                        if (cand) cand = !(alpha_at<TSEL>(a.tex_pool, toff, tw, th, s2, s3, u, v) < c);
                         return cand;
                     };
                     if (ANY) {
@@ -215,7 +215,7 @@
 #endif
 }
 
-template <bool ANY, bool WIDE, bool COUNT = false, bool ALPHA = false, bool HINTS = false, bool MASKS = true>
+template <bool ANY, bool WIDE, bool COUNT = false, bool ALPHA = false, bool HINTS = false, bool MASKS = true, bool TSEL = false>
 __device__ __forceinline__ void walk_dispatch(const FrameArgs &a, const Ray &r, bool alive, int *stk, float &tbest, float &bu, float &bv, uint32_t &bpos, uint32_t &bgid, uint32_t &steps, PacketHints &h) {
     typename std::conditional<MASKS, uint64_t, bool>::type on;
     int oct;
@@ -235,15 +235,15 @@
         oct = !uniform ? 8 : (nx ? 1 : 0) | (ny ? 2 : 0) | (nz ? 4 : 0);
     }
     switch (oct) {
-    case 0: packet_walk<ANY, WIDE, 0, COUNT, ALPHA, HINTS>(a, r, on, stk, tbest, bu, bv, bpos, bgid, steps, h); break;
-    case 1: packet_walk<ANY, WIDE, 1, COUNT, ALPHA, HINTS>(a, r, on, stk, tbest, bu, bv, bpos, bgid, steps, h); break;
-    case 2: packet_walk<ANY, WIDE, 2, COUNT, ALPHA, HINTS>(a, r, on, stk, tbest, bu, bv, bpos, bgid, steps, h); break;
-    case 3: packet_walk<ANY, WIDE, 3, COUNT, ALPHA, HINTS>(a, r, on, stk, tbest, bu, bv, bpos, bgid, steps, h); break;
-    case 4: packet_walk<ANY, WIDE, 4, COUNT, ALPHA, HINTS>(a, r, on, stk, tbest, bu, bv, bpos, bgid, steps, h); break;
-    case 5: packet_walk<ANY, WIDE, 5, COUNT, ALPHA, HINTS>(a, r, on, stk, tbest, bu, bv, bpos, bgid, steps, h); break;
-    case 6: packet_walk<ANY, WIDE, 6, COUNT, ALPHA, HINTS>(a, r, on, stk, tbest, bu, bv, bpos, bgid, steps, h); break;
-    case 7: packet_walk<ANY, WIDE, 7, COUNT, ALPHA, HINTS>(a, r, on, stk, tbest, bu, bv, bpos, bgid, steps, h); break;
-    default: packet_walk<ANY, WIDE, 8, COUNT, ALPHA, HINTS>(a, r, on, stk, tbest, bu, bv, bpos, bgid, steps, h); break;
+    case 0: packet_walk<ANY, WIDE, 0, COUNT, ALPHA, HINTS, TSEL>(a, r, on, stk, tbest, bu, bv, bpos, bgid, steps, h); break;
+    case 1: packet_walk<ANY, WIDE, 1, COUNT, ALPHA, HINTS, TSEL>(a, r, on, stk, tbest, bu, bv, bpos, bgid, steps, h); break;
+    case 2: packet_walk<ANY, WIDE, 2, COUNT, ALPHA, HINTS, TSEL>(a, r, on, stk, tbest, bu, bv, bpos, bgid, steps, h); break;
+    case 3: packet_walk<ANY, WIDE, 3, COUNT, ALPHA, HINTS, TSEL>(a, r, on, stk, tbest, bu, bv, bpos, bgid, steps, h); break;
+    case 4: packet_walk<ANY, WIDE, 4, COUNT, ALPHA, HINTS, TSEL>(a, r, on, stk, tbest, bu, bv, bpos, bgid, steps, h); break;
+    case 5: packet_walk<ANY, WIDE, 5, COUNT, ALPHA, HINTS, TSEL>(a, r, on, stk, tbest, bu, bv, bpos, bgid, steps, h); break;
+    case 6: packet_walk<ANY, WIDE, 6, COUNT, ALPHA, HINTS, TSEL>(a, r, on, stk, tbest, bu, bv, bpos, bgid, steps, h); break;
+    case 7: packet_walk<ANY, WIDE, 7, COUNT, ALPHA, HINTS, TSEL>(a, r, on, stk, tbest, bu, bv, bpos, bgid, steps, h); break;
+    default: packet_walk<ANY, WIDE, 8, COUNT, ALPHA, HINTS, TSEL>(a, r, on, stk, tbest, bu, bv, bpos, bgid, steps, h); break;
     }
 }
 
@@ -276,6 +276,14 @@
 #else
 template <bool WIDE, bool ONE_LIGHT, bool COUNT, bool BATCH, bool ALPHA> constexpr uint32_t kFrameMoves = kFrameMovesTable[WIDE << 4 | ONE_LIGHT << 3 | COUNT << 2 | BATCH << 1 | ALPHA];
 #endif
+constexpr uint16_t kFrameShortTable[32] = {0x1800, 0x3800, 0x1800, 0x1800, 0x1800, 0x3800, 0x1800, 0x3800, 0x1ffb, 0x2800, 0x0800, 0x2800, 0x1e00, 0x2800, 0x0800, 0x2800, 0x1800, 0x3800, 0x1800, 0x3800, 0x1800, 0x3800, 0x1800, 0x3800, 0x1ffb, 0x2800, 0x0800, 0x2800, 0x1ffb, 0x2800, 0x0800, 0x2800};
+#ifdef ART_SHORT_FORCE
+template <bool WIDE, bool ONE_LIGHT, bool COUNT, bool BATCH, bool ALPHA> constexpr uint32_t kFrameShortRaw = ART_SHORT_FORCE;
+#else
+template <bool WIDE, bool ONE_LIGHT, bool COUNT, bool BATCH, bool ALPHA> constexpr uint32_t kFrameShortRaw = kFrameShortTable[WIDE << 4 | ONE_LIGHT << 3 | COUNT << 2 | BATCH << 1 | ALPHA];
+#endif
+template <bool WIDE, bool ONE_LIGHT, bool COUNT, bool BATCH, bool ALPHA> constexpr uint32_t kFrameShort =
+    kFrameShortRaw<WIDE, ONE_LIGHT, COUNT, BATCH, ALPHA> & ((kFrameFastMath<WIDE, ONE_LIGHT, COUNT, BATCH, ALPHA> ? 0x7FFu : 0u) | 0x1800u | (ALPHA ? 0x2000u : 0u));
 __device__ __forceinline__ const FrameArgs &frame_args_again(const FrameArgs &a) {
 #ifdef __HIP_DEVICE_COMPILE__
     __attribute__((address_space(4))) const char *p = (__attribute__((address_space(4))) const char *)__builtin_amdgcn_kernarg_segment_ptr();
@@ -291,6 +299,7 @@
     constexpr bool HINTS = kFrameHints<WIDE, ONE_LIGHT, COUNT, BATCH, ALPHA>;
     constexpr bool FASTM = kFrameFastMath<WIDE, ONE_LIGHT, COUNT, BATCH, ALPHA>;
     constexpr uint32_t MV = kFrameMoves<WIDE, ONE_LIGHT, COUNT, BATCH, ALPHA>;
+    constexpr uint32_t SH = kFrameShort<WIDE, ONE_LIGHT, COUNT, BATCH, ALPHA>;
     int *stk = wstack;
     const uint32_t wid = blockIdx.x;
     if (wid >= a_.n_wave_items) return;
@@ -307,9 +316,9 @@
         uint32_t p, x, y; bool mine;
         in = frame_pixel(a_, wid, p, x, y, mine);
         float fx = (float)x + 0.5f, fy = (float)y + 0.5f;
-        float dx = (fx / (float)a_.W) * 2.0f - 1.0f, dy = (fy / (float)a_.H) * 2.0f - 1.0f;
+        float dx = ((SH & 0x800u) ? div_core(fx, (float)a_.W) : fx / (float)a_.W) * 2.0f - 1.0f, dy = ((SH & 0x800u) ? div_core(fy, (float)a_.H) : fy / (float)a_.H) * 2.0f - 1.0f;
         V3 org = mat4_mul(cam0.view_inv, 0.f, 0.f, 0.f, 1.f);
-        V3 tgt = nrm3<FASTM>(mat4_mul(cam0.proj_inv, dx, dy, 1.f, 1.f), a_.plain_math);
+        V3 tgt = nrm3<FASTM, (SH & 0x200u) != 0u>(mat4_mul(cam0.proj_inv, dx, dy, 1.f, 1.f), a_.plain_math);
         V3 dir = mat4_mul(cam0.view_inv, tgt.x, tgt.y, tgt.z, 0.f);
         ray_init(r, org, dir, 0.001f, 10000.0f);
     }
@@ -317,7 +326,7 @@
     PHASE(0, r.inv.x)
     float tbest = on ? r.tmax : -1.0f, bu = 0.f, bv = 0.f;
     uint32_t bpos = kNoHit, bgid = kNoHit;
-    { PacketHints none{0, 0, 0u}; walk_dispatch<false, WIDE, COUNT, ALPHA, false, (MV & 1u) != 0u>(a_, r, on, stk, tbest, bu, bv, bpos, bgid, steps, none); }
+    { PacketHints none{0, 0, 0u}; walk_dispatch<false, WIDE, COUNT, ALPHA, false, (MV & 1u) != 0u, (SH & 0x2000u) != 0u>(a_, r, on, stk, tbest, bu, bv, bpos, bgid, steps, none); }
     PHASE(1, tbest)
     const FrameArgs &a = (MV & 2u) ? frame_args_again(a_) : a_;
     const FrameArgs &as = (MV & 4u) ? a : a_;
@@ -331,7 +340,7 @@
     Surface S;
     S.world_pos = mk(0.f, 0.f, 0.f); S.N = mk(0.f, 0.f, 1.f); S.Vv = mk(0.f, 0.f, 1.f); S.albedo = mk(0.f, 0.f, 0.f);
     S.metallic = 0.f; S.alpha = 0.f; S.nc_NdotV = 0.f; S.NdotV = 0.f;
-    if (hit) shade_surface<FASTM, ONE_LIGHT && !BATCH && ALPHA>(as, cam, bpos, bu, bv, S, out_depth, out_normal);
+    if (hit) shade_surface<FASTM, ONE_LIGHT && !BATCH && ALPHA, SH & 0x1FFu, (SH & 0x1000u) != 0u>(as, cam, bpos, bu, bv, S, out_depth, out_normal);
     if (in) {
         const size_t pix = frame_px + (size_t)y * a.W + x;
         st_nt(&a.depth[pix], out_depth);
@@ -352,7 +361,7 @@
         float4 c4 = make_float4(0.f, 0.f, 0.f, 0.f), ro = make_float4(0.f, 0.f, 0.f, 1.0f), rd = make_float4(0.f, 0.f, 1.f, 0.f);
         bool want = false;
         const ArtLight L = ONE_LIGHT ? b.lights[0] : frame_light(b, i);
-        if (hit) want = shade_light<FASTM>(L, S, b.plain_math, c4, ro, rd);
+        if (hit) want = shade_light<FASTM, (SH & 0x400u) != 0u>(L, S, b.plain_math, c4, ro, rd);
         if (want) { if (i < 16u) sbits |= 1u << (16u + i); else more++; }
         Ray sr;
         if (L.type == 2u) ray_init_inv(sr, mk(ro.x, ro.y, ro.z), ld3(L.area_pos2), ld3(L.area_pos3), 0.01f, L.penumbra_angle);
@@ -362,7 +371,7 @@
         float st = son ? sr.tmax : -1.0f, su = 0.f, sv = 0.f;
         uint32_t spos = kNoHit, sgid = kNoHit;
         const uint64_t traced = HINTS ? ballot64(son) : 0ull;
-        walk_dispatch<true, WIDE, COUNT, ALPHA, HINTS, (MV & 1u) != 0u>(b, sr, son, stk, st, su, sv, spos, sgid, steps, hn);
+        walk_dispatch<true, WIDE, COUNT, ALPHA, HINTS, (MV & 1u) != 0u, (SH & 0x2000u) != 0u>(b, sr, son, stk, st, su, sv, spos, sgid, steps, hn);
         const FrameArgs &c = (MV & 16u) ? frame_args_again(a_) : a_;
         if (HINTS && c.hints && traced != 0ull) {
             uint32_t o[4];
diff --git a/araytracingjourney_amd/csrc/art_internal.h b/araytracingjourney_amd/csrc/art_internal.h
--- a/araytracingjourney_amd/csrc/art_internal.h
+++ b/araytracingjourney_amd/csrc/art_internal.h
@@ -206,6 +206,9 @@
 void launch_frame_stats(const FrameArgs &a, uint32_t *out, hipStream_t s);
 void launch_math_sweep(uint32_t which, uint32_t first_bits, uint64_t count, uint32_t stride, unsigned long long *out, hipStream_t s);
 void math_sweep_guard(float guard[2]);
+void launch_div_sweep(uint32_t which, uint32_t first_bits, uint64_t count, uint32_t stride, uint32_t numer_bits, unsigned long long *out, hipStream_t s);
+void div_sweep_guard(float guard[4]);
+bool div_sweep_pair(uint32_t which, uint32_t j, uint32_t seed, uint32_t &a, uint32_t &b);
 void launch_radiance_sweep(uint32_t which, uint32_t first_bits, uint64_t count, uint32_t stride, float numer, unsigned long long *out, hipStream_t s);
 struct PlanArgs {
     const uint2 *items_in; uint32_t n_items_in; const uint32_t *cost;
diff --git a/araytracingjourney_amd/csrc/art_shade.h b/araytracingjourney_amd/csrc/art_shade.h
--- a/araytracingjourney_amd/csrc/art_shade.h
+++ b/araytracingjourney_amd/csrc/art_shade.h
@@ -89,7 +89,7 @@
 
 struct Surface { V3 world_pos, N, Vv, albedo; float metallic, alpha, nc_NdotV, NdotV; };
 
-template <bool CORE, bool HOLD = false> __device__ __forceinline__ void shade_surface_body(const FrameArgs &a, const CameraArg &cam, uint32_t pos, float hu, float hv, Surface &S, float &out_depth, V3 &out_normal, uint32_t &far) {
+template <bool CORE, bool HOLD = false, uint32_t SITES = 0u, bool SEL = false> __device__ __forceinline__ void shade_surface_body(const FrameArgs &a, const CameraArg &cam, uint32_t pos, float hu, float hv, Surface &S, float &out_depth, V3 &out_normal, uint32_t &far) {
     const float4 *sq = reinterpret_cast<const float4 *>(a.shade_tris + pos);
     float4 s0 = sq[0], s1 = sq[1], s2 = sq[2], s3 = sq[3], s4 = sq[4], s5 = sq[5], s6 = sq[6], s7 = sq[7], s8 = sq[8];
     const DevPrim &P = a.prims[__float_as_uint(s8.z)];
@@ -97,22 +97,22 @@
     V3 posv = (mk(s0.x, s0.y, s0.z) * bx + mk(s0.w, s1.x, s1.y) * by) + mk(s1.z, s1.w, s2.x) * bz;
     V3 world_pos = xform_point(P.o2w, posv);
     float tu = (s2.y * bx + s2.w * by) + s3.y * bz, tv = (s2.z * bx + s3.x * by) + s3.z * bz;
-    V3 nrm = nrm3_noting<CORE>((mk(s3.w, s4.x, s4.y) * bx + mk(s4.z, s4.w, s5.x) * by) + mk(s5.y, s5.z, s5.w) * bz, far);
+    V3 nrm = nrm3_noting<CORE, (SITES >> 0 & 1u) != 0u>((mk(s3.w, s4.x, s4.y) * bx + mk(s4.z, s4.w, s5.x) * by) + mk(s5.y, s5.z, s5.w) * bz, far);
     const float *Wm = P.w2o;
-    V3 world_normal = nrm3_noting<CORE>(mk(dot3(nrm, mk(Wm[0], Wm[4], Wm[8])), dot3(nrm, mk(Wm[1], Wm[5], Wm[9])), dot3(nrm, mk(Wm[2], Wm[6], Wm[10]))), far);
-    V3 tan = nrm3_noting<CORE>((mk(s6.x, s6.y, s6.z) * bx + mk(s6.w, s7.x, s7.y) * by) + mk(s7.z, s7.w, s8.x) * bz, far);
-    V3 world_tangent = nrm3_noting<CORE>(xform_vec(P.o2w, tan), far);
-    world_tangent = nrm3_noting<CORE>(world_tangent - world_normal * dot3(world_tangent, world_normal), far);
+    V3 world_normal = nrm3_noting<CORE, (SITES >> 1 & 1u) != 0u>(mk(dot3(nrm, mk(Wm[0], Wm[4], Wm[8])), dot3(nrm, mk(Wm[1], Wm[5], Wm[9])), dot3(nrm, mk(Wm[2], Wm[6], Wm[10]))), far);
+    V3 tan = nrm3_noting<CORE, (SITES >> 2 & 1u) != 0u>((mk(s6.x, s6.y, s6.z) * bx + mk(s6.w, s7.x, s7.y) * by) + mk(s7.z, s7.w, s8.x) * bz, far);
+    V3 world_tangent = nrm3_noting<CORE, (SITES >> 3 & 1u) != 0u>(xform_vec(P.o2w, tan), far);
+    world_tangent = nrm3_noting<CORE, (SITES >> 4 & 1u) != 0u>(world_tangent - world_normal * dot3(world_tangent, world_normal), far);
     V3 world_binormal = cross3(world_normal, world_tangent) * s8.y;
-    float4 tx = sample_tex(a.tex_pool, P, 2, tu, tv);
-    V3 N = nrm3_noting<CORE>(mk(tx.x * 2.0f - 1.0f, tx.y * 2.0f - 1.0f, tx.z * 2.0f - 1.0f), far);
-    N = nrm3_noting<CORE>((world_tangent * N.x + world_binormal * N.y) + world_normal * N.z, far);
-    tx = sample_tex(a.tex_pool, P, 0, tu, tv);
+    float4 tx = sample_tex<SEL>(a.tex_pool, P, 2, tu, tv);
+    V3 N = nrm3_noting<CORE, (SITES >> 5 & 1u) != 0u>(mk(tx.x * 2.0f - 1.0f, tx.y * 2.0f - 1.0f, tx.z * 2.0f - 1.0f), far);
+    N = nrm3_noting<CORE, (SITES >> 6 & 1u) != 0u>((world_tangent * N.x + world_binormal * N.y) + world_normal * N.z, far);
+    tx = sample_tex<SEL>(a.tex_pool, P, 0, tu, tv);
     V3 albedo = mk(pow22_texel(tx.x), pow22_texel(tx.y), pow22_texel(tx.z));
-    tx = sample_tex(a.tex_pool, P, 1, tu, tv);
+    tx = sample_tex<SEL>(a.tex_pool, P, 1, tu, tv);
     float roughness = tx.y, metallic = tx.z;
     S.world_pos = world_pos; S.N = N; S.albedo = albedo; S.metallic = metallic;
-    S.Vv = nrm3_noting<CORE>(ld3(cam.camera_pos) - world_pos, far);
+    S.Vv = nrm3_noting<CORE, (SITES >> 7 & 1u) != 0u>(ld3(cam.camera_pos) - world_pos, far);
     S.alpha = roughness * roughness;
     S.nc_NdotV = dot3(N, S.Vv);
     S.NdotV = clampf(S.nc_NdotV, 1e-5f, 1.0f);
@@ -121,21 +121,21 @@
     const float *VI = cam.view_inv;
     V3 on = mk((VI[0] * N.x + VI[1] * N.y) + VI[2] * N.z, (VI[4] * N.x + VI[5] * N.y) + VI[6] * N.z, (VI[8] * N.x + VI[9] * N.y) + VI[10] * N.z);
     on.y = -on.y; on.z = -on.z;
-    on = nrm3_noting<CORE>(on, far);
+    on = nrm3_noting<CORE, (SITES >> 8 & 1u) != 0u>(on, far);
     out_normal = mk(on.x * 0.5f + 0.5f, on.y * 0.5f + 0.5f, on.z * 0.5f + 0.5f);
     if (HOLD) { asm volatile("" : "+{v60}"(out_normal.x)); }
 }
 
-template <bool FAST, bool HOLD = false> __device__ __forceinline__ void shade_surface(const FrameArgs &a, const CameraArg &cam, uint32_t pos, float hu, float hv, Surface &S, float &out_depth, V3 &out_normal) {
+template <bool FAST, bool HOLD = false, uint32_t SITES = 0u, bool SEL = false> __device__ __forceinline__ void shade_surface(const FrameArgs &a, const CameraArg &cam, uint32_t pos, float hu, float hv, Surface &S, float &out_depth, V3 &out_normal) {
     uint32_t far = 0u;
-    if (FAST) { if (!a.plain_math) { shade_surface_body<true>(a, cam, pos, hu, hv, S, out_depth, out_normal, far); if (exact_noted_in_range(far)) return; } }
-    shade_surface_body<false, HOLD>(a, cam, pos, hu, hv, S, out_depth, out_normal, far);
+    if (FAST) { if (!a.plain_math) { shade_surface_body<true, false, SITES, SEL>(a, cam, pos, hu, hv, S, out_depth, out_normal, far); if (exact_noted_in_range(far)) return; } }
+    shade_surface_body<false, HOLD, 0u, SEL>(a, cam, pos, hu, hv, S, out_depth, out_normal, far);
 }
-template <bool FAST> __device__ __forceinline__ bool shade_light(const ArtLight &l, const Surface &S, bool plain, float4 &c4, float4 &ro, float4 &rd) {
+template <bool FAST, bool SHORT = false> __device__ __forceinline__ bool shade_light(const ArtLight &l, const Surface &S, bool plain, float4 &c4, float4 &ro, float4 &rd) {
     const bool directional = l.type == 2u;
     V3 nn_L = directional ? mk(0.f, 0.f, 0.f) : get_unnormalized_L_vec(l, S.world_pos);
-    V3 L = directional ? ld3(l.area_pos2) : nrm3<FAST>(nn_L, plain);
-    V3 Hh = nrm3<FAST>(S.Vv + L, plain);
+    V3 L = directional ? ld3(l.area_pos2) : nrm3<FAST, SHORT>(nn_L, plain);
+    V3 Hh = nrm3<FAST, SHORT>(S.Vv + L, plain);
     float nc_NdotL = dot3(S.N, L);
     float NdotL = clampf(nc_NdotL, 0.0f, 1.0f);
     float NdotH = clampf(dot3(S.N, Hh), 0.0f, 1.0f);
diff --git a/araytracingjourney_amd/csrc/art_sweeps.hip b/araytracingjourney_amd/csrc/art_sweeps.hip
--- a/araytracingjourney_amd/csrc/art_sweeps.hip
+++ b/araytracingjourney_amd/csrc/art_sweeps.hip
@@ -4,14 +4,6 @@
 
 __device__ __attribute__((noinline)) float plain_inv_sqrt(float x) { return 1.0f / sqrtf(x); }
 __device__ __attribute__((noinline)) float plain_sqrt(float x) { return sqrtf(x); }
-__device__ __forceinline__ float inv_sqrt_short(float x) {
-    float y = __builtin_amdgcn_rsqf(x);
-    float s = x * y, h = 0.5f * y;
-    s = fmaf(s, fmaf(-h, s, 0.5f), s);
-    s = fmaf(fmaf(-s, s, x), h, s);
-    float q = __builtin_amdgcn_rcpf(s);
-    return fmaf(fmaf(-s, q, 1.0f), q, q);
-}
 constexpr uint32_t kSweepBlocks = 4096;
 template <int WHICH> __global__ __launch_bounds__(kBlock) void k_math_sweep(uint32_t first_bits, uint64_t count, uint32_t stride, unsigned long long *__restrict__ out) {
     unsigned long long bad = 0, fast_n = 0, bad_at = ~0ull;
@@ -56,6 +48,69 @@
 }
 void math_sweep_guard(float guard[2]) { guard[0] = kExactLo; guard[1] = kExactHi; }
 
+__device__ __attribute__((noinline)) float plain_rcp_dir(float x) { return 1.0f / safe_dir(x); }
+__device__ __attribute__((noinline)) float plain_div(float a, float b) { return a / b; }
+constexpr uint32_t kDivPairSet = 254u * 254u * 64u, kDivCamMaxW = 16384u, kDivCamCols = kDivCamMaxW + 32u;
+__host__ __device__ inline uint32_t div_hash(uint32_t v) { v ^= v >> 16; v *= 0x7feb352du; v ^= v >> 15; v *= 0x846ca68bu; v ^= v >> 16; return v; }
+__host__ __device__ inline bool div_pair(uint32_t which, uint32_t j, uint32_t seed, uint32_t &a, uint32_t &b) {
+    if (which == 3u) {
+        if (j >= kDivPairSet) return false;
+        const uint32_t k = j & 63u, e = j >> 6, ea = e / 254u + 1u, eb = e % 254u + 1u;
+        const uint32_t edge[4] = {0u, 1u, 0x400000u, 0x7FFFFFu};
+        uint32_t ma, mb, sa = 0u, sb = 0u;
+        if (k < 16u) { ma = edge[k >> 2]; mb = edge[k & 3u]; }
+        else { const uint32_t h0 = div_hash(2u * j + seed), h1 = div_hash(2u * j + 1u + seed * 0x9E3779B1u); ma = h0 & 0x7FFFFFu; mb = h1 & 0x7FFFFFu; sa = h0 >> 31; sb = h1 >> 31; }
+        a = sa << 31 | ea << 23 | ma; b = sb << 31 | eb << 23 | mb;
+        return true;
+    }
+    const uint32_t W = j / kDivCamCols + 1u, x = j % kDivCamCols;
+    if (W > kDivCamMaxW || x >= ((W + 31u) & ~31u)) return false;
+    const float fa = (float)x + 0.5f, fb = (float)W;
+    __builtin_memcpy(&a, &fa, 4); __builtin_memcpy(&b, &fb, 4);
+    return true;
+}
+template <int WHICH> __global__ __launch_bounds__(kBlock) void k_div_sweep(uint32_t first_bits, uint64_t count, uint32_t stride, uint32_t numer_bits, unsigned long long *__restrict__ out) {
+    unsigned long long bad = 0, short_n = 0, lanes = 0, bad_at = ~0ull;
+    const uint64_t step = (uint64_t)gridDim.x * kBlock;
+    for (uint64_t i = (uint64_t)blockIdx.x * kBlock + threadIdx.x; i < count; i += step) {
+        const uint32_t j = first_bits + (uint32_t)i * stride;
+        float got, ref; bool in;
+        if (WHICH == 0) {
+            const float x = __uint_as_float(j), d = fabsf(safe_dir(x));
+            in = d >= kExactLo && d <= kExactHi;
+            got = in ? rcp_core(safe_dir(x)) : 1.0f / safe_dir(x); ref = plain_rcp_dir(x);
+        } else {
+            uint32_t ab = numer_bits, bb = j;
+            if (WHICH >= 3 && !div_pair((uint32_t)WHICH, j, numer_bits, ab, bb)) continue;
+            const float a = __uint_as_float(ab), b = __uint_as_float(bb);
+            in = div_core_domain(a, b);
+            got = in ? (WHICH == 2 ? a * __builtin_amdgcn_rcpf(b) : div_core(a, b)) : a / b; ref = plain_div(a, b);
+        }
+        if (__float_as_uint(got) != __float_as_uint(ref)) { bad++; if (i < bad_at) bad_at = i; }
+        short_n += in ? 1u : 0u; lanes++;
+    }
+    for (int off = 32; off >= 1; off >>= 1) {
+        bad += __shfl_xor(bad, off); short_n += __shfl_xor(short_n, off); lanes += __shfl_xor(lanes, off);
+        const unsigned long long o = __shfl_xor(bad_at, off); bad_at = o < bad_at ? o : bad_at;
+    }
+    if ((threadIdx.x & 63u) == 0) {
+        if (bad) { atomicAdd(&out[0], bad); atomicMin(&out[1], bad_at); }
+        if (short_n) atomicAdd(&out[2], short_n);
+        if (lanes) atomicAdd(&out[3], lanes);
+    }
+}
+void launch_div_sweep(uint32_t which, uint32_t first_bits, uint64_t count, uint32_t stride, uint32_t numer_bits, unsigned long long *out, hipStream_t s) {
+    const uint32_t blocks = (uint32_t)std::min<uint64_t>(kSweepBlocks, (count + kBlock - 1) / kBlock);
+    if (!blocks) return;
+    if (which == 0) k_div_sweep<0><<<blocks, kBlock, 0, s>>>(first_bits, count, stride, numer_bits, out);
+    else if (which == 1) k_div_sweep<1><<<blocks, kBlock, 0, s>>>(first_bits, count, stride, numer_bits, out);
+    else if (which == 2) k_div_sweep<2><<<blocks, kBlock, 0, s>>>(first_bits, count, stride, numer_bits, out);
+    else if (which == 3) k_div_sweep<3><<<blocks, kBlock, 0, s>>>(first_bits, count, stride, numer_bits, out);
+    else k_div_sweep<4><<<blocks, kBlock, 0, s>>>(first_bits, count, stride, numer_bits, out);
+}
+void div_sweep_guard(float guard[4]) { guard[0] = kExactLo; guard[1] = kExactHi; guard[2] = kDivLo; guard[3] = kDivHi; }
+bool div_sweep_pair(uint32_t which, uint32_t j, uint32_t seed, uint32_t &a, uint32_t &b) { return div_pair(which, j, seed, a, b); }
+
 __device__ __attribute__((noinline)) float plain_pow22(float x) { return __ocml_pow_f32(x, 2.2f); }
 __device__ __attribute__((noinline)) float plain_quotient(float a, float b) { return a / b; }
 __device__ __forceinline__ float quotient_rcp(float a, float b) { return a * __builtin_amdgcn_rcpf(b); }
diff --git a/araytracingjourney_amd/renderer.py b/araytracingjourney_amd/renderer.py
--- a/araytracingjourney_amd/renderer.py
+++ b/araytracingjourney_amd/renderer.py
@@ -628,6 +628,11 @@
         bad, fast, first, guard = C.c_uint64(0), C.c_uint64(0), C.c_uint32(0), (C.c_float * 2)()
         check(self._L.art_parity_math_sweep(self._ctx, which, first_bits, count, stride, C.byref(bad), C.byref(first), C.byref(fast), guard))
         return dict(mismatches=bad.value, first_bad_bits=first.value if bad.value else None, fast_lanes=fast.value, guard=(guard[0], guard[1]))
+
+    def div_sweep(self, which, first_bits=0, count=1 << 32, stride=1, numerator_bits=0x3F800000):
+        bad, short, lanes, first, guard = C.c_uint64(0), C.c_uint64(0), C.c_uint64(0), (C.c_uint32 * 2)(), (C.c_float * 4)()
+        check(self._L.art_parity_div_sweep(self._ctx, which, first_bits, count, stride, numerator_bits, C.byref(bad), first, C.byref(short), C.byref(lanes), guard))
+        return dict(mismatches=bad.value, first_bad=(first[0], first[1]) if bad.value else None, short_lanes=short.value, lanes=lanes.value, guard=(guard[0], guard[1]), domain=(guard[2], guard[3]))
 
     def radiance_sweep(self, which, first_bits=0, count=1 << 32, stride=1, numerator=1.0):
         ulps, worst, bad, first = C.c_uint32(0), C.c_uint32(0), C.c_uint64(0), C.c_uint32(0)
diff --git a/include/art_parity.h b/include/art_parity.h
--- a/include/art_parity.h
+++ b/include/art_parity.h
@@ -45,6 +45,8 @@
 int32_t art_get_wide_nodes(ArtContext *ctx, void *quantised, void *floats, size_t capacity_nodes, uint32_t *n_nodes);
 int32_t art_parity_math_sweep(ArtContext *ctx, uint32_t which, uint32_t first_bits, uint64_t count, uint32_t stride, uint64_t *mismatches, uint32_t *first_bad_bits,
                               uint64_t *fast_lanes, float guard[2]);
+int32_t art_parity_div_sweep(ArtContext *ctx, uint32_t which, uint32_t first_bits, uint64_t count, uint32_t stride, uint32_t numerator_bits, uint64_t *mismatches,
+                             uint32_t first_bad[2], uint64_t *short_lanes, uint64_t *lanes, float guard[4]);
 int32_t art_parity_radiance_sweep(ArtContext *ctx, uint32_t which, uint32_t first_bits, uint64_t count, uint32_t stride, float numerator, uint32_t *max_ulps, uint32_t *worst_bits,
                                   uint64_t *class_mismatches, uint32_t *first_class_bits);
 
```

Measured after the change: 24070 Mray/s (median of 6 runs). 1.02x the previous value.
